# ma-compbio/MATCHA

Measured on AMD Instinct MI355X. Metric: training hyperedges/sec at k∈{2..5}, embed_dim=64; 1/2/4/8 MI355X, higher is better.
Workload: dtype f32; 1 GPU; hg38_1mb bins (N=3067), k in {2,3,4,5} mixed-k zero-padded to L=5, embed_dim=64, front end=table, neg_num=3, dropout on, AdamW lr=1e-3, 400000 known hyperedges; parallelism=dp1, hipgraph=False, table_gradient_exchange=none, embedding_backward=float atomics, exchange_overlapped=False

## Files before the change

matcha_amd/csrc/fused_bwd.hip:

```cpp
#include <stdlib.h>
#include <string.h>

#include "bf16x3.hpp"
#include "kernels.hpp"
#include "tail_reduce.hpp"

namespace matcha {

typedef float f32x16 __attribute__((ext_vector_type(16)));

namespace {

constexpr int kLd = 68;
constexpr float kEpsLn = 1e-5f;
constexpr int kWgSlab = 4 * 4096 + 6 * 64;
constexpr int kVecOff = 4 * 4096;
constexpr int kMaxChunks = 64;

#define ZR8(p)                                                                                           \
  do {                                                                                                   \
    *reinterpret_cast<float4*>(p) = make_float4(0.f, 0.f, 0.f, 0.f);                                     \
    *reinterpret_cast<float4*>((p) + 4) = make_float4(0.f, 0.f, 0.f, 0.f);                               \
  } while (0)

__device__ __forceinline__ void ln_row16(const float4& v, float& mean, float& rstd) {
  const float s = group_sum<16>((v.x + v.y) + (v.z + v.w));
  mean = s * (1.f / 64.f);
  const float a = v.x - mean, b = v.y - mean, c = v.z - mean, e = v.w - mean;
  const float q = group_sum<16>((a * a + b * b) + (c * c + e * e));
  rstd = __builtin_amdgcn_rsqf(q * (1.f / 64.f) + kEpsLn);
}


#define FB_PIN(addr, x) asm volatile("" : "+v"(addr), "+v"((x).a), "+v"((x).b), "+v"((x).c), "+v"((x).d))
template <int ML>
__device__ __forceinline__ void attn_row8_kv(const float* __restrict__ Qs, const float* __restrict__ Xs, const float* __restrict__ Fs,
                                             const float* __restrict__ xpad, const float* __restrict__ Ps, float* __restrict__ dSs, int li, int li0,
                                             int k, int n_pad, int sub, float inv_temp, V8& o, V8& gq, V8& accK, V8& accV) {
  const float padf = (float)n_pad;
  const bool hp = n_pad > 0;
  float p[ML], ds[ML], pp;
  {
    const float4 pa = *reinterpret_cast<const float4*>(&Ps[li * 8]), pb = *reinterpret_cast<const float4*>(&Ps[li * 8 + 4]);
    const float w[8] = {pa.x, pa.y, pa.z, pa.w, pb.x, pb.y, pb.z, pb.w};
#pragma unroll
    for (int j = 0; j < ML; ++j) p[j] = (j < k) ? w[j] : 0.f;
    pp = hp ? w[7] : 0.f;
  }
  const float ppf = padf * pp;
  const int ro0 = li0 * kLd + 8 * sub;
  const V8 go = ld8(&Fs[li * kLd + 8 * sub]);
  const V8 vp = ld8(xpad + 8 * sub);
  const float dsp_raw = group_sum8_dpp(dot8(go, vp));
  float sig = ppf * dsp_raw;
  o = scale8(ppf, vp);
  V8 a = scale8(ppf * dsp_raw, vp);
  V8 vn = ld8(&Xs[ro0]), vn2 = ld8(&Xs[ro0 + (1 < k ? 1 : 0) * kLd]);
#pragma unroll
  for (int j = 0; j < ML; ++j) {
    const V8 v = vn;
    vn = vn2;
    if (j + 2 < ML) {
      int ad = ro0 + (j + 2 < k ? j + 2 : 0) * kLd;
      FB_PIN(ad, o);
      vn2 = ld8(&Xs[ad]);
    }
    axpy8(o, p[j], v);
    const float d = group_sum8_dpp(dot8(go, v));
    ds[j] = d;
    const float wd = p[j] * d;
    sig += wd;
    axpy8(a, wd, v);
  }
#pragma unroll
  for (int j = 0; j < ML; ++j) ds[j] = p[j] * (ds[j] - sig) * inv_temp;
  const float dspf = padf * (pp * (dsp_raw - sig) * inv_temp);
  axpy8(accV, ppf, go);
  {
    const float ns = -sig;
    axpy8(a, ns, o);
    gq = scale8(inv_temp, a);
  }
  {
    int ad = li * kLd + 8 * sub;
    FB_PIN(ad, gq);
    const V8 q = ld8(&Qs[ad]);
    axpy8(accK, dspf, q);
  }
  if (sub == 1) {
    float* dst = dSs + li * 8;
    *reinterpret_cast<float4*>(dst) = make_float4(ds[0], ds[1 % ML], ML > 2 ? ds[2 % ML] : 0.f, ML > 3 ? ds[3 % ML] : 0.f);
    if (ML > 4) *reinterpret_cast<float4*>(dst + 4) = make_float4(ds[4 % ML], ML > 5 ? ds[5 % ML] : 0.f, ML > 6 ? ds[6 % ML] : 0.f, ML > 7 ? ds[7 % ML] : 0.f);
  }
}

template <int ML>
__device__ __forceinline__ void attn_col8(const float* __restrict__ Qs, const float* __restrict__ Fs, const float* __restrict__ Ps,
                                          const float* __restrict__ dSs, int li, int li0, int k, int sub, V8& gk, V8& gv) {
  const int jj = li - li0;
  gk = zero8();
  gv = zero8();
  const int ro0 = li0 * kLd + 8 * sub;
  V8 qn = ld8(&Qs[ro0]), gn = ld8(&Fs[ro0]);
#pragma unroll
  for (int i = 0; i < ML; ++i) {
    const V8 q = qn, go = gn;
    const int ri = li0 + (i < k ? i : 0);
    const float pl = Ps[ri * 8 + jj], dl = dSs[ri * 8 + jj];
    const float pij = (i < k) ? pl : 0.f, dsij = (i < k) ? dl : 0.f;
    if (i + 1 < ML) {
      int a = ro0 + (i + 1 < k ? i + 1 : 0) * kLd;
      FB_PIN(a, gk);
      qn = ld8(&Qs[a]); gn = ld8(&Fs[a]);
    }
    axpy8(gv, pij, go);
    axpy8(gk, dsij, q);
  }
}

#ifdef FB_TIMING
#define FB_T(i) do { const long long now__ = wall_clock64(); tph[i] += now__ - tlast; tlast = now__; } while (0)
#else
#define FB_T(i) do { } while (0)
#endif

#define MFMA16(A, B, C) __builtin_amdgcn_mfma_f32_16x16x4f32((A), (B), (C), 0, 0, 0)

constexpr int kWgSlabM = 2 * 4096 + 4 * 64;
constexpr int kVecOffM = 2 * 4096;
constexpr int kTileH = 32 * kLd;
constexpr int kPS = 80;
constexpr int kPlane = 32 * kPS;
constexpr int kPT = 3 * kPlane;
typedef Planes<kPS, 16> PL;
__device__ __forceinline__ Frag3 frag_row(const short* __restrict__ p) { return PL::row(p); }
__device__ __forceinline__ void frag_store(short* __restrict__ p, const Frag3& f) { PL::store(p, f); }
__device__ __forceinline__ Frag3 frag_col(const short* __restrict__ p) { return PL::col(p); }

struct FusedBwdHArgs {
  const float* X; const float* dDyn; const int32_t* count; const int32_t* half_meta; const int32_t* tok_pos;
  int L; int nhalves; int nchunks;
  const float* mB; const float* mM;
  float* dxh; int64_t tcap;
  int dx_atomic;
  float* wslab;
  const float* rimg;
  const int32_t* xrow;
  const float* rn; int64_t rn_head;
};
constexpr size_t kBwdLdsBytes = (size_t)2 * kTileH * 4 + (size_t)4 * kPT * 2 + (64 + 256 + 256 + 32) * 4;

template <int ML, bool NODE>
__global__ __launch_bounds__(256) __attribute__((amdgpu_waves_per_eu(2, 2))) void fused_bwdh_kernel(FusedBwdHArgs g) {
  extern __shared__ __attribute__((aligned(16))) float lds[];
  float* Xs = lds;
  float* Gs = lds + kTileH;
  short* Xp = reinterpret_cast<short*>(lds + 2 * kTileH);
  short* Dp = Xp + kPT;
  short* RBp = Dp + kPT;
  short* FBp = RBp + kPT;
  float* Rs = reinterpret_cast<float*>(RBp);
  float* Fs = reinterpret_cast<float*>(FBp);
  float* sm = reinterpret_cast<float*>(FBp + kPT);
  float* xpad = sm;
  float* dSs = xpad + 64;
  float* Ps = dSs + 256;
  int* tinfo = reinterpret_cast<int*>(Ps + 256);

  const int tid = threadIdx.x, lane = tid & 63, wave = tid >> 6;
  const int c16 = lane & 15, kq = lane >> 4;
  const int fb = 16 * wave;
  const int srow = tid >> 4, sc4 = (tid & 15) * 4;

  int head, chunk;
  if ((g.nchunks & 7) == 0) {
    const int xcd = blockIdx.x & 7, j = blockIdx.x >> 3;
    head = j & 7;
    chunk = (j >> 3) * 8 + xcd;
  } else {
    head = blockIdx.x & 7;
    chunk = blockIdx.x >> 3;
  }
  const int tr = g.count[1];
  int nh = g.count[3];
  if (nh > g.nhalves) nh = g.nhalves;
  const int per = (nh + g.nchunks - 1) / g.nchunks;
  const int tile_lo = chunk * per;
  const int tile_hi = (tile_lo + per < nh) ? tile_lo + per : nh;
  const float inv_temp = 0.125f;
#ifdef FB_TIMING
  long long tph[8] = {0, 0, 0, 0, 0, 0, 0, 0};
  long long tlast = wall_clock64();
#endif

  if (tid < 16) {
    const float4 xv = *reinterpret_cast<const float4*>(g.X + (NODE ? (int64_t)0 : (int64_t)tr * 64) + sc4);
    if constexpr (NODE) {
      *reinterpret_cast<float4*>(&xpad[sc4]) = xv;
    } else {
      float m, rs;
      ln_row16(xv, m, rs);
      *reinterpret_cast<float4*>(&xpad[sc4]) = make_float4((xv.x - m) * rs, (xv.y - m) * rs, (xv.z - m) * rs, (xv.w - m) * rs);
    }
  }

  f32x4 ab0 = {0.f, 0.f, 0.f, 0.f}, ab1 = ab0, ab2 = ab0, ab3 = ab0, am0 = ab0, am1 = ab0, am2 = ab0, am3 = ab0;
  V8 accK = zero8(), accV = zero8();
  f2 cd0 = {0.f, 0.f}, cd1 = cd0;
  V8 accR = zero8();

  const int4* meta = reinterpret_cast<const int4*>(g.half_meta);
  const int4 mzero = make_int4(0, 0, 0, 0);
  int4 mc = tile_lo < tile_hi ? meta[tile_lo] : mzero;
  int4 mn = tile_lo + 1 < tile_hi ? meta[tile_lo + 1] : mzero;
  float4 xn0, xn1, dn0, dn1;
  int tpn = 0;
  int kx0 = 0, kx1 = 0;
#define FBH_KEY_GLOAD(I, M)                                                                              \
  do {                                                                                                   \
    const int row__ = srow + 16 * (I);                                                                   \
    kx##I = g.xrow[(M).x + (row__ < (M).y ? row__ : ((M).y > 0 ? (M).y - 1 : 0))];                       \
  } while (0)
  f32x4 ri0, ri1, pn = {0.f, 0.f, 0.f, 0.f};
#define FBH_ROW_GLOAD(I, M)                                                                              \
  do {                                                                                                   \
    const int row__ = srow + 16 * (I);                                                                   \
    const int64_t tok__ = (M).x + (row__ < (M).y ? row__ : ((M).y > 0 ? (M).y - 1 : 0));                 \
    xn##I = *reinterpret_cast<const float4*>(g.X + (NODE ? (int64_t)kx##I : tok__) * 64 + sc4);           \
    dn##I = *reinterpret_cast<const float4*>(g.dDyn + tok__ * 64 + sc4);                                 \
  } while (0)
#define FBH_ROWS_GLOAD(M)                                                                                \
  do {                                                                                                   \
    FBH_ROW_GLOAD(0, M); FBH_ROW_GLOAD(1, M);                                                            \
    if (tid < 32) tpn = g.tok_pos[(M).x + (tid < (M).y ? tid : ((M).y > 0 ? (M).y - 1 : 0))];           \
  } while (0)
  const bool r_tab = NODE && g.rn != nullptr;
#define FBH_R_GLOAD()                                                                                    \
  do {                                                                                                   \
    const float* rh__ = g.rn + (int64_t)head * g.rn_head + sc4;                                          \
    ri0 = *reinterpret_cast<const f32x4*>(rh__ + (int64_t)kx0 * 64); ri1 = *reinterpret_cast<const f32x4*>(rh__ + (int64_t)kx1 * 64); \
  } while (0)
#define FBH_ROW_STAGE(I)                                                                                 \
  do {                                                                                                   \
    const int row__ = srow + 16 * (I);                                                                   \
    const float msk__ = row__ < n_real ? 1.f : 0.f;                                                      \
    const float4 xv__ = xn##I, dv__ = dn##I;                                                             \
    float4 xh__;                                                                                         \
    if constexpr (NODE) {                                                                                \
      xh__ = make_float4(xv__.x * msk__, xv__.y * msk__, xv__.z * msk__, xv__.w * msk__);                \
    } else {                                                                                             \
      const float mean__ = group_sum16_dpp((xv__.x + xv__.y) + (xv__.z + xv__.w)) * (1.f / 64.f);        \
      const float a__ = xv__.x - mean__, b__ = xv__.y - mean__, c__ = xv__.z - mean__, e__ = xv__.w - mean__; \
      const float q__ = group_sum16_dpp((a__ * a__ + b__ * b__) + (c__ * c__ + e__ * e__));              \
      const float rs__ = msk__ * __builtin_amdgcn_rsqf(q__ * (1.f / 64.f) + kEpsLn);                     \
      xh__ = make_float4(a__ * rs__, b__ * rs__, c__ * rs__, e__ * rs__);                                \
    }                                                                                                    \
    *reinterpret_cast<float4*>(&Xs[row__ * kLd + sc4]) = xh__;                                           \
    {                                                                                                    \
      const P3 p0__ = split2(xh__.x, xh__.y), p1__ = split2(xh__.z, xh__.w);                             \
      short* d__ = Xp + row__ * kPS + sc4;                                                               \
      *reinterpret_cast<u32x2*>(d__) = (u32x2){p0__.h, p1__.h}; *reinterpret_cast<u32x2*>(d__ + kPlane) = (u32x2){p0__.m, p1__.m}; \
      *reinterpret_cast<u32x2*>(d__ + 2 * kPlane) = (u32x2){p0__.l, p1__.l};                             \
    }                                                                                                    \
    const float4 dm__ = make_float4(dv__.x * msk__, dv__.y * msk__, dv__.z * msk__, dv__.w * msk__);     \
    {                                                                                                    \
      const P3 p0__ = split2(dm__.x, dm__.y), p1__ = split2(dm__.z, dm__.w);                             \
      short* d__ = Dp + row__ * kPS + sc4;                                                               \
      *reinterpret_cast<u32x2*>(d__) = (u32x2){p0__.h, p1__.h}; *reinterpret_cast<u32x2*>(d__ + kPlane) = (u32x2){p0__.m, p1__.m}; \
      *reinterpret_cast<u32x2*>(d__ + 2 * kPlane) = (u32x2){p0__.l, p1__.l};                             \
    }                                                                                                    \
    cd0 += (f2){dm__.x, dm__.y}; cd1 += (f2){dm__.z, dm__.w};                                            \
  } while (0)
#define FBH_RIMG_GLOAD(HALF)                                                                             \
  do {                                                                                                   \
    const f32x4* r__ = reinterpret_cast<const f32x4*>(g.rimg + ((int64_t)(HALF) * MATCHA_N_HEAD + head) * kImgRecH);  \
    if (tid < 64) pn = __builtin_nontemporal_load(r__ + 512 + tid);                                      \
    if (!r_tab) { ri0 = __builtin_nontemporal_load(r__ + tid); ri1 = __builtin_nontemporal_load(r__ + 256 + tid); } \
  } while (0)
  Frag3 Mf[2], Bf[2];
  {
    if constexpr (NODE) { FBH_KEY_GLOAD(0, mc); FBH_KEY_GLOAD(1, mc); }
    FBH_ROWS_GLOAD(mc);
    if constexpr (NODE) { if (r_tab) FBH_R_GLOAD(); FBH_KEY_GLOAD(0, mn); FBH_KEY_GLOAD(1, mn); }
    if (tile_lo < tile_hi) FBH_RIMG_GLOAD(tile_lo);
    const float* mp = g.mM + (int64_t)head * 4096 + (8 * kq) * 64 + fb + c16;
    const float* bp = g.mB + (int64_t)head * 4096 + (8 * kq) * 64 + fb + c16;
#pragma unroll
    for (int s = 0; s < 2; ++s) {
      float vm[8], vb[8];
#pragma unroll
      for (int j = 0; j < 8; ++j) { vm[j] = mp[(32 * s + j) * 64]; vb[j] = bp[(32 * s + j) * 64]; }
      Mf[s] = split8(vm); Bf[s] = split8(vb);
    }
  }

  for (int tile = tile_lo; tile < tile_hi; ++tile) {
    const int4 mnn = tile + 2 < tile_hi ? meta[tile + 2] : mzero;
    const int t0 = mc.x, n_real = mc.y;
    FB_T(0);
    __syncthreads();
    FB_T(7);
    {
      FBH_ROW_STAGE(0); FBH_ROW_STAGE(1);
      if (tid < 32) tinfo[tid] = tid < n_real ? ((tid - (tpn & 255)) | (tpn & ~255)) : 0;
      if (r_tab) {
        *reinterpret_cast<f32x4*>(&Rs[srow * kLd + sc4]) = ri0; *reinterpret_cast<f32x4*>(&Rs[(srow + 16) * kLd + sc4]) = ri1;
      } else {
        f32x4* d__ = reinterpret_cast<f32x4*>(&Rs[(lane & 31) * kLd + 8 * wave + 4 * (lane >> 5)]);
        d__[0] = ri0; d__[8] = ri1;
      }
      if (tid < 64) reinterpret_cast<f32x4*>(Ps)[tid] = pn;
    }
    __syncthreads();
    int tid_ = tid;
    asm volatile("" : "+v"(tid_));
    const int lane = tid_ & 63, wave = tid_ >> 6;
    const int c16 = lane & 15, kq = lane >> 4;
    const int fb = 16 * wave;
    const int srow = tid_ >> 4, sc4 = (tid_ & 15) * 4;
    const int sub = lane & 7;
    (void)srow; (void)sc4;
    {
      f32x4 acc0 = {0.f, 0.f, 0.f, 0.f}, acc1 = acc0;
      const short* dp = Dp + c16 * kPS + 8 * kq;
#pragma unroll
      for (int s = 0; s < 2; ++s) {
        const Frag3 b0 = frag_row(dp + 32 * s), b1 = frag_row(dp + 16 * kPS + 32 * s);
        acc0 = mma6(acc0, Mf[s], b0); acc1 = mma6(acc1, Mf[s], b1);
      }
      *reinterpret_cast<f32x4*>(&Fs[c16 * kLd + fb + 4 * kq]) = acc0;
      *reinterpret_cast<f32x4*>(&Fs[(16 + c16) * kLd + fb + 4 * kq]) = acc1;
    }
    FB_T(1);
    __syncthreads();
    FB_T(7);
    {
      V8 o0, q0, k0, v0;
      const int la = wave * 8 + (lane >> 3);
      const bool acta = la < n_real;
      int ia = 0;
      if (acta) { ia = tinfo[la]; attn_row8_kv<ML>(Rs, Xs, Fs, xpad, Ps, dSs, la, ia & 255, ia >> 8, g.L - (ia >> 8), sub, inv_temp, o0, q0, accK, accV); }
      __builtin_amdgcn_sched_barrier(0);
      FB_T(2);
      __syncthreads();
      FB_T(7);
      if (acta) {
        attn_col8<ML>(Rs, Fs, Ps, dSs, la, ia & 255, ia >> 8, sub, k0, v0);
        k0.a += v0.a; k0.b += v0.b; k0.c += v0.c; k0.d += v0.d;
        st8(&Gs[la * kLd + 8 * sub], k0);
      } else {
        ZR8(&Gs[la * kLd + 8 * sub]);
      }
      FB_T(3);
      __syncthreads();
      FB_T(7);
      if (!acta) { o0 = zero8(); q0 = zero8(); }
      frag_store(FBp + la * kPS + 8 * sub, split8(o0));
      frag_store(RBp + la * kPS + 8 * sub, split8(q0));
      accR.a += q0.a; accR.b += q0.b; accR.c += q0.c; accR.d += q0.d;
    }
    FB_T(4);
    __syncthreads();
    FB_T(7);
    FBH_ROWS_GLOAD(mn);
    if constexpr (NODE) { if (r_tab) FBH_R_GLOAD(); FBH_KEY_GLOAD(0, mnn); FBH_KEY_GLOAD(1, mnn); }
    if (g.dx_atomic) {
      const float* gp = Gs + (4 * kq) * kLd + fb + c16;
      f32x4 dx0 = {gp[0], gp[kLd], gp[2 * kLd], gp[3 * kLd]};
      f32x4 dx1 = {gp[16 * kLd], gp[17 * kLd], gp[18 * kLd], gp[19 * kLd]};
      const short* arow = RBp + c16 * kPS + 8 * kq;
#pragma unroll
      for (int s = 0; s < 2; ++s) {
        const Frag3 a0 = frag_row(arow + 32 * s), a1 = frag_row(arow + 16 * kPS + 32 * s);
        dx0 = mma6(dx0, a0, Bf[s]); dx1 = mma6(dx1, a1, Bf[s]);
      }
      float* out = g.dxh + ((int64_t)t0 + 4 * kq) * 64 + fb + c16;
#pragma unroll
      for (int reg = 0; reg < 4; ++reg) {
        if (4 * kq + reg < n_real) unsafeAtomicAdd(out + reg * 64, dx0[reg]);
        if (16 + 4 * kq + reg < n_real) unsafeAtomicAdd(out + (16 + reg) * 64, dx1[reg]);
      }
    } else {
      f32x4 dx0 = *reinterpret_cast<const f32x4*>(&Gs[c16 * kLd + fb + 4 * kq]);
      f32x4 dx1 = *reinterpret_cast<const f32x4*>(&Gs[(16 + c16) * kLd + fb + 4 * kq]);
      const short* arow = RBp + c16 * kPS + 8 * kq;
#pragma unroll
      for (int s = 0; s < 2; ++s) {
        const Frag3 a0 = frag_row(arow + 32 * s), a1 = frag_row(arow + 16 * kPS + 32 * s);
        dx0 = mma6(dx0, Bf[s], a0); dx1 = mma6(dx1, Bf[s], a1);
      }
      float* out = g.dxh + ((int64_t)head * g.tcap + t0 + c16) * 64 + fb + 4 * kq;
      if (c16 < n_real) *reinterpret_cast<f32x4*>(out) = dx0;
      if (16 + c16 < n_real) *reinterpret_cast<f32x4*>(out + 16 * 64) = dx1;
    }
    FB_T(5);
    if (tile + 1 < tile_hi) FBH_RIMG_GLOAD(tile + 1);
    {
      const int blk = ((4 * kq + ((lane & 15) >> 2)) * kPS) + 4 * (lane & 3);
      const Frag3 xb = frag_col(Xp + blk + fb), zb = frag_col(FBp + blk + fb);
      {
        const Frag3 r0 = frag_col(RBp + blk), r1 = frag_col(RBp + blk + 16);
        ab0 = mma6(ab0, r0, xb); ab1 = mma6(ab1, r1, xb);
        const Frag3 r2 = frag_col(RBp + blk + 32), r3 = frag_col(RBp + blk + 48);
        ab2 = mma6(ab2, r2, xb); ab3 = mma6(ab3, r3, xb);
      }
      {
        const Frag3 d0 = frag_col(Dp + blk), d1 = frag_col(Dp + blk + 16);
        am0 = mma6(am0, d0, zb); am1 = mma6(am1, d1, zb);
        const Frag3 d2 = frag_col(Dp + blk + 32), d3 = frag_col(Dp + blk + 48);
        am2 = mma6(am2, d2, zb); am3 = mma6(am3, d3, zb);
      }
    }
    FB_T(6);
    mc = mn; mn = mnn;
  }

  __syncthreads();
#ifdef FB_TIMING
  if (blockIdx.x == 0 && (tid == 0 || tid == 192))
    printf("fused_bwdh wg0 wave %d us: stage %.1f dZ %.1f attn-row %.1f attn-col %.1f attn-write %.1f dx %.1f tn %.1f barrier-wait %.1f (halves %d)\n", tid >> 6,
           tph[0] * 0.01, tph[1] * 0.01, tph[2] * 0.01, tph[3] * 0.01, tph[4] * 0.01, tph[5] * 0.01, tph[6] * 0.01, tph[7] * 0.01, tile_hi - tile_lo);
#endif
  float* slab = g.wslab + ((int64_t)head * g.nchunks + chunk) * kWgSlabM;
  {
    const int col = fb + c16;
#pragma unroll
    for (int reg = 0; reg < 4; ++reg) {
      const int row = 4 * kq + reg;
      slab[0 * 4096 + row * 64 + col] = ab0[reg]; slab[0 * 4096 + (row + 16) * 64 + col] = ab1[reg];
      slab[0 * 4096 + (row + 32) * 64 + col] = ab2[reg]; slab[0 * 4096 + (row + 48) * 64 + col] = ab3[reg];
      slab[1 * 4096 + row * 64 + col] = am0[reg]; slab[1 * 4096 + (row + 16) * 64 + col] = am1[reg];
      slab[1 * 4096 + (row + 32) * 64 + col] = am2[reg]; slab[1 * 4096 + (row + 48) * 64 + col] = am3[reg];
    }
  }
  float* redd = lds;
  {
    const float cdv[4] = {cd0.x, cd0.y, cd1.x, cd1.y};
#pragma unroll
    for (int i = 0; i < 4; ++i) {
      float v = cdv[i];
      v += __shfl_xor(v, 16, 64);
      v += __shfl_xor(v, 32, 64);
      if (lane < 16) redd[wave * 64 + 4 * lane + i] = v;
    }
  }
  float* redr = lds + 4 * 64;
  float* redp = lds + 8 * 64;
  const float accp[16] = {accK.a.x + accV.a.x, accK.a.y + accV.a.y, accK.b.x + accV.b.x, accK.b.y + accV.b.y,
                          accK.c.x + accV.c.x, accK.c.y + accV.c.y, accK.d.x + accV.d.x, accK.d.y + accV.d.y,
                          accR.a.x, accR.a.y, accR.b.x, accR.b.y, accR.c.x, accR.c.y, accR.d.x, accR.d.y};
#pragma unroll
  for (int i = 0; i < 16; ++i) {
    float v = accp[i];
    v += __shfl_xor(v, 8, 64);
    v += __shfl_xor(v, 16, 64);
    v += __shfl_xor(v, 32, 64);
    if (lane < 8) (i < 8 ? redp : redr)[wave * 64 + 8 * lane + (i & 7)] = v;
  }
  __syncthreads();
  if (tid < 64) {
    slab[kVecOffM + 64 + tid] = (redd[tid] + redd[64 + tid]) + (redd[128 + tid] + redd[192 + tid]);
    slab[kVecOffM + tid] = (redr[tid] + redr[64 + tid]) + (redr[128 + tid] + redr[192 + tid]);
    slab[kVecOffM + 128 + tid] = (redp[tid] + redp[64 + tid]) + (redp[128 + tid] + redp[192 + tid]);
  }
}

struct ChainArgs {
  const float* wslab; int nchunks;
  float* red;
  const float* wq; const float* wk; const float* wv; const float* cq; const float* cv;
  const float* fc1_w;
  float* out;
  float* dxpad;
};
constexpr int kFbmReduceX = (kWgSlabM + 255) / 256;
constexpr int kFbmReduceBlocks = kFbmReduceX * MATCHA_N_HEAD;
__global__ __launch_bounds__(256) void fbm_reduce_kernel(ChainArgs a, TailReduceArgs tl, int tail_blocks) {
  __shared__ float4 part[8 * 32];
  if ((int)blockIdx.x >= kFbmReduceBlocks) {
    tail_reduce_role(tl, (int)blockIdx.x - kFbmReduceBlocks, part);
    return;
  }
  const int head = blockIdx.x / kFbmReduceX, i = (blockIdx.x % kFbmReduceX) * 256 + threadIdx.x;
  if (i >= kWgSlabM) return;
  const float* base = a.wslab + (int64_t)head * a.nchunks * kWgSlabM + i;
  float s0 = 0.f, s1 = 0.f, s2 = 0.f, s3 = 0.f, s4 = 0.f, s5 = 0.f, s6 = 0.f, s7 = 0.f;
  int c = 0;
  for (; c + 7 < a.nchunks; c += 8) {
    s0 += base[(int64_t)c * kWgSlabM]; s1 += base[(int64_t)(c + 1) * kWgSlabM]; s2 += base[(int64_t)(c + 2) * kWgSlabM]; s3 += base[(int64_t)(c + 3) * kWgSlabM];
    s4 += base[(int64_t)(c + 4) * kWgSlabM]; s5 += base[(int64_t)(c + 5) * kWgSlabM]; s6 += base[(int64_t)(c + 6) * kWgSlabM]; s7 += base[(int64_t)(c + 7) * kWgSlabM];
  }
  for (; c < a.nchunks; ++c) s0 += base[(int64_t)c * kWgSlabM];
  a.red[(int64_t)head * kWgSlabM + i] = ((s0 + s1) + (s2 + s3)) + ((s4 + s5) + (s6 + s7));
}
__device__ __forceinline__ void mm64_slice(const float* __restrict__ A, int a_rs, int a_cs, const float* __restrict__ B, int b_rs, int b_cs,
                                           const float* __restrict__ u, const float* __restrict__ v, float* __restrict__ out, int slice,
                                           float* __restrict__ As, float* __restrict__ Bs) {
  const int tid = threadIdx.x;
  {
    float av[4], bv[16];
#pragma unroll
    for (int t = 0; t < 4; ++t) { const int i = tid + 256 * t; av[t] = A[(int64_t)(16 * slice + (i >> 6)) * a_rs + (int64_t)(i & 63) * a_cs]; }
#pragma unroll
    for (int t = 0; t < 16; ++t) { const int i = tid + 256 * t; bv[t] = B[(int64_t)(i >> 6) * b_rs + (int64_t)(i & 63) * b_cs]; }
#pragma unroll
    for (int t = 0; t < 4; ++t) { const int i = tid + 256 * t; As[(i >> 6) * 65 + (i & 63)] = av[t]; }
#pragma unroll
    for (int t = 0; t < 16; ++t) { const int i = tid + 256 * t; Bs[(i >> 6) * 65 + (i & 63)] = bv[t]; }
  }
  __syncthreads();
  const int lane = tid & 63, wave = tid >> 6, c16 = lane & 15, kq = lane >> 4;
  f32x4 acc = {0.f, 0.f, 0.f, 0.f};
#pragma unroll
  for (int kk = 0; kk < 16; ++kk) acc = MFMA16(As[c16 * 65 + 4 * kk + kq], Bs[(4 * kk + kq) * 65 + 16 * wave + c16], acc);
  const int j = 16 * wave + c16;
  const float vj = u ? v[j] : 0.f;
#pragma unroll
  for (int reg = 0; reg < 4; ++reg) {
    const int i = 4 * kq + reg;
    out[(16 * slice + i) * 64 + j] = acc[reg] + (u ? u[16 * slice + i] * vj : 0.f);
  }
}
__global__ __launch_bounds__(256) void fbm_chain_kernel(ChainArgs a) {
  __shared__ float As[16 * 65];
  __shared__ float Bs[64 * 65];
  const int slice = blockIdx.x, job = blockIdx.y, head = blockIdx.z, tid = threadIdx.x;
  const float* red = a.red + (int64_t)head * kWgSlabM;
  const float* dB = red; const float* dM = red + 4096; const float* db = red + kVecOffM;
  const float* dbdyn = a.red + kVecOffM + 64;
  const float* Wq = a.wq + (int64_t)head * 4096; const float* Wk = a.wk + (int64_t)head * 4096; const float* Wv = a.wv + (int64_t)head * 4096;
  const float* Wf = a.fc1_w + head * 64;
  float* out = a.out + (int64_t)head * kWgSlab;
  if (job == 0) {
    mm64_slice(Wk, 64, 1, dB, 64, 1, nullptr, nullptr, out + 0 * 4096, slice, As, Bs);
  } else if (job == 1) {
    mm64_slice(Wq, 64, 1, dB, 1, 64, a.cq + head * 64, db, out + 1 * 4096, slice, As, Bs);
  } else if (job == 2) {
    mm64_slice(Wf, 1, 512, dM, 64, 1, nullptr, nullptr, out + 2 * 4096, slice, As, Bs);
  } else {
    mm64_slice(dM, 64, 1, Wv, 1, 64, dbdyn, a.cv + head * 64, out + 3 * 4096, slice, As, Bs);
  }
  if (slice == 0 && job == 0 && tid < 64) {
    float s0 = 0.f, s1 = 0.f, t0 = 0.f, t1 = 0.f;
#pragma unroll 8
    for (int x = 0; x < 64; x += 2) {
      s0 += Wk[tid * 64 + x] * db[x]; s1 += Wk[tid * 64 + x + 1] * db[x + 1];
      t0 += Wf[x * 512 + tid] * dbdyn[x]; t1 += Wf[(x + 1) * 512 + tid] * dbdyn[x + 1];
    }
    const float s = s0 + s1, t = t0 + t1;
    out[kVecOff + tid] = s;
    out[kVecOff + 64 + tid] = 0.f;
    out[kVecOff + 128 + tid] = t;
    out[kVecOff + 192 + tid] = 0.f; out[kVecOff + 256 + tid] = 0.f;
    out[kVecOff + 320 + tid] = head == 0 ? dbdyn[tid] : 0.f;
    if (head == 0) {
      float p = 0.f;
      for (int hh = 0; hh < MATCHA_N_HEAD; ++hh) p += a.red[(int64_t)hh * kWgSlabM + kVecOffM + 128 + tid];
      a.dxpad[tid] = p;
    }
  }
}

struct UnfoldArgs {
  const float* wslab; int nchunks;
  const float* X; const int32_t* count; int x_pad_row0;
  const float* W[3]; const float* g[3]; const float* b[3];
  float* gW[3]; float* gfc1;
  float* part;
};
__global__ __launch_bounds__(256) void fb_unfold_kernel(UnfoldArgs a) {
  __shared__ float red[16][3][64];
  const int slice = blockIdx.x, mat = blockIdx.y, head = blockIdx.z;
  const int tid = threadIdx.x, rl = tid >> 4, c4 = (tid & 15) * 4;
  const int row = slice * 16 + rl;
  const float* base = a.wslab + (int64_t)head * a.nchunks * kWgSlab;
  float4 s = make_float4(0.f, 0.f, 0.f, 0.f);
  {
    float4 t0 = s, t1 = s, t2 = s, t3 = s;
    const float* pb = base + mat * 4096 + row * 64 + c4;
    int c = 0;
    for (; c + 3 < a.nchunks; c += 4) {
      const float4 v0 = *reinterpret_cast<const float4*>(pb + (int64_t)c * kWgSlab), v1 = *reinterpret_cast<const float4*>(pb + (int64_t)(c + 1) * kWgSlab);
      const float4 v2 = *reinterpret_cast<const float4*>(pb + (int64_t)(c + 2) * kWgSlab), v3 = *reinterpret_cast<const float4*>(pb + (int64_t)(c + 3) * kWgSlab);
      t0.x += v0.x; t0.y += v0.y; t0.z += v0.z; t0.w += v0.w;
      t1.x += v1.x; t1.y += v1.y; t1.z += v1.z; t1.w += v1.w;
      t2.x += v2.x; t2.y += v2.y; t2.z += v2.z; t2.w += v2.w;
      t3.x += v3.x; t3.y += v3.y; t3.z += v3.z; t3.w += v3.w;
    }
    for (; c < a.nchunks; ++c) {
      const float4 v = *reinterpret_cast<const float4*>(pb + (int64_t)c * kWgSlab);
      t0.x += v.x; t0.y += v.y; t0.z += v.z; t0.w += v.w;
    }
    s.x = (t0.x + t1.x) + (t2.x + t3.x); s.y = (t0.y + t1.y) + (t2.y + t3.y);
    s.z = (t0.z + t1.z) + (t2.z + t3.z); s.w = (t0.w + t1.w) + (t2.w + t3.w);
  }
  if (mat == 3) {
    float4* o = reinterpret_cast<float4*>(a.gfc1 + (int64_t)row * 512 + head * 64 + c4);
    float4 v = *o;
    v.x += s.x; v.y += s.y; v.z += s.z; v.w += s.w;
    *o = v;
    return;
  }
  float dc = 0.f, dpad = 0.f;
  for (int c = 0; c < a.nchunks; ++c) {
    const float* vb = base + (int64_t)c * kWgSlab + kVecOff;
    dc += vb[mat * 64 + row];
    if (mat > 0) dpad += vb[192 + (mat - 1) * 64 + row];
  }
  const float4 xv = *reinterpret_cast<const float4*>(a.X + (a.x_pad_row0 ? (int64_t)0 : (int64_t)a.count[1] * 64) + c4);
  float m, rs;
  ln_row16(xv, m, rs);
  s.x += dpad * (xv.x - m) * rs; s.y += dpad * (xv.y - m) * rs; s.z += dpad * (xv.z - m) * rs; s.w += dpad * (xv.w - m) * rs;
  dc += dpad;
  const int64_t wi = ((int64_t)head * 64 + row) * 64 + c4;
  const float4 W = *reinterpret_cast<const float4*>(a.W[mat] + wi);
  const float4 G = *reinterpret_cast<const float4*>(a.g[mat] + c4), Bv = *reinterpret_cast<const float4*>(a.b[mat] + c4);
  {
    float4* o = reinterpret_cast<float4*>(a.gW[mat] + wi);
    float4 v = *o;
    v.x += s.x * G.x + dc * Bv.x; v.y += s.y * G.y + dc * Bv.y; v.z += s.z * G.z + dc * Bv.z; v.w += s.w * G.w + dc * Bv.w;
    *o = v;
  }
  *reinterpret_cast<float4*>(&red[rl][0][c4]) = make_float4(s.x * W.x, s.y * W.y, s.z * W.z, s.w * W.w);
  *reinterpret_cast<float4*>(&red[rl][1][c4]) = make_float4(dc * W.x, dc * W.y, dc * W.z, dc * W.w);
  *reinterpret_cast<float4*>(&red[rl][2][c4]) = make_float4(dpad * W.x * G.x, dpad * W.y * G.y, dpad * W.z * G.z, dpad * W.w * G.w);
  __syncthreads();
  if (tid < 192) {
    const int which = tid >> 6, k = tid & 63;
    float t = 0.f;
#pragma unroll
    for (int q = 0; q < 16; ++q) t += red[q][which][k];
    a.part[(((int64_t)(head * 4 + slice) * 3 + mat) * 3 + which) * 64 + k] = t;
  }
}

struct Unfold2Args {
  const float* part; const float* wslab; int nchunks;
  float* dg[3]; float* db[3]; float* dfc1_b; float* dxpad;
  int dxpad_add;
};
__global__ __launch_bounds__(512) void fb_unfold2_kernel(Unfold2Args a) {
  const int vec = threadIdx.x >> 6, k = threadIdx.x & 63;
  float s = 0.f;
  if (vec < 6) {
    const int mat = vec >> 1, which = vec & 1;
    for (int p = 0; p < 32; ++p) s += a.part[(((int64_t)p * 3 + mat) * 3 + which) * 64 + k];
    float* o = (which == 0 ? a.dg[mat] : a.db[mat]) + k;
    *o += s;
  } else if (vec == 6) {
    for (int p = 0; p < 32; ++p) s += a.part[(((int64_t)p * 3 + 1) * 3 + 2) * 64 + k] + a.part[(((int64_t)p * 3 + 2) * 3 + 2) * 64 + k];
    a.dxpad[k] = a.dxpad_add ? a.dxpad[k] + s : s;
  } else {
    for (int c = 0; c < a.nchunks; ++c) s += a.wslab[(int64_t)c * kWgSlab + kVecOff + 320 + k];
    a.dfc1_b[k] += s;
  }
}

__global__ __launch_bounds__(256) void lnhat_bwd_kernel(const float* __restrict__ X, const float* __restrict__ dxh, int64_t tcap,
                                                        const float* __restrict__ dxpad, const float* __restrict__ dXs,
                                                        float* __restrict__ dZ0, const int32_t* __restrict__ count, int nslab) {
  const int T = count[0];
  const int64_t t = (int64_t)blockIdx.x * 16 + (threadIdx.x >> 4);
  const int c4 = (threadIdx.x & 15) * 4;
  if (t >= T) return;
  const float4 xv = *reinterpret_cast<const float4*>(X + t * 64 + c4);
  float m, rs;
  ln_row16(xv, m, rs);
  const float4 xh = make_float4((xv.x - m) * rs, (xv.y - m) * rs, (xv.z - m) * rs, (xv.w - m) * rs);
  float4 d;
  if (t < T - 1) {
    d = *reinterpret_cast<const float4*>(dxh + t * 64 + c4);
    for (int hd = 1; hd < nslab; ++hd) {
      const float4 v = *reinterpret_cast<const float4*>(dxh + ((int64_t)hd * tcap + t) * 64 + c4);
      d.x += v.x; d.y += v.y; d.z += v.z; d.w += v.w;
    }
  } else {
    d = *reinterpret_cast<const float4*>(dxpad + c4);
  }
  const float a = group_sum<16>((d.x + d.y) + (d.z + d.w)) * (1.f / 64.f);
  const float b = group_sum<16>((d.x * xh.x + d.y * xh.y) + (d.z * xh.z + d.w * xh.w)) * (1.f / 64.f);
  const float4 s = *reinterpret_cast<const float4*>(dXs + t * 64 + c4);
  float4 o;
  o.x = (rs * (d.x - a - xh.x * b) + s.x) * (1.f - xv.x * xv.x);
  o.y = (rs * (d.y - a - xh.y * b) + s.y) * (1.f - xv.y * xv.y);
  o.z = (rs * (d.z - a - xh.z * b) + s.z) * (1.f - xv.z * xv.z);
  o.w = (rs * (d.w - a - xh.w * b) + s.w) * (1.f - xv.w * xv.w);
  *reinterpret_cast<float4*>(dZ0 + t * 64 + c4) = o;
}

int chunks_for(int ntiles) {
  const int cus = device_cu_count();
  int c = cus / MATCHA_N_HEAD;
  if (c > kMaxChunks) c = kMaxChunks;
  if (c > ntiles) c = ntiles;
  return c < 1 ? 1 : c;
}

}

const float* fused_bwd_dxpad(const float* ws) { return ws + (size_t)MATCHA_N_HEAD * kMaxChunks * kWgSlab + 32 * 3 * 3 * 64; }

size_t fused_bwd_ws_floats(int64_t B, int L) {
  (void)B; (void)L;
  return (size_t)MATCHA_N_HEAD * kMaxChunks * kWgSlab + (size_t)32 * 3 * 3 * 64 + 64;
}

int launch_fused_bwd_merged(const matcha_tensors& p, const float* folded, const float* merged, const float* X, const float* dDyn, const float* dXs,
                            const Ragged& rg, int64_t B, int L, float* dxh, float* ws, matcha_tensors& grads, float* dZ0, hipStream_t st, const float* rimg,
                            bool dx_atomic, bool dx_zeroed, const TailReduceArgs* tail, const int32_t* xrow, const float* xhatN, const float* rn, int64_t rn_rows) {
  const int64_t tcap = B * L + 1;
  MATCHA_CHECK_ARG(!xrow || xhatN, "fused backward: the node route needs the table of normalised rows");
  MATCHA_CHECK_ARG(!rn || xrow, "fused backward: the r table belongs to the node route");
  if (dx_atomic && !dx_zeroed) MATCHA_TRY(zero_async(dxh, (size_t)tcap * 64 * sizeof(float), st));
  int nchunks = 2 * chunks_for(rg.nhalves);
  if (nchunks > kMaxChunks) nchunks = kMaxChunks;
  if (nchunks > rg.nhalves) nchunks = rg.nhalves > 0 ? rg.nhalves : 1;
  float* wslab = ws;
  float* chain = ws + (size_t)MATCHA_N_HEAD * kMaxChunks * kWgSlabM;
  float* part = ws + (size_t)MATCHA_N_HEAD * kMaxChunks * kWgSlab;
  float* dxpad = part + 32 * 3 * 3 * 64;
  const size_t wsz = (size_t)MATCHA_N_HEAD * 64 * 64, csz = (size_t)MATCHA_N_HEAD * 64;
  const MergedView mv = merged_view(merged);
  {
    FusedBwdHArgs g;
    g.X = xrow ? xhatN : X; g.dDyn = dDyn; g.count = rg.count; g.half_meta = rg.half_meta; g.tok_pos = rg.tok_pos; g.L = L; g.nhalves = rg.nhalves; g.nchunks = nchunks;
    g.mB = mv.B; g.mM = mv.M; g.dxh = dxh; g.tcap = tcap; g.dx_atomic = dx_atomic ? 1 : 0; g.wslab = wslab; g.rimg = rimg; g.xrow = xrow;
    g.rn = rn; g.rn_head = rn_rows * 64;
    const size_t lds = kBwdLdsBytes;
    auto launch = [&](auto kfn) {
      (void)hipFuncSetAttribute(reinterpret_cast<const void*>(kfn), hipFuncAttributeMaxDynamicSharedMemorySize, 160 * 1024);
      hipLaunchKernelGGL(kfn, dim3(MATCHA_N_HEAD * nchunks), dim3(256), lds, st, g);
    };
    ProfScope ps(MATCHA_PROF_FUSED_BWD, (double)tcap * MATCHA_N_HEAD * 8.0 * 2.0 * 64.0 * 64.0, st);
    switch (L <= 2 ? 2 : (L <= 6 ? L : 8)) {
      case 2: if (xrow) launch(fused_bwdh_kernel<2, true>); else launch(fused_bwdh_kernel<2, false>); break;
      case 3: if (xrow) launch(fused_bwdh_kernel<3, true>); else launch(fused_bwdh_kernel<3, false>); break;
      case 4: if (xrow) launch(fused_bwdh_kernel<4, true>); else launch(fused_bwdh_kernel<4, false>); break;
      case 5: if (xrow) launch(fused_bwdh_kernel<5, true>); else launch(fused_bwdh_kernel<5, false>); break;
      case 6: if (xrow) launch(fused_bwdh_kernel<6, true>); else launch(fused_bwdh_kernel<6, false>); break;
      default: if (xrow) launch(fused_bwdh_kernel<8, true>); else launch(fused_bwdh_kernel<8, false>); break;
    }
    MATCHA_CHECK_LAUNCH("fused_bwdh_kernel");
  }
  {
    ChainArgs c;
    c.wslab = wslab; c.nchunks = nchunks; c.red = chain + (size_t)MATCHA_N_HEAD * kWgSlab;
    c.wq = folded; c.wk = folded + wsz; c.wv = folded + 2 * wsz; c.cq = folded + 3 * wsz; c.cv = c.cq + 2 * csz;
    c.fc1_w = p.fc1_w; c.out = chain; c.dxpad = dxpad;
    TailReduceArgs tl;
    if (tail) tl = *tail; else memset(&tl, 0, sizeof(tl));
    const int tail_blocks = tail ? kTailRoleBlocks : 0;
    hipLaunchKernelGGL(fbm_reduce_kernel, dim3((unsigned)(kFbmReduceBlocks + tail_blocks)), dim3(256), 0, st, c, tl, tail_blocks);
    MATCHA_CHECK_LAUNCH("fbm_reduce_kernel");
    hipLaunchKernelGGL(fbm_chain_kernel, dim3(4, 4, MATCHA_N_HEAD), dim3(256), 0, st, c);
    MATCHA_CHECK_LAUNCH("fbm_chain_kernel");
  }
  {
    UnfoldArgs a;
    a.wslab = chain; a.nchunks = 1; a.X = X; a.count = rg.count; a.x_pad_row0 = xrow ? 1 : 0;
    a.W[0] = p.w_q; a.W[1] = p.w_k; a.W[2] = p.w_v;
    a.g[0] = p.ln_q_g; a.g[1] = p.ln_k_g; a.g[2] = p.ln_v_g;
    a.b[0] = p.ln_q_b; a.b[1] = p.ln_k_b; a.b[2] = p.ln_v_b;
    a.gW[0] = grads.w_q; a.gW[1] = grads.w_k; a.gW[2] = grads.w_v; a.gfc1 = grads.fc1_w;
    a.part = part;
    hipLaunchKernelGGL(fb_unfold_kernel, dim3(4, 4, MATCHA_N_HEAD), dim3(256), 0, st, a);
    MATCHA_CHECK_LAUNCH("fb_unfold_kernel");
    Unfold2Args b;
    b.part = part; b.wslab = chain; b.nchunks = 1;
    b.dg[0] = grads.ln_q_g; b.dg[1] = grads.ln_k_g; b.dg[2] = grads.ln_v_g;
    b.db[0] = grads.ln_q_b; b.db[1] = grads.ln_k_b; b.db[2] = grads.ln_v_b;
    b.dfc1_b = grads.fc1_b; b.dxpad = dxpad; b.dxpad_add = 1;
    hipLaunchKernelGGL(fb_unfold2_kernel, dim3(1), dim3(512), 0, st, b);
    MATCHA_CHECK_LAUNCH("fb_unfold2_kernel");
  }
  if (dZ0) {
    MATCHA_CHECK_ARG(!xrow, "fused backward: the node route has no dZ0 output");
    hipLaunchKernelGGL(lnhat_bwd_kernel, dim3((unsigned)cdiv(tcap, 16)), dim3(256), 0, st, X, dxh, tcap, dxpad, dXs, dZ0, rg.count, dx_atomic ? 1 : MATCHA_N_HEAD);
    MATCHA_CHECK_LAUNCH("lnhat_bwd_kernel");
  }
  return MATCHA_OK;
}

}
```

matcha_amd/csrc/fused_fwd32.hip:

```cpp
#include "kernels.hpp"
#include "prep_heads.hpp"

#ifndef F32_ABL
#define F32_ABL 0
#endif

namespace matcha {

typedef float f32x16 __attribute__((ext_vector_type(16)));

namespace {

constexpr int kLdH = 68;
constexpr int kHT = 32 * kLdH;
constexpr float kEps32 = 1e-5f;
constexpr int kTailVec32 = 2 * 4096;
constexpr int kTailSlab32 = 2 * 4096 + 10 * 64;

struct FL { f32x16 lo, hi; };

__device__ __forceinline__ float xhalf_sum(float v) {
  float a = v, b = v;
  asm volatile("s_nop 1\n\tv_permlane32_swap_b32 %0, %1" : "+v"(a), "+v"(b));
  return a + b;
}
__device__ __forceinline__ float fl_sum(const FL& a) {
  float s0 = 0.f, s1 = 0.f;
#pragma unroll
  for (int e = 0; e < 16; ++e) { s0 += a.lo[e]; s1 += a.hi[e]; }
  return s0 + s1;
}
__device__ __forceinline__ float fl_dot(const FL& a, const FL& b) {
  float s0 = 0.f, s1 = 0.f;
#pragma unroll
  for (int e = 0; e < 16; ++e) { s0 += a.lo[e] * b.lo[e]; s1 += a.hi[e] * b.hi[e]; }
  return s0 + s1;
}
__device__ __forceinline__ void fl_stats(const FL& v, float& mean, float& rstd) {
  mean = xhalf_sum(fl_sum(v)) * (1.f / 64.f);
  float q0 = 0.f, q1 = 0.f;
#pragma unroll
  for (int e = 0; e < 16; ++e) { const float a = v.lo[e] - mean, b = v.hi[e] - mean; q0 += a * a; q1 += b * b; }
  rstd = __builtin_amdgcn_rsqf(xhalf_sum(q0 + q1) * (1.f / 64.f) + kEps32);
}
__device__ __forceinline__ void fl_store(float* __restrict__ rowp, const FL& v) {
#pragma unroll
  for (int g = 0; g < 4; ++g) {
    *reinterpret_cast<f32x4*>(rowp + 8 * g) = (f32x4){v.lo[4 * g], v.lo[4 * g + 1], v.lo[4 * g + 2], v.lo[4 * g + 3]};
    *reinterpret_cast<f32x4*>(rowp + 32 + 8 * g) = (f32x4){v.hi[4 * g], v.hi[4 * g + 1], v.hi[4 * g + 2], v.hi[4 * g + 3]};
  }
}
__device__ __forceinline__ FL fl_load(const float* __restrict__ rowp) {
  FL v;
#pragma unroll
  for (int g = 0; g < 4; ++g) {
    const f32x4 a = *reinterpret_cast<const f32x4*>(rowp + 8 * g), b = *reinterpret_cast<const f32x4*>(rowp + 32 + 8 * g);
    v.lo[4 * g] = a.x; v.lo[4 * g + 1] = a.y; v.lo[4 * g + 2] = a.z; v.lo[4 * g + 3] = a.w;
    v.hi[4 * g] = b.x; v.hi[4 * g + 1] = b.y; v.hi[4 * g + 2] = b.z; v.hi[4 * g + 3] = b.w;
  }
  return v;
}
__device__ __forceinline__ float fl_dot_lds(const FL& q, const float* __restrict__ rowp) {
  f2 s = {0.f, 0.f}, t = {0.f, 0.f};
#pragma unroll
  for (int g = 0; g < 4; ++g) {
    const f32x4 a = *reinterpret_cast<const f32x4*>(rowp + 8 * g), b = *reinterpret_cast<const f32x4*>(rowp + 32 + 8 * g);
    s = __builtin_elementwise_fma((f2){q.lo[4 * g], q.lo[4 * g + 1]}, (f2){a.x, a.y}, s);
    t = __builtin_elementwise_fma((f2){q.lo[4 * g + 2], q.lo[4 * g + 3]}, (f2){a.z, a.w}, t);
    s = __builtin_elementwise_fma((f2){q.hi[4 * g], q.hi[4 * g + 1]}, (f2){b.x, b.y}, s);
    t = __builtin_elementwise_fma((f2){q.hi[4 * g + 2], q.hi[4 * g + 3]}, (f2){b.z, b.w}, t);
  }
  s += t;
  return s.x + s.y;
}
__device__ __forceinline__ void fl_axpy_lds(FL& o, float w, const float* __restrict__ rowp) {
#pragma unroll
  for (int g = 0; g < 4; ++g) {
    const f32x4 a = *reinterpret_cast<const f32x4*>(rowp + 8 * g), b = *reinterpret_cast<const f32x4*>(rowp + 32 + 8 * g);
    o.lo[4 * g] += w * a.x; o.lo[4 * g + 1] += w * a.y; o.lo[4 * g + 2] += w * a.z; o.lo[4 * g + 3] += w * a.w;
    o.hi[4 * g] += w * b.x; o.hi[4 * g + 1] += w * b.y; o.hi[4 * g + 2] += w * b.z; o.hi[4 * g + 3] += w * b.w;
  }
}
__device__ __forceinline__ void fl_add_vec(FL& v, const float* __restrict__ vec_h) {
#pragma unroll
  for (int g = 0; g < 4; ++g) {
    const f32x4 a = *reinterpret_cast<const f32x4*>(vec_h + 8 * g), b = *reinterpret_cast<const f32x4*>(vec_h + 32 + 8 * g);
    v.lo[4 * g] += a.x; v.lo[4 * g + 1] += a.y; v.lo[4 * g + 2] += a.z; v.lo[4 * g + 3] += a.w;
    v.hi[4 * g] += b.x; v.hi[4 * g + 1] += b.y; v.hi[4 * g + 2] += b.z; v.hi[4 * g + 3] += b.w;
  }
}
__device__ __forceinline__ FL fl_vec(const float* __restrict__ vec_h) {
  FL v;
#pragma unroll
  for (int e = 0; e < 16; ++e) { v.lo[e] = 0.f; v.hi[e] = 0.f; }
  fl_add_vec(v, vec_h);
  return v;
}
__device__ __forceinline__ void fl_store_global(float* __restrict__ rowp_h, const FL& v) {
#pragma unroll
  for (int g = 0; g < 4; ++g) {
    *reinterpret_cast<f32x4*>(rowp_h + 8 * g) = (f32x4){v.lo[4 * g], v.lo[4 * g + 1], v.lo[4 * g + 2], v.lo[4 * g + 3]};
    *reinterpret_cast<f32x4*>(rowp_h + 32 + 8 * g) = (f32x4){v.hi[4 * g], v.hi[4 * g + 1], v.hi[4 * g + 2], v.hi[4 * g + 3]};
  }
}

__device__ __forceinline__ int f32_tok(int lane, int t0, int n, int tok_pad) {
  asm volatile("" : "+v"(lane));
  const int rr = lane & 31;
  return rr < n ? t0 + rr : tok_pad;
}
__device__ __forceinline__ int64_t f32_row(int lane, int t0, int n, int tok_pad) {
  asm volatile("" : "+v"(lane));
  const int rr = lane & 31;
  return (int64_t)(rr < n ? t0 + rr : tok_pad) * 64 + 4 * (lane >> 5);
}
#define F32_TOK() f32_tok(lane, t0, n, tok_pad)
#define F32_ROW() f32_row(lane, t0, n, tok_pad)
__device__ __forceinline__ FL fl_unpark(const float* __restrict__ base, int64_t off) { return fl_load(base + off); }
__device__ __forceinline__ FL fl_unpark_lds(const float* __restrict__ base, int off) {
  asm volatile("" : "+v"(off));
  return fl_load(base + off);
}
#define F32_WAVE_SYNC() asm volatile("s_waitcnt lgkmcnt(0)" ::: "memory")

#define MFMA32(A, B, C) __builtin_amdgcn_mfma_f32_32x32x2f32((A), (B), (C), 0, 0, 0)

#define MFMA_BF(A, B, C) __builtin_amdgcn_mfma_f32_32x32x16_bf16(__builtin_bit_cast(bf16x8, (A)), __builtin_bit_cast(bf16x8, (B)), (C), 0, 0, 0)
#ifndef F32_WIN
#define F32_WIN 6
#endif

struct B3 { u32x4 h, m, l; };
#define FL_CHUNK(V, C, J) ((C) < 2 ? (V).lo[8 * ((C) & 1) + (J)] : (V).hi[8 * ((C) & 1) + (J)])
#define FL_SPLIT(OUT, V, C)                                                                              \
  do {                                                                                                   \
    _Pragma("unroll") for (int q__ = 0; q__ < 4; ++q__) {                                                \
      if (F32_ABL & 128) { (OUT).h[q__] = __builtin_bit_cast(uint32_t, FL_CHUNK(V, C, 2 * q__)); (OUT).m[q__] = (OUT).h[q__]; (OUT).l[q__] = (OUT).h[q__]; continue; } \
      const P3 p__ = split2(FL_CHUNK(V, C, 2 * q__), FL_CHUNK(V, C, 2 * q__ + 1));                       \
      (OUT).h[q__] = p__.h; (OUT).m[q__] = p__.m; (OUT).l[q__] = p__.l;                                  \
    }                                                                                                    \
  } while (0)
#define WB_MMA(ACC, XB, S)                                                                               \
  do {                                                                                                   \
    const u32x4 ah__ = W_[(3 * (S)) % F32_WIN], am__ = W_[(3 * (S) + 1) % F32_WIN], al__ = W_[(3 * (S) + 2) % F32_WIN]; \
    if constexpr (((S) & 1) == 0) {                                                                      \
      ACC.lo = MFMA_BF(al__, (XB).h, ACC.lo); ACC.lo = MFMA_BF(ah__, (XB).l, ACC.lo); ACC.lo = MFMA_BF(am__, (XB).m, ACC.lo); \
      ACC.lo = MFMA_BF(am__, (XB).h, ACC.lo); ACC.lo = MFMA_BF(ah__, (XB).m, ACC.lo); ACC.lo = MFMA_BF(ah__, (XB).h, ACC.lo); \
    } else {                                                                                             \
      ACC.hi = MFMA_BF(al__, (XB).h, ACC.hi); ACC.hi = MFMA_BF(ah__, (XB).l, ACC.hi); ACC.hi = MFMA_BF(am__, (XB).m, ACC.hi); \
      ACC.hi = MFMA_BF(am__, (XB).h, ACC.hi); ACC.hi = MFMA_BF(ah__, (XB).m, ACC.hi); ACC.hi = MFMA_BF(ah__, (XB).h, ACC.hi); \
    }                                                                                                    \
  } while (0)
#define WB_REFILL(S, PF)                                                                                 \
  do {                                                                                                   \
    if ((PF) && !(F32_ABL & 32)) {                                                                       \
      W_[(3 * (S)) % F32_WIN] = wp[lane]; W_[(3 * (S) + 1) % F32_WIN] = (wp + 64)[lane]; W_[(3 * (S) + 2) % F32_WIN] = (wp + 128)[lane]; \
    }                                                                                                    \
    wp += 192;                                                                                           \
    asm volatile("" ::: "memory");          \
    __builtin_amdgcn_sched_barrier(0);                                                                   \
  } while (0)
#define WB_CHUNK(ACC, B, C, PF)                                                                          \
  do {                                                                                                   \
    B3 xb__;                                                                                             \
    FL_SPLIT(xb__, B, C);                                                                                \
    WB_MMA(ACC, xb__, 2 * (C)); WB_REFILL(2 * (C), PF); WB_MMA(ACC, xb__, 2 * (C) + 1); WB_REFILL(2 * (C) + 1, PF); \
  } while (0)
#define W32_CHAIN(ACC, B, PF_LAST)                                                                       \
  do { WB_CHUNK(ACC, B, 0, true); WB_CHUNK(ACC, B, 1, true); WB_CHUNK(ACC, B, 2, true); WB_CHUNK(ACC, B, 3, PF_LAST); } while (0)
#define W32_CHAIN_XS(ACC, XS, PF_LAST)                                                                   \
  do {                                                                                                   \
    WB_MMA(ACC, XS[0], 0); WB_REFILL(0, true); WB_MMA(ACC, XS[0], 1); WB_REFILL(1, true);                \
    WB_MMA(ACC, XS[1], 2); WB_REFILL(2, true); WB_MMA(ACC, XS[1], 3); WB_REFILL(3, true);                \
    WB_MMA(ACC, XS[2], 4); WB_REFILL(4, true); WB_MMA(ACC, XS[2], 5); WB_REFILL(5, true);                \
    WB_MMA(ACC, XS[3], 6); WB_REFILL(6, PF_LAST); WB_MMA(ACC, XS[3], 7); WB_REFILL(7, PF_LAST);          \
  } while (0)
#define W32_PRIME_AT(MAT)                                                                                \
  do {                                                                                                   \
    wp = g.wfrag + (MAT) * kFragU4;                                                                      \
    _Pragma("unroll") for (int i__ = 0; i__ < F32_WIN; ++i__) W_[i__] = (wp + i__ * 64)[lane];           \
    wp += F32_WIN * 64;                                                                                  \
  } while (0)

__device__ __forceinline__ FL fl_zero() {
  FL v;
#pragma unroll
  for (int e = 0; e < 16; ++e) { v.lo[e] = 0.f; v.hi[e] = 0.f; }
  return v;
}

}

__global__ __launch_bounds__(256) void prep_heads_kernel(PrepArgs a) {
  __shared__ __attribute__((aligned(16))) float sm[kPrepLdsFloats];
  prep_heads_role(a, blockIdx.x, blockIdx.y, blockIdx.z, sm);
}

struct Fwd32Args {
  const float* X;
  const int32_t* xrow;
  const int32_t* row_off; const int32_t* tok_slot; const int32_t* count; const int32_t* half_meta; const int32_t* tok_pos;
  int L;
  const u32x4* wfrag;
  HeadParams hp;
  const float* y; const float* w;
  float* Y; float* H1; float* H2;
  float* logits; float* row_loss;
  const uint64_t* seed;
  float p_fc1, p_pff;
  float* ddyn0; float* dXs; float* tslab; float alpha_over_B;
  int objective;
  float* qkv;
  float* tail_dh2;
  const float* rn;
  int rn_rows;
};

template <int ML>
__global__ __launch_bounds__(64) __attribute__((amdgpu_waves_per_eu(2, 2))) void fused_fwd32_kernel(Fwd32Args g) {
  extern __shared__ __attribute__((aligned(16))) float lds[];
#ifdef FF_TIMING
  long long tph[16] = {0};
  long long tlast = wall_clock64();
#define FF_T(i) do { const long long now__ = wall_clock64(); tph[i] += now__ - tlast; tlast = now__; } while (0)
#else
#define FF_T(i) do { } while (0)
#endif
  float* TK = lds;
  float* TV = lds + kHT;
  float* outs = lds + 2 * kHT;
  float* douts = outs + 32;
  const int lane = threadIdx.x, r = lane & 31, h = lane >> 5;

  const int4 meta = reinterpret_cast<const int4*>(g.half_meta)[blockIdx.x];
  const int t0 = meta.x, n = meta.y, b0 = meta.z, n_h = meta.w;
  if (n_h <= 0) return;
  const int tok_pad = g.count[1];
  const float inv_temp = 0.125f;
  const bool real = r < n;

  const u32x4* wp;
  u32x4 W_[F32_WIN];
  W32_PRIME_AT(g.rn ? 2 : 0);
  {
    const f32x4* bsrc = reinterpret_cast<const f32x4*>(g.wfrag + (kNMat + 1) * kFragU4);
    for (int i4 = lane; i4 < kNBias * 16; i4 += 64) reinterpret_cast<f32x4*>(TV)[i4] = bsrc[i4];
  }
#define F32_BIAS(ROW) fl_vec(TV + (ROW) * 64 + 4 * h)

  int64_t xoff = F32_ROW();
  if (g.xrow) xoff = (int64_t)g.xrow[F32_TOK()] * 64 + 4 * h;
  FL xh = fl_load(g.X + xoff);
  int pos = 0, k = 0;
  if (real) {
    const int tp = g.tok_pos[F32_TOK()];
    pos = tp & 255; k = tp >> 8;
  }
  const int li0 = r - pos;
  float rx;
  {
    float mean;
    fl_stats(xh, mean, rx);
#pragma unroll
    for (int e = 0; e < 16; ++e) { xh.lo[e] = (xh.lo[e] - mean) * rx; xh.hi[e] = (xh.hi[e] - mean) * rx; }
  }
  constexpr int kRec = kImgRecH;
  float* const img_base = g.qkv ? g.qkv + (int64_t)blockIdx.x * MATCHA_N_HEAD * kImgRecH : nullptr;
  const bool img_on = g.qkv != nullptr && real;
#define F32_IMG_STORE(ACC, HD, M)                                                                        \
  do {                                                                                                   \
    if (img_on && !(F32_ABL & 2)) {                                                                      \
      int l__ = lane;                                                                                    \
      asm volatile("" : "+v"(l__));                                                                      \
      f32x4* d__ = reinterpret_cast<f32x4*>(img_base + (HD) * kRec + (M) * 4096 + l__ * 4);             \
      _Pragma("unroll") for (int g__ = 0; g__ < 4; ++g__) {                                              \
        if (F32_ABL & 16) {                                                                              \
          d__[g__ * 64] = (f32x4){ACC.lo[4 * g__], ACC.lo[4 * g__ + 1], ACC.lo[4 * g__ + 2], ACC.lo[4 * g__ + 3]};   \
          d__[(4 + g__) * 64] = (f32x4){ACC.hi[4 * g__], ACC.hi[4 * g__ + 1], ACC.hi[4 * g__ + 2], ACC.hi[4 * g__ + 3]}; \
        } else {                                                                                         \
        __builtin_nontemporal_store((f32x4){ACC.lo[4 * g__], ACC.lo[4 * g__ + 1], ACC.lo[4 * g__ + 2], ACC.lo[4 * g__ + 3]}, d__ + g__ * 64); \
        __builtin_nontemporal_store((f32x4){ACC.hi[4 * g__], ACC.hi[4 * g__ + 1], ACC.hi[4 * g__ + 2], ACC.hi[4 * g__ + 3]}, d__ + (4 + g__) * 64); \
        }                                                                                                \
      }                                                                                                  \
    }                                                                                                    \
  } while (0)

  const int n_pad = g.L - k;
  const float padf = (float)n_pad;
  const bool hpad = n_pad > 0;
  int ro[ML + 1];
#pragma unroll
  for (int j = 0; j < ML; ++j) ro[j] = (li0 + (j < k ? j : 0)) * kLdH + 4 * h;
  ro[ML] = n * kLdH + 4 * h;
  float* krow = TK + r * kLdH + 4 * h;
  float* vrow = TV + r * kLdH + 4 * h;

#define F32_PIN1(V) asm volatile("" : "+v"(V))
  float p[ML + 1];
  float sc_part = 0.f;
#define F32_SC_PIECE(S)                                                                                  \
  do {                                                                                                   \
    constexpr int j__ = (S) >> 1, hf__ = (S) & 1;                                                        \
    if constexpr (j__ <= ML) {                                                                           \
      const float* rp__ = TK + ro[j__] + 32 * hf__;                                                      \
      f2 s__ = {0.f, 0.f}, t__ = {0.f, 0.f};                                                             \
      _Pragma("unroll") for (int g__ = 0; g__ < 4; ++g__) {                                              \
        const f32x4 a__ = *reinterpret_cast<const f32x4*>(rp__ + 8 * g__);                               \
        const f32x16& qq__ = hf__ ? q.hi : q.lo;                                                         \
        s__ = __builtin_elementwise_fma((f2){qq__[4 * g__], qq__[4 * g__ + 1]}, (f2){a__.x, a__.y}, s__); \
        t__ = __builtin_elementwise_fma((f2){qq__[4 * g__ + 2], qq__[4 * g__ + 3]}, (f2){a__.z, a__.w}, t__); \
      }                                                                                                  \
      s__ += t__;                                                                                        \
      if constexpr (hf__ == 0) { sc_part = s__.x + s__.y; F32_PIN1(sc_part); }                            \
      else {                                                                                             \
        float a__ = xhalf_sum(sc_part + (s__.x + s__.y)) * inv_temp;                                     \
        if constexpr (j__ < ML) a__ = (j__ == pos) ? -1e32f : a__;      \
        p[j__] = a__;                                                                                    \
        F32_PIN1(p[j__]);                                                                                \
      }                                                                                                  \
    }                                                                                                    \
    if constexpr ((S) == 2 * (ML + 1)) {                                                                 \
      float mx__ = -3.4e38f;                                                                             \
      _Pragma("unroll") for (int i__ = 0; i__ < ML; ++i__) mx__ = (i__ < k) ? fmaxf(mx__, p[i__]) : mx__; \
      mx__ = hpad ? fmaxf(mx__, p[ML]) : mx__;                                                           \
      float den__ = 0.f;                                                                                 \
      _Pragma("unroll") for (int i__ = 0; i__ < ML; ++i__) { p[i__] = (i__ < k) ? __expf(p[i__] - mx__) : 0.f; den__ += p[i__]; } \
      p[ML] = hpad ? __expf(p[ML] - mx__) : 0.f;                                                         \
      den__ += padf * p[ML];                                                                             \
      const float inv__ = __builtin_amdgcn_rcpf(den__);                                                  \
      _Pragma("unroll") for (int i__ = 0; i__ <= ML; ++i__) { p[i__] *= inv__; F32_PIN1(p[i__]); }       \
    }                                                                                                    \
    if constexpr ((S) == 2 * (ML + 1) + 1) {                                                             \
       \
      if (img_on && h == 0) {                                                                            \
        float wv__[8];                                                                                   \
        _Pragma("unroll") for (int i__ = 0; i__ < 8; ++i__) wv__[i__] = i__ < ML ? p[i__ < ML ? i__ : 0] : 0.f; \
        if (hpad) wv__[7] = p[ML];                                                                       \
        int l__ = lane;                                                                                  \
        asm volatile("" : "+v"(l__));                                                                    \
        f32x4* dst__ = reinterpret_cast<f32x4*>(img_base + hd * kRec + 2048 + (l__ & 31) * 8);          \
        __builtin_nontemporal_store((f32x4){wv__[0], wv__[1], wv__[2], wv__[3]}, dst__);                 \
        __builtin_nontemporal_store((f32x4){wv__[4], wv__[5], wv__[6], wv__[7]}, dst__ + 1);             \
      }                                                                                                  \
    }                                                                                                    \
  } while (0)
#define F32_STAGE8(MAC) do { MAC(0); MAC(1); MAC(2); MAC(3); MAC(4); MAC(5); MAC(6); MAC(7); } while (0)

  FF_T(0);
  fl_store(krow, xh);
  FL dyn;
  if (!g.rn) {
  B3 xs[4];
  FL_SPLIT(xs[0], xh, 0); FL_SPLIT(xs[1], xh, 1); FL_SPLIT(xs[2], xh, 2); FL_SPLIT(xs[3], xh, 3);
  F32_WAVE_SYNC();
  dyn = F32_BIAS(kBiasDyn);
  {
    FL q = F32_BIAS(kBiasR), o;
    W32_CHAIN_XS(q, xs, true);
    F32_IMG_STORE(q, 0, 0);
    FF_T(1);
#define F32_Z_PIECE(S)                                                                                   \
  do {                                                                                                   \
    constexpr int j__ = (S) >> 1, hf__ = (S) & 1;                                                        \
    if constexpr (j__ <= ML) {                                                                           \
      const float* rp__ = TK + ro[j__] + 32 * hf__;                                                      \
      const float w__ = j__ < ML ? p[j__] : padf * p[ML];                                                \
      const f2 w2__ = {w__, w__};                                                                        \
      f32x16& oo__ = hf__ ? o.hi : o.lo;                                                                 \
      _Pragma("unroll") for (int g__ = 0; g__ < 4; ++g__) {                                              \
        const f32x4 a__ = *reinterpret_cast<const f32x4*>(rp__ + 8 * g__);                               \
        const f2 u0__ = __builtin_elementwise_fma(w2__, (f2){a__.x, a__.y}, (f2){oo__[4 * g__], oo__[4 * g__ + 1]});     \
        const f2 u1__ = __builtin_elementwise_fma(w2__, (f2){a__.z, a__.w}, (f2){oo__[4 * g__ + 2], oo__[4 * g__ + 3]}); \
        oo__[4 * g__] = u0__.x; oo__[4 * g__ + 1] = u0__.y; oo__[4 * g__ + 2] = u1__.x; oo__[4 * g__ + 3] = u1__.y;      \
      }                                                                                                  \
      asm volatile("" : "+v"(oo__));                                                                     \
    }                                                                                                    \
  } while (0)
#define F32_MG_PIECE(Q)                                                                                  \
  do {                                                                                                   \
    if constexpr ((F32_ABL & 1) != 0) { } else                                                           \
    if constexpr ((Q) < 2 * (ML + 1) + 2) F32_SC_PIECE(Q); else F32_Z_PIECE((Q) - (2 * (ML + 1) + 2));   \
  } while (0)
#define F32_MG_ONLY(S) do { F32_MG_PIECE(5 * (S)); F32_MG_PIECE(5 * (S) + 1); F32_MG_PIECE(5 * (S) + 2); F32_MG_PIECE(5 * (S) + 3); F32_MG_PIECE(5 * (S) + 4); } while (0)
#define F32_MG_STEP(S) do { WB_MMA(acc, xs[(S) >> 1], S); F32_MG_ONLY(S); WB_REFILL(S, true); } while (0)
    int hd = 0;
    for (; hd + 1 < MATCHA_N_HEAD; ++hd) {
      o = fl_zero();
      {
        FL acc = F32_BIAS(kBiasR + hd + 1);
        F32_STAGE8(F32_MG_STEP);
        q = acc;
        F32_IMG_STORE(q, hd + 1, 0);
      }
      FF_T(2);
      W32_CHAIN(dyn, o, true);
      FF_T(5);
    }
    o = fl_zero();
    F32_STAGE8(F32_MG_ONLY);
    FF_T(2);
    W32_CHAIN(dyn, o, true);
    FF_T(5);
  }
  } else {
    F32_WAVE_SYNC();
    dyn = F32_BIAS(kBiasDyn);
    int roff = g.xrow[F32_TOK()] * 64 + 4 * h;
    const float* rnh = g.rn;
    FL q = fl_load(rnh + roff), o;
    FF_T(1);
    int hd = 0;
    for (; hd + 1 < MATCHA_N_HEAD; ++hd) {
      o = fl_zero();
      rnh += (int64_t)g.rn_rows * 64;
      const FL acc = fl_load(rnh + roff);
      F32_STAGE8(F32_MG_ONLY);
      FF_T(2);
      W32_CHAIN(dyn, o, false);
      W32_PRIME_AT(hd + 1 < MATCHA_N_HEAD - 1 ? 2 * hd + 4 : 15);
      q = acc;
      FF_T(5);
    }
    o = fl_zero();
    F32_STAGE8(F32_MG_ONLY);
    FF_T(2);
    W32_CHAIN(dyn, o, true);
    FF_T(5);
  }
  if (F32_ABL & 8) { if (dyn.lo[0] == 12345.f) g.logits[0] = dyn.hi[3]; return; }
#define F32_XH_RELOAD() do { xh = fl_load(krow); } while (0)
#define F32_TAIL_SYNC() F32_WAVE_SYNC()
#define F32_PARK_Y(V) do { if (g.Y) fl_store_global(g.Y + F32_ROW(), V); } while (0)
#define F32_PARK_H1(V) do { if (g.H1) fl_store_global(g.H1 + F32_ROW(), V); } while (0)
#define F32_UNPARK_Y() fl_unpark(g.Y, F32_ROW())
#define F32_UNPARK_H1() fl_unpark(g.H1, F32_ROW())
#define F32_PARK_HH(V) do { if (g.H2) fl_store_global(g.H2 + F32_ROW(), V); } while (0)
#define F32_UNPARK_HH() fl_unpark(g.H2, F32_ROW())
#include "fused_fwd32_tail.hpp"
#undef F32_TAIL_SYNC
#undef F32_PARK_Y
#undef F32_PARK_H1
#undef F32_UNPARK_Y
#undef F32_UNPARK_H1
#undef F32_PARK_HH
#undef F32_UNPARK_HH
#ifdef FF_TIMING
  if (blockIdx.x == 2000 && lane == 0)
    printf("fused_fwd32 wave 2000 us: setup %.1f prologue K0 Q0 %.1f | 8 heads: V+scores %.1f K'+PV %.1f Q' %.1f fc1 %.1f | pff fwd %.1f ln+logit %.1f | ln-bwd+colsums %.1f dW1 %.1f dZ1 %.1f dW0 %.1f ddyn %.1f\n",
           tph[0] * 0.01, tph[1] * 0.01, tph[2] * 0.01, tph[3] * 0.01, tph[4] * 0.01, tph[5] * 0.01, tph[7] * 0.01, tph[8] * 0.01, tph[9] * 0.01,
           tph[10] * 0.01, tph[11] * 0.01, tph[12] * 0.01, tph[13] * 0.01);
#endif
}

template <int ML>
__global__ __launch_bounds__(512) void fused_fwd32h_kernel(Fwd32Args g) {
  extern __shared__ __attribute__((aligned(16))) float lds[];
#undef FF_T
#define FF_T(i) do { } while (0)
  float* TK = lds;
  float* TV = lds + kHT;
  float* outs = lds + 2 * kHT;
  float* douts = outs + 32;
  float* Pd = lds + 2 * kHT + 64;
  const int lane = threadIdx.x & 63, r = lane & 31, h = lane >> 5;
  const int hd = __builtin_amdgcn_readfirstlane(threadIdx.x >> 6);

  const int4 meta = reinterpret_cast<const int4*>(g.half_meta)[blockIdx.x];
  const int t0 = meta.x, n = meta.y, b0 = meta.z, n_h = meta.w;
  if (n_h <= 0) return;
  const int tok_pad = g.count[1];
  const float inv_temp = 0.125f;
  const bool real = r < n;

  const u32x4* wp;
  u32x4 W_[F32_WIN];
  W32_PRIME_AT(hd == 0 ? 0 : 2 * hd - 1);
#undef F32_BIAS
#define F32_BIAS(ROW) fl_vec(reinterpret_cast<const float*>(g.wfrag + (kNMat + 1) * kFragU4) + (ROW) * 64 + 4 * h)

  FL xh = fl_load(g.X + F32_ROW());
  int pos = 0, k = 0;
  if (real) {
    const int tp = g.tok_pos[F32_TOK()];
    pos = tp & 255; k = tp >> 8;
  }
  const int li0 = r - pos;
  float rx;
  {
    float mean;
    fl_stats(xh, mean, rx);
#pragma unroll
    for (int e = 0; e < 16; ++e) { xh.lo[e] = (xh.lo[e] - mean) * rx; xh.hi[e] = (xh.hi[e] - mean) * rx; }
  }
  const int kRec = kImgRecH;
  float* const img_base = g.qkv ? g.qkv + (int64_t)blockIdx.x * MATCHA_N_HEAD * kImgRecH : nullptr;
  const bool img_on = g.qkv != nullptr && real;
  const int n_pad = g.L - k;
  const float padf = (float)n_pad;
  const bool hpad = n_pad > 0;
  int ro[ML + 1];
#pragma unroll
  for (int j = 0; j < ML; ++j) ro[j] = (li0 + (j < k ? j : 0)) * kLdH + 4 * h;
  ro[ML] = n * kLdH + 4 * h;
  float* krow = TK + r * kLdH + 4 * h;
  float p[ML + 1];
  float sc_part = 0.f;

  if (hd == 0) fl_store(krow, xh);
  FL q = F32_BIAS(kBiasR + hd), o = fl_zero();
  W32_CHAIN(q, xh, false);
  F32_IMG_STORE(q, hd, 0);
  W32_PRIME_AT(hd < 7 ? 2 * hd + 2 : 15);
  __syncthreads();
  F32_STAGE8(F32_MG_ONLY);
  {
    FL dynp = fl_zero();
    if (hd == 0) dynp = F32_BIAS(kBiasDyn);
    W32_CHAIN(dynp, o, false);
    fl_store(Pd + hd * kHT + r * kLdH + 4 * h, dynp);
  }
  __syncthreads();
  if (hd != 0) return;
  FL dyn = fl_load(Pd + r * kLdH + 4 * h);
#pragma unroll 1
  for (int j = 1; j < MATCHA_N_HEAD; ++j) {
    const FL t = fl_load(Pd + j * kHT + r * kLdH + 4 * h);
#pragma unroll
    for (int e = 0; e < 16; ++e) { dyn.lo[e] += t.lo[e]; dyn.hi[e] += t.hi[e]; }
  }
  W32_PRIME_AT(16);
#define F32_TAIL_SYNC() F32_WAVE_SYNC()
#define F32_PARK_Y(V) do { fl_store(Pd + r * kLdH + 4 * h, V); if (g.Y && !g.ddyn0 && r <= n) fl_store_global(g.Y + F32_ROW(), V); } while (0)
#define F32_PARK_H1(V) do { fl_store(Pd + kHT + r * kLdH + 4 * h, V); if (g.H1 && !g.ddyn0 && r <= n) fl_store_global(g.H1 + F32_ROW(), V); } while (0)
#define F32_UNPARK_Y() fl_unpark_lds(Pd, r * kLdH + 4 * h)
#define F32_UNPARK_H1() fl_unpark_lds(Pd + kHT, r * kLdH + 4 * h)
#define F32_PARK_HH(V) fl_store(Pd + 2 * kHT + r * kLdH + 4 * h, V)
#define F32_UNPARK_HH() fl_unpark_lds(Pd + 2 * kHT, r * kLdH + 4 * h)
#include "fused_fwd32_tail.hpp"
#undef F32_TAIL_SYNC
#undef F32_PARK_Y
#undef F32_PARK_H1
#undef F32_UNPARK_Y
#undef F32_UNPARK_H1
#undef F32_PARK_HH
#undef F32_UNPARK_HH
#ifdef F32H_REPRO
  if (g.L == 0x40000000) {
    __threadfence();
    unsigned int* ctr = reinterpret_cast<unsigned int*>(g.tslab);
    unsigned int t = 0;
    if (lane == 0) t = atomicAdd(ctr, 1u);
    t = __shfl(t, 0, 64);
    if (t == gridDim.x - 1) {
      float s = 0.f;
      for (int i = lane; i < g.L * 977; i += 64) s += g.row_loss[i];
#pragma unroll
      for (int o = 32; o > 0; o >>= 1) s += __shfl_xor(s, o, 64);
      if (lane == 0) g.logits[0] = s;
    }
  }
#endif
}

struct NodeRArgs { const float* X; const u32x4* wfrag; float* rn; int rows; };
__global__ __launch_bounds__(64) void node_r_kernel(NodeRArgs g) {
  const int lane = threadIdx.x, r = lane & 31, h = lane >> 5;
  const int hd = blockIdx.y;
  const int row = (int)blockIdx.x * 32 + r;
  const bool live = row < g.rows;
  const u32x4* wp;
  u32x4 W_[F32_WIN];
  W32_PRIME_AT(hd == 0 ? 0 : 2 * hd - 1);
  FL xh = fl_load(g.X + (int64_t)(live ? row : g.rows - 1) * 64 + 4 * h);
  {
    float mean, rx;
    fl_stats(xh, mean, rx);
#pragma unroll
    for (int e = 0; e < 16; ++e) { xh.lo[e] = (xh.lo[e] - mean) * rx; xh.hi[e] = (xh.hi[e] - mean) * rx; }
  }
  B3 xs[4];
  FL_SPLIT(xs[0], xh, 0); FL_SPLIT(xs[1], xh, 1); FL_SPLIT(xs[2], xh, 2); FL_SPLIT(xs[3], xh, 3);
  FL q = F32_BIAS(kBiasR + hd);
  W32_CHAIN_XS(q, xs, false);
  if (live) fl_store_global(g.rn + ((int64_t)hd * g.rows + row) * 64 + 4 * h, q);
}

size_t node_r_floats(int64_t rows) { return (size_t)MATCHA_N_HEAD * rows * 64; }
int launch_node_r(const float* XN, const float* frag, int64_t rows, float* rn, hipStream_t st) {
  NodeRArgs g;
  g.X = XN; g.wfrag = reinterpret_cast<const u32x4*>(frag); g.rn = rn; g.rows = (int)rows;
  ProfScope ps(MATCHA_PROF_FUSED_FWD, 0.0, st);
  hipLaunchKernelGGL(node_r_kernel, dim3((unsigned)cdiv(rows, 32), MATCHA_N_HEAD), dim3(64), 0, st, g);
  MATCHA_CHECK_LAUNCH("node_r_kernel");
  return MATCHA_OK;
}

static int fwd32h_max_halves() { return 2 * device_cu_count(); }

bool fused_small_batch(const Ragged& rg) { return rg.nhalves <= fwd32h_max_halves() && !options().disable_small_batch; }

size_t fused_frag_floats() { return (size_t)(kNMat + 1) * kFragU4 * 4 + (size_t)kNBias * 64; }
size_t fused_tail_slab32_floats(int64_t B, int L) { return (size_t)(ragged_halves_cap(B, L) + 2) * kTailSlab32; }

size_t fused_merged_floats() { return (size_t)2 * MATCHA_N_HEAD * 4096 + MATCHA_N_HEAD * 64 + 64; }
MergedView merged_view(const float* m) {
  return MergedView{m, m + (size_t)MATCHA_N_HEAD * 4096, m + (size_t)2 * MATCHA_N_HEAD * 4096, m + (size_t)2 * MATCHA_N_HEAD * 4096 + MATCHA_N_HEAD * 64};
}
void prep_heads_args(const matcha_tensors& p, float* folded, float* merged, float* frag, PrepArgs& a) {
  const size_t wsz = (size_t)MATCHA_N_HEAD * 64 * 64, csz = (size_t)MATCHA_N_HEAD * 64;
  a.Wq = p.w_q; a.Wk = p.w_k; a.Wv = p.w_v;
  a.gq = p.ln_q_g; a.gk = p.ln_k_g; a.gv = p.ln_v_g; a.bq = p.ln_q_b; a.bv = p.ln_v_b;
  a.fc1_w = p.fc1_w; a.fc1_b = p.fc1_b; a.p0w = p.pff0_w; a.p0b = p.pff0_b; a.p1w = p.pff1_w; a.p1b = p.pff1_b;
  a.fwq = folded; a.fwk = folded + wsz; a.fwv = folded + 2 * wsz; a.fcq = folded + 3 * wsz; a.fcv = a.fcq + 2 * csz;
  const MergedView v = merged_view(merged);
  a.B = const_cast<float*>(v.B); a.M = const_cast<float*>(v.M); a.bvec = const_cast<float*>(v.bvec); a.bdyn = const_cast<float*>(v.bdyn);
  a.frag = reinterpret_cast<u32x4*>(frag);
}
int launch_prep_heads(const matcha_tensors& p, float* folded, float* merged, float* frag, hipStream_t st) {
  PrepArgs a;
  prep_heads_args(p, folded, merged, frag, a);
  hipLaunchKernelGGL(prep_heads_kernel, dim3(kPrepGridX, kPrepGridY, kPrepGridZ), dim3(256), 0, st, a);
  MATCHA_CHECK_LAUNCH("prep_heads_kernel");
  return MATCHA_OK;
}

int launch_fused_fwd32(const matcha_tensors& p, const float* folded, const float* frag, const float* X, const Ragged& rg, int64_t B, int L, const float* y,
                       const float* w, float* Y, float* H1, float* H2, float* logits, float* row_loss, const uint64_t* seed, float p_fc1, float p_pff,
                       hipStream_t st, float* ddyn0, float* dXs, float* tslab, float alpha, float* rimg, float* tail_dh2, int objective, const int32_t* xrow,
                       const float* rn, int64_t rn_rows) {
  Fwd32Args g;
  g.xrow = xrow;
  MATCHA_CHECK_ARG(!rn || xrow, "fused forward: the r table belongs to the node route");
  g.rn = rn; g.rn_rows = (int)rn_rows;
  g.tail_dh2 = nullptr;
  g.X = X; g.row_off = rg.row_off; g.tok_slot = rg.tok_slot; g.count = rg.count; g.half_meta = rg.half_meta; g.tok_pos = rg.tok_pos;
  g.L = L;
  g.wfrag = reinterpret_cast<const u32x4*>(frag);
  (void)folded;
  g.hp = HeadParams{p.pff_ln_g, p.pff_ln_b, p.ln1_g, p.ln1_b, p.ln2_g, p.ln2_b, p.cls_w, p.cls_b};
  const bool target = objective == MATCHA_OBJECTIVE_SOFTPLUS_MSE ? y != nullptr : (y && w);
  g.objective = objective;
  g.y = y; g.w = w; g.Y = Y; g.H1 = H1; g.H2 = H2; g.logits = logits; g.row_loss = target ? row_loss : nullptr;
  g.seed = seed; g.p_fc1 = p_fc1; g.p_pff = p_pff;
  g.ddyn0 = target ? ddyn0 : nullptr; g.dXs = dXs; g.tslab = tslab; g.alpha_over_B = alpha / (float)B; g.qkv = rimg;
  size_t lds = ((size_t)2 * kHT + 64) * sizeof(float);
  auto launch = [&](auto kfn) { hipLaunchKernelGGL(kfn, dim3(rg.nhalves), dim3(64), lds, st, g); };
  ProfScope ps(MATCHA_PROF_FUSED_FWD, (double)(B * L + 1) * (MATCHA_N_HEAD * 4.0 + 2.0) * 2.0 * 64.0 * 64.0, st);
  const int ml = L <= 2 ? 2 : (L <= 6 ? L : 8);
  if (fused_small_batch(rg)) {
    MATCHA_CHECK_ARG(!xrow, "fused forward: the node route runs the large-batch kernel only");
    const size_t ldsh = ((size_t)10 * kHT + 64) * sizeof(float);
    auto launchh = [&](auto kfn) {
      (void)hipFuncSetAttribute(reinterpret_cast<const void*>(kfn), hipFuncAttributeMaxDynamicSharedMemorySize, (int)ldsh);
      hipLaunchKernelGGL(kfn, dim3(rg.nhalves), dim3(512), ldsh, st, g);
    };
    switch (ml) {
      case 2: launchh(fused_fwd32h_kernel<2>); break;
      case 3: launchh(fused_fwd32h_kernel<3>); break;
      case 4: launchh(fused_fwd32h_kernel<4>); break;
      case 5: launchh(fused_fwd32h_kernel<5>); break;
      case 6: launchh(fused_fwd32h_kernel<6>); break;
      default: launchh(fused_fwd32h_kernel<8>); break;
    }
    MATCHA_CHECK_LAUNCH("fused_fwd32h_kernel");
    return MATCHA_OK;
  }
  g.tail_dh2 = g.ddyn0 ? tail_dh2 : nullptr;
  switch (ml) {
    case 2: launch(fused_fwd32_kernel<2>); break;
    case 3: launch(fused_fwd32_kernel<3>); break;
    case 4: launch(fused_fwd32_kernel<4>); break;
    case 5: launch(fused_fwd32_kernel<5>); break;
    case 6: launch(fused_fwd32_kernel<6>); break;
    default: launch(fused_fwd32_kernel<8>); break;
  }
  MATCHA_CHECK_LAUNCH("fused_fwd32_kernel");
  return MATCHA_OK;
}

}
```

matcha_amd/csrc/kernels.hpp:

```cpp
#pragma once
#include "common.hpp"

namespace matcha {

struct GemmArgs {
  const float* A[3];
  const float* B[3];
  float* C[3];
  int64_t M, N, K;
  int64_t lda, ldb, ldc;
  int batch;
  int flags;
  const float* bias[3];
  const float* residual;
  const float* aux;
  const int64_t* row_ids;
  const uint64_t* seed;
  uint32_t stream_id;
  float p_drop;
  float aux_scale;
  const int32_t* m_dev;
  const int32_t* a_row_map;
  const int32_t* c_row_map;
  const int32_t* seg;
  int n_groups;
  int64_t b_group_stride;
  const int32_t* rng_row_map;
};

struct Ragged {
  int32_t* row_off;
  int32_t* tok_slot;
  int64_t* tok_id;
  int32_t* count;
  int32_t* blk_sum;
  int nblk;
  int ntiles;
  int32_t* tok_pos;
  int32_t* tok_key;
  int32_t* tile_meta;
  int32_t* sb_tiles;
  int32_t* sb_cnt;
  int32_t* sb_first;
  int nsb, sb_cap;
  int32_t* half_meta;
  int32_t* tok_tile;
  int32_t* sb_htiles;
  int32_t* sb_hcnt;
  int nhalves, sb_hcap;
};
size_t ragged_bytes(int64_t B, int L);
int ragged_tiles_cap(int64_t B, int L);
int ragged_halves_cap(int64_t B, int L);
void ragged_carve(int64_t B, int L, char* base, Ragged& r);
int launch_ragged_plan(const int64_t* x, int64_t B, int L, int64_t n_nodes, int32_t* status, const Ragged& r, hipStream_t st, int level = 2,
                       int64_t* node_ids = nullptr, int32_t* node_cnt = nullptr, float* node_zero = nullptr);

struct HeadParams {
  const float *gp, *bp, *g1, *b1, *g2, *b2, *wc, *bc;
};

int launch_gemm_rm(bool b_kn, const GemmArgs& g, hipStream_t st);
size_t gemm_tn_ws_bytes(int64_t M, int64_t N, int64_t R);
int launch_gemm_tn(const float* A, const float* B, float* C, float* colsum, int64_t M, int64_t N, int64_t R, int64_t lda,
                   int64_t ldb, const int64_t* b_gather, bool accumulate, void* ws, size_t ws_bytes, hipStream_t st,
                   const int32_t* r_dev = nullptr, const float* out_scale_dev = nullptr, float out_scale = 1.f);
int launch_slab_reduce(const float* slab, float* out1, int64_t n1, float* out2, int64_t stride, int P, bool accumulate, hipStream_t st,
                       const float* scale_dev = nullptr, float scale = 1.f);

struct BmmProduct {
  const float* A; int64_t a_rs, a_cs, a_hs;
  const float* B; int64_t b_rs, b_cs, b_hs;
  float* C; int64_t c_rs, c_hs;
  int accumulate;
};
bool bmm_heads_supported(int d);
int launch_bmm_heads(const BmmProduct* prods, int n, int d, hipStream_t st);

bool gemm_wide_eligible(bool b_kn, const GemmArgs& g);
int launch_gemm_wide(bool b_kn, const GemmArgs& g, hipStream_t st);
bool gemm_tn_wide_eligible(int64_t M, int64_t N, int64_t R, int64_t lda, int64_t ldb, const float* A, const float* B, const int64_t* b_gather);
size_t gemm_tn_wide_ws_bytes(int64_t M, int64_t N, int64_t R);
int launch_gemm_tn_wide(const float* A, const float* B, int64_t M, int64_t N, int64_t R, int64_t lda, int64_t ldb, bool colsum, void* ws,
                        size_t ws_bytes, const int32_t* r_dev, int* P_out, int64_t* slab_stride_out, hipStream_t st);

int launch_embed_fwd(const int64_t* x, int64_t T, int d, const float* table, const float* dense, const matcha_frozen& f,
                     int n_attr, const float* Wa, const float* ba, float* x0, hipStream_t st, const int32_t* t_dev = nullptr);
int launch_embed_scatter(const int64_t* x, int64_t T, int d, const float* dx0, float* dtable, hipStream_t st, const int32_t* t_dev = nullptr);
int launch_gather_rows(const int64_t* ids, int64_t T, int d, const float* table, int64_t n_nodes, float* rows, int32_t* status, hipStream_t st);
int launch_check_ids(const int64_t* ids, int64_t T, int64_t n_nodes, int32_t* status, hipStream_t st);
int launch_expand_embedding(const int64_t* x, int64_t B, int L, int d, const int32_t* row_off, const float* H2, const float* X, const float* gp,
                            const float* bp, float* dynamic, float* static_, hipStream_t st);

size_t table_grad_ws_bytes(int64_t n, int n_nodes);
int launch_table_grad(const int32_t* ids, const float* rows, int64_t n, int d, int n_nodes, float* dtable, void* ws, size_t ws_bytes, hipStream_t st);

struct Options {
  int disable_fused;
  int disable_merged;
  int disable_small_batch;
  int disable_wide_gemm;
  int disable_node_front;
  int disable_node_r;
  int debug_nan, fused_dbg;
};
Options& options();
int launch_fill_i32(int32_t* p, int n, int32_t v, hipStream_t st);
int zero_async(void* p, size_t bytes, hipStream_t st);
int launch_ln3_fwd(const float* X, int64_t T, int d, const float* gq, const float* bq, const float* gk, const float* bk,
                   const float* gv, const float* bv, float* qin, float* kin, float* vin, float* stats, hipStream_t st,
                   const int32_t* t_dev = nullptr);
int launch_ln3_bwd(const float* X, const float* dqin, const float* dkin, const float* dvin, const float* dXs, int64_t T, int d,
                   const float* gq, const float* gk, const float* gv, float* dZ0, float* slab, float* dgq, float* dbq,
                   float* dgk, float* dbk, float* dgv, float* dbv, hipStream_t st, const int32_t* t_dev = nullptr);
int launch_head_fwd(const int32_t* row_off, const float* H2, const float* X, int64_t B, int L, int d, const HeadParams& hp,
                    const float* y, const float* w, float* logits, float* row_loss, float* bce_out, hipStream_t st,
                    int objective = MATCHA_OBJECTIVE_BCE);
int launch_head_bwd(const int32_t* row_off, const float* H2, const float* X, int64_t B, int L, int d, const HeadParams& hp,
                    const float* y, const float* w, const float* logits, const float* dlogits, float alpha, float* dH2,
                    float* dXs, float* slab, const HeadParams& ghp, hipStream_t st, int objective = MATCHA_OBJECTIVE_BCE,
                    const int32_t* xrow = nullptr);
size_t colsum_slab_bytes(int64_t n, int nv, int d);
int launch_loss_reduce(const float* row_loss, int64_t B, float* bce_out, hipStream_t st, bool zero_recon = false,
                       float* zero_buf = nullptr, size_t zero_bytes = 0);

size_t fused_fold_floats();
size_t fused_tail_slab_floats(int64_t B, int L);
size_t fused_tail_partial_floats();
int launch_tail_reduce(const float* tslab, const Ragged& rg, int L, matcha_tensors& grads, hipStream_t st, bool halves, float* partial);
bool fused_small_batch(const Ragged& rg);

size_t fused_frag_floats();
size_t fused_tail_slab32_floats(int64_t B, int L);
size_t fused_merged_floats();
struct MergedView { const float* B; const float* M; const float* bvec; const float* bdyn; };
MergedView merged_view(const float* merged);
int launch_prep_heads(const matcha_tensors& p, float* folded, float* merged, float* frag, hipStream_t st);
int launch_fused_fwd32(const matcha_tensors& p, const float* folded, const float* frag, const float* X, const Ragged& rg, int64_t B, int L, const float* y,
                       const float* w, float* Y, float* H1, float* H2, float* logits, float* row_loss, const uint64_t* seed, float p_fc1, float p_pff,
                       hipStream_t st, float* ddyn0 = nullptr, float* dXs = nullptr, float* tslab = nullptr, float alpha = 0.f, float* rimg = nullptr,
                       float* tail_dh2 = nullptr, int objective = MATCHA_OBJECTIVE_BCE,
                       const int32_t* xrow = nullptr,
                       const float* rn = nullptr, int64_t rn_rows = 0);
size_t node_r_floats(int64_t rows);
int launch_node_r(const float* XN, const float* frag, int64_t rows, float* rn, hipStream_t st);
int tail_bwd_grid();
size_t tail_bwd_slab_floats();
int launch_tail_bwd64(const matcha_tensors& p, const float* dH2, const float* Y, const float* H1, const Ragged& rg, const uint64_t* seed, float p_fc1,
                      float p_pff, float* ddyn0, float* slab, const float* vslab, float* zero_rows, hipStream_t st,
                      const float* row_loss = nullptr, int64_t B = 0, float* losses = nullptr, bool zero_recon = false);

size_t fused_bwd_ws_floats(int64_t B, int L);
struct TailReduceArgs;
int launch_fused_bwd_merged(const matcha_tensors& p, const float* folded, const float* merged, const float* X, const float* dDyn, const float* dXs,
                            const Ragged& rg, int64_t B, int L, float* dxh, float* ws, matcha_tensors& grads, float* dZ0, hipStream_t st, const float* rimg,
                            bool dx_atomic, bool dx_zeroed = false,
                            const struct TailReduceArgs* tail = nullptr, const int32_t* xrow = nullptr, const float* xhatN = nullptr,
                            const float* rn = nullptr, int64_t rn_rows = 0);
size_t fused_qkv_floats(int64_t B, int L);
constexpr int kImgRecH = 2048 + 256;

const float* fused_bwd_dxpad(const float* ws);

bool enc128_shape(int d);
size_t enc128_ws_floats();
size_t enc128_rec_floats(const Ragged& rg);
int launch_enc128_fwd(const matcha_tensors& p, const float* lwB, const float* lwM, const float* X, const Ragged& rg, int64_t B, int L, float* Y, float* rec,
                      float* ws, const int32_t* tok_slot, const uint64_t* seed, float p_drop, hipStream_t st);
int launch_enc128_bwd(const matcha_tensors& p, const float* lwB, const float* lwM, const float* X, const float* dDyn, const float* dXs, const Ragged& rg,
                      int64_t B, int L, float* dxh, const float* rec, float* ws, float* lwdB, float* lwdM, matcha_tensors& grads, float* dZ0,
                      hipStream_t st);

bool front_bwd_supported(int d, int n_attr);
struct PrepSpec { const matcha_tensors* p; float* folded; float* merged; float* frag; };
int launch_front_fwd(const matcha_tensors& p, const int64_t* ids, const float* table, const float* dense, const matcha_frozen& f, int n_attr,
                     const Ragged& rg, int64_t tcap, float* x0, float* X, hipStream_t st, const PrepSpec* prep = nullptr,
                     const int32_t* count = nullptr);
size_t front_bwd_ws_floats();
int launch_front_bwd(const matcha_tensors& p, const float* X, const float* dxh, int nslab, int64_t tcap, const float* dxpad, const float* dXs, const float* x0,
                     const int64_t* ids, const matcha_frozen& f, int n_attr, const Ragged& rg, float* dX0, float* dtable, float* ws,
                     matcha_tensors& grads, hipStream_t st, int32_t* touched = nullptr,
                     const int32_t* node_count = nullptr);
int launch_node_xhat(const float* XN, const int32_t* node_count, int64_t rows_cap, float* xhatN, hipStream_t st);
int launch_node_scatter(const float* XN, const float* dxh, const float* dxpad, const float* dXs, const Ragged& rg, int64_t tcap, float* G, hipStream_t st);

int launch_attn_fwd(const float* Q, const float* K, const float* V, const int32_t* row_off, int64_t B, int L, int d, float* O, float* P,
                    hipStream_t st, bool shared_kv = false);
int launch_attn_bwd(const float* Q, const float* K, const float* V, const float* P, const float* dO, const int32_t* row_off, int64_t B, int L,
                    int d, float* dQ, float* dK, float* dV, float* slab, hipStream_t st, bool shared_kv = false, float* dKsum = nullptr,
                    float* dVsum = nullptr);
size_t attn_bwd_slab_bytes(int64_t B, int d);
bool attn_wide_eligible(int d);
int launch_attn_fwd_wide(const float* Q, const float* K, const float* V, const int32_t* row_off, int64_t B, int L, int d, float inv_temp, float* O,
                         float* P, int nblk, hipStream_t st, bool shared_kv = false);
int launch_attn_bwd_wide(const float* Q, const float* K, const float* V, const float* P, const float* dO, const int32_t* row_off, int64_t B, int L,
                         int d, float inv_temp, float* dQ, float* dK, float* dV, float* slab, int nblk, hipStream_t st, bool shared_kv = false,
                         float* dKs = nullptr, float* dVs = nullptr);

}
```

matcha_amd/csrc/model.hip:

```cpp
#include <stdlib.h>
#include <string.h>

#include <mutex>
#include <unordered_map>

#include "kernels.hpp"
#include "tail_reduce.hpp"

namespace matcha {

thread_local char g_err[512] = "";
void set_error(const char* fmt, ...) {
  va_list ap;
  va_start(ap, fmt);
  vsnprintf(g_err, sizeof(g_err), fmt, ap);
  va_end(ap);
}

int device_cu_count() {
  static int cache[64] = {};
  int dev = 0;
  if (hipGetDevice(&dev) != hipSuccess) { (void)hipGetLastError(); return 256; }
  if (dev >= 0 && dev < 64 && cache[dev] > 0) return cache[dev];
  int n = 0;
  if (hipDeviceGetAttribute(&n, hipDeviceAttributeMultiprocessorCount, dev) != hipSuccess || n <= 0) { (void)hipGetLastError(); return 256; }
  if (dev >= 0 && dev < 64) cache[dev] = n;
  return n;
}

int g_prof_class = 0;
static hipEvent_t* g_prof_ev = nullptr;
static int g_prof_cap = 0, g_prof_used = 0;
static double g_prof_work = 0.0;
void prof_record(bool start, double work, hipStream_t st) {
  if (start) {
    if (g_prof_used + 2 > g_prof_cap) {
      const int ncap = g_prof_cap ? 2 * g_prof_cap : 1024;
      hipEvent_t* ne = (hipEvent_t*)realloc(g_prof_ev, sizeof(hipEvent_t) * ncap);
      if (!ne) return;
      g_prof_ev = ne;
      for (int i = g_prof_cap; i < ncap; ++i)
        if (hipEventCreate(&g_prof_ev[i]) != hipSuccess) { g_prof_cap = i & ~1; return; }
      g_prof_cap = ncap;
    }
    g_prof_work += work;
    (void)hipEventRecord(g_prof_ev[g_prof_used], st);
  } else if (g_prof_used + 1 < g_prof_cap) {
    (void)hipEventRecord(g_prof_ev[g_prof_used + 1], st);
    g_prof_used += 2;
  }
}

int g_launch_log = 0;
namespace {
struct LaunchCount { const char* name; int64_t n; };
constexpr int kLaunchNames = 128;
LaunchCount g_launches[kLaunchNames];
int g_launch_names = 0;
}
void note_launch(const char* name) {
  for (int i = 0; i < g_launch_names; ++i)
    if (g_launches[i].name == name || strcmp(g_launches[i].name, name) == 0) { ++g_launches[i].n; return; }
  if (g_launch_names < kLaunchNames) g_launches[g_launch_names++] = LaunchCount{name, 1};
}

int adj_forward(const matcha_shape& s, const matcha_tensors& p, const matcha_frozen& f, const matcha_step_opts& o,
                const int64_t* x, int64_t T, float* node_out, float* recon_out, void* ws, size_t ws_bytes, hipStream_t st,
                const int32_t* t_dev, const int32_t* slot_map, float* fused_x0 = nullptr, float* fused_X = nullptr, bool save = false,
                bool fused_node = false);
int adj_backward(const matcha_shape& s, const matcha_tensors& p, const matcha_frozen& f, const matcha_step_opts& o,
                 const int64_t* x, int64_t T, float* dnode, const float* drecon, matcha_tensors& g, int32_t* touched,
                 void* ws, size_t ws_bytes, void* gemm_ws, size_t gemm_ws_bytes, hipStream_t st, const int32_t* slot_map, bool fused = false);
size_t adj_workspace_bytes(const matcha_shape& s, int64_t T);
bool adj_fused_eligible(const matcha_shape& s, const matcha_frozen& f);

struct Workspace {
  Ragged rg;
  float *x0, *X, *qin, *kin, *vin, *stats, *Q, *K, *V, *P, *O, *Y, *H1, *H2, *row_loss, *logits, *node;
  float *dH2, *dXs, *dZ1, *ddyn0, *dO, *dQ, *dK, *dV, *dqin, *dkin, *dvin, *dZ0, *dX0;
  float* slab;      size_t slab_bytes;
  float* gemm_ws;   size_t gemm_ws_bytes;
  void* adj_ws;     size_t adj_ws_bytes;
  float* folded;
  float* lwB; float* lwM; float* lwdB; float* lwdM;
  float* enc;
  float* enc_rec; size_t enc_rec_floats;
  float* merged;
  float* frag;
  float* fb_ws;
  float* tslab;
  float* tpart;
  float* tslab2;
  float* qkv;
  float* front_ws;
  void* tg_ws;      size_t tg_ws_bytes;
  float *XN, *x0N, *xhN, *GN; int64_t* node_ids; int32_t* node_cnt;
  float* RN;
  size_t total;
};

struct OptionName { const char* name; int Options::*field; };
static const OptionName kOptionNames[] = {
    {"disable_fused", &Options::disable_fused}, {"disable_merged", &Options::disable_merged}, {"disable_small_batch", &Options::disable_small_batch},
    {"disable_wide_gemm", &Options::disable_wide_gemm}, {"disable_node_front", &Options::disable_node_front}, {"disable_node_r", &Options::disable_node_r}, {"debug_nan", &Options::debug_nan}, {"fused_dbg", &Options::fused_dbg}};
Options& options() {
  static Options o = [] {
    Options v;
    memset(&v, 0, sizeof(v));
    for (const OptionName& n : kOptionNames) {
      char env[64] = "MATCHA_";
      size_t k = strlen(env);
      for (const char* c = n.name; *c && k + 1 < sizeof(env); ++c) env[k++] = (char)((*c >= 'a' && *c <= 'z') ? *c - 32 : *c);
      env[k] = 0;
      const char* e = getenv(env);
      if (e) v.*(n.field) = (*e == 0) ? 1 : atoi(e);
      if (e && v.*(n.field) == 0 && strcmp(e, "0") != 0) v.*(n.field) = 1;
    }
    return v;
  }();
  return o;
}
static bool merged_layerwise_shape(const matcha_shape& s) { return s.d >= 128 && s.d % 64 == 0; }
static bool merged_layerwise(const matcha_shape& s) { return merged_layerwise_shape(s) && attn_wide_eligible(s.d) && !options().disable_merged; }
static bool enc128_enabled(const matcha_shape& s, const matcha_step_opts& o) {
  return enc128_shape(s.d) && merged_layerwise(s) && options().disable_fused != 1 && !o.deterministic && !o.sparse_table_grad;
}
static bool fused_enabled(const matcha_shape& s) { return s.d == 64 && options().disable_fused != 1 && !options().disable_merged; }
static bool fused_front_enabled() { return (options().disable_fused & 2) == 0; }
static bool node_front_shape(const matcha_shape& s, int64_t B, int L) {
  return s.mode == 0 && s.d == 64 && front_bwd_supported(s.d, s.n_attr) && B * L + 1 >= 4 * ((int64_t)s.n_nodes + 1);
}
static bool has_target(int objective, const float* y, const float* w) { return objective == MATCHA_OBJECTIVE_SOFTPLUS_MSE ? y != nullptr : (y && w); }
static bool loss_in_forward(const matcha_shape& s, const matcha_step_opts& o, const float* y, const float* w, int objective) {
  return o.loss_in_forward && !o.forward_only && has_target(objective, y, w) && fused_enabled(s);
}
static int check_objective(int32_t objective, const char* fn) {
  if (objective == MATCHA_OBJECTIVE_BCE || objective == MATCHA_OBJECTIVE_SOFTPLUS_MSE) return MATCHA_OK;
  set_error("%s: unknown objective %d (MATCHA_OBJECTIVE_BCE or MATCHA_OBJECTIVE_SOFTPLUS_MSE)", fn, (int)objective);
  return MATCHA_EINVAL;
}
static std::mutex g_fwd_mu;
static std::unordered_map<const void*, std::pair<int, uint64_t>> g_fwd_state;
static uint64_t g_fwd_clock = 0;
static void note_forward(const void* ws, bool merged, bool fused, bool enc = false, bool split_tail = false, bool dx_zeroed = false, bool node = false, bool node_r = false) {
  std::lock_guard<std::mutex> lk(g_fwd_mu);
  if (g_fwd_state.size() >= 4096 && g_fwd_state.find(ws) == g_fwd_state.end()) {
    auto old = g_fwd_state.begin();
    for (auto it = g_fwd_state.begin(); it != g_fwd_state.end(); ++it)
      if (it->second.second < old->second.second) old = it;
    g_fwd_state.erase(old);
  }
  g_fwd_state[ws] = std::make_pair((merged ? 1 : 0) | (fused ? 2 : 0) | (enc ? 4 : 0) | (split_tail ? 8 : 0) | (dx_zeroed ? 16 : 0) | (node ? 32 : 0) | (node_r ? 64 : 0), ++g_fwd_clock);
}
static int ws_state(const void* ws) {
  std::lock_guard<std::mutex> lk(g_fwd_mu);
  auto it = g_fwd_state.find(ws);
  return it != g_fwd_state.end() ? it->second.first : -1;
}
static void forget_forward(const void* ws) {
  std::lock_guard<std::mutex> lk(g_fwd_mu);
  g_fwd_state.erase(ws);
}

static int merged_weights(const matcha_shape& s, const matcha_tensors& p, Workspace& w, hipStream_t st) {
  const int64_t d = s.d, hd = (int64_t)MATCHA_N_HEAD * d;
  const BmmProduct pr[2] = {
      {p.w_k, 1, d, d * d, p.w_q, d, 1, d * d, w.lwB, d, d * d, 0},
      {p.fc1_w, hd, 1, d, p.w_v, d, 1, d * d, w.lwM, hd, d, 0}};
  return launch_bmm_heads(pr, 2, s.d, st);
}
static int merged_chain(const matcha_shape& s, const matcha_tensors& p, matcha_tensors& g_, Workspace& w, hipStream_t st) {
  const int64_t d = s.d, hd = (int64_t)MATCHA_N_HEAD * d;
  const BmmProduct pr[4] = {
      {p.w_k, d, 1, d * d, w.lwdB, d, 1, d * d, g_.w_q, d, d * d, 1},
      {p.w_q, d, 1, d * d, w.lwdB, 1, d, d * d, g_.w_k, d, d * d, 1},
      {w.lwdM, hd, 1, d, p.w_v, 1, d, d * d, g_.fc1_w, hd, d, 1},
      {p.fc1_w, 1, hd, d, w.lwdM, hd, 1, d, g_.w_v, d, d * d, 1}};
  return launch_bmm_heads(pr, 4, s.d, st);
}

static size_t carve(const matcha_shape& s, int64_t B, int L, char* base, Workspace& w, bool compact = false) {
  const int64_t Tn = B * L + 1, d = s.d, hd = (int64_t)MATCHA_N_HEAD * d;
  size_t off = 0;
  auto take_always = [&](size_t n_floats) {
    float* p = base ? (float*)(base + off) : nullptr;
    off += align_up(n_floats * sizeof(float), 256);
    return p;
  };
  auto take = [&](size_t n_floats) { return compact ? (float*)nullptr : take_always(n_floats); };
  {
    const size_t rb = ragged_bytes(B, L);
    if (base) ragged_carve(B, L, base + off, w.rg);
    off += align_up(rb, 256);
  }
  w.x0 = take_always(Tn * d); w.X = take_always(Tn * d);
  w.qin = take(Tn * d); w.kin = take(Tn * d); w.vin = take(Tn * d);
  w.stats = take(Tn * 2);
  w.Q = take(Tn * hd); w.K = take(Tn * hd); w.V = take(Tn * hd);
  w.P = take(B * MATCHA_N_HEAD * L * L);
  w.O = take(Tn * hd);
  w.Y = take(Tn * d); w.H1 = take(Tn * d); w.H2 = take(Tn * d);
  w.row_loss = take_always(B); w.logits = take_always(B);
  w.node = take_always(s.mode == 1 ? Tn * d : 0);
  w.dH2 = take(Tn * d); w.dXs = take(Tn * d); w.dZ1 = take(Tn * d); w.ddyn0 = take(Tn * d);
  w.dO = w.O; w.dQ = w.K; w.dK = w.Q; w.dV = w.V;
  w.dqin = w.qin; w.dkin = w.kin; w.dvin = w.vin;
  w.dZ0 = take(Tn * d); w.dX0 = take(Tn * d);
  size_t sb = colsum_slab_bytes(Tn, 6, (int)d);
  size_t sb2 = colsum_slab_bytes(B, 7, (int)d);
  if (sb2 > sb) sb = sb2;
  sb2 = attn_bwd_slab_bytes(B, (int)d);
  if (sb2 > sb) sb = sb2;
  w.slab_bytes = sb; w.slab = take(sb / sizeof(float));
  size_t gb = gemm_tn_ws_bytes(hd, d, Tn);
  size_t g2 = gemm_tn_ws_bytes(d, hd, Tn); if (g2 > gb) gb = g2;
  g2 = gemm_tn_ws_bytes(d, d, Tn); if (g2 > gb) gb = g2;
  g2 = gemm_tn_ws_bytes(d, s.n_attr, Tn); if (g2 > gb) gb = g2;
  if (s.mode == 1) {
    for (int64_t m = 64;; m += 64) {
      const int64_t mm = m < s.max_bins ? m : s.max_bins;
      g2 = gemm_tn_ws_bytes(mm, d, Tn); if (g2 > gb) gb = g2;
      if (mm >= s.max_bins) break;
    }
  }
  w.gemm_ws_bytes = gb; w.gemm_ws = take(gb / sizeof(float));
  w.adj_ws_bytes = (s.mode == 1) ? adj_workspace_bytes(s, Tn) : 0;
  w.adj_ws = take_always(w.adj_ws_bytes / sizeof(float));
  w.folded = take_always(s.d == 64 ? fused_fold_floats() : 0);
  w.frag = take_always(s.d == 64 ? fused_frag_floats() : 0);
  w.merged = take_always(s.d == 64 ? fused_merged_floats() : 0);
  {
    const size_t nm = merged_layerwise_shape(s) ? (size_t)hd * d : 0;
    w.lwB = take_always(nm); w.lwM = take_always(nm);
    w.lwdB = take(nm); w.lwdM = take(nm);
  }
  w.enc = take_always(enc128_shape((int)d) ? enc128_ws_floats() : 0);
  w.enc_rec = w.Q;
  w.enc_rec_floats = (w.Q && w.O) ? (size_t)((w.O + Tn * hd) - w.Q) : 0;
  w.fb_ws = take(s.d == 64 ? fused_bwd_ws_floats(B, L) : 0);
  w.tpart = take(s.d == 64 ? fused_tail_partial_floats() : 0);
  w.tslab = take(s.d == 64 ? fused_tail_slab32_floats(B, L) : 0);
  w.tslab2 = take(s.d == 64 ? tail_bwd_slab_floats() : 0);
  w.qkv = take(s.d == 64 ? fused_qkv_floats(B, L) : 0);
  w.front_ws = take(front_bwd_supported(s.d, s.n_attr) ? front_bwd_ws_floats() : 0);
  w.tg_ws_bytes = (s.mode == 0 && !compact) ? table_grad_ws_bytes(Tn, s.n_nodes) : 0;
  w.tg_ws = take(w.tg_ws_bytes / sizeof(float));
  {
    const size_t nn = node_front_shape(s, B, L) ? (size_t)(s.n_nodes + 1) : 0;
    w.XN = take_always(nn * 64); w.x0N = take(nn * 64); w.xhN = take(nn * 64); w.GN = take(nn * 64);
    w.node_ids = reinterpret_cast<int64_t*>(take_always(nn * 2));
    w.node_cnt = reinterpret_cast<int32_t*>(take_always(nn ? 64 : 0));
    w.RN = nn ? (compact ? take_always(node_r_floats((int64_t)nn)) : w.Q) : nullptr;
  }
  w.total = off;
  return off;
}

static int table_gradient(const matcha_shape& s, const matcha_step_opts& o, const Workspace& w, int64_t Tn, matcha_tensors& g, hipStream_t st) {
  if (o.sparse_table_grad) return MATCHA_OK;
  if (!o.deterministic) return MATCHA_OK;
  return launch_table_grad(w.rg.tok_key, w.dX0, Tn, s.d, s.n_nodes, g.table, w.tg_ws, w.tg_ws_bytes, st);
}

static int encoder_done(const matcha_step_opts& o, hipStream_t st) {
  if (o.encoder_done_event && hipEventRecord((hipEvent_t)o.encoder_done_event, st) != hipSuccess) {
    set_error("matcha_backward: recording encoder_done_event failed"); return MATCHA_EHIP;
  }
  return MATCHA_OK;
}

static int check_shape(const matcha_shape* s, int64_t B, int32_t L) {
  MATCHA_CHECK_ARG(s, "null shape");
  MATCHA_CHECK_ARG(s->d >= 8 && s->d <= 256 && s->d % 8 == 0 && (s->d <= 64 || s->d % 64 == 0),
                   "embed_dim d=%d unsupported (multiples of 8 up to 64, then 128, 192, 256)", s->d);
  MATCHA_CHECK_ARG(s->d % 4 == 0, "d must be a multiple of 4");
  MATCHA_CHECK_ARG(L >= 1 && L <= MATCHA_MAX_L, "L=%d outside 1..%d", L, MATCHA_MAX_L);
  MATCHA_CHECK_ARG(B >= 1 && B * (int64_t)L < (1ll << 31) - 2, "B=%lld must be >= 1 and B*L < 2^31", (long long)B);
  MATCHA_CHECK_ARG(s->d == 64 || B * (int64_t)L + 1 <= 65535ll * 128, "B*L=%lld exceeds the %lld token rows the layer-by-layer kernels (embed_dim != 64) launch",
                   (long long)(B * (int64_t)L), 65535ll * 128);
  MATCHA_CHECK_ARG(s->n_nodes >= 1, "n_nodes=%d must be >= 1", s->n_nodes);
  MATCHA_CHECK_ARG(s->mode == 0 || s->mode == 1, "mode=%d must be 0 (table) or 1 (adj)", s->mode);
  MATCHA_CHECK_ARG(s->n_attr >= 1 && (size_t)s->n_attr * s->d * 4 <= 160 * 1024, "n_attr=%d does not fit the LDS staging", s->n_attr);
  return MATCHA_OK;
}

static GemmArgs gemm1(const Workspace& w, const float* A, const float* B, float* C, int64_t M, int64_t N, int64_t K, bool b_kn) {
  GemmArgs g;
  memset(&g, 0, sizeof(g));
  g.A[0] = A; g.B[0] = B; g.C[0] = C; g.batch = 1;
  g.M = M; g.N = N; g.K = K; g.lda = K; g.ldb = b_kn ? N : K; g.ldc = N;
  g.aux_scale = 1.f;
  g.m_dev = w.rg.count;
  g.rng_row_map = w.rg.tok_slot;
  return g;
}

__global__ void nan_count_kernel(const float* __restrict__ p, const int32_t* __restrict__ rows_dev, int64_t rows, int64_t width, int* __restrict__ out) {
  if (rows_dev) rows = *rows_dev;
  int bad = 0;
  for (int64_t i = (int64_t)blockIdx.x * blockDim.x + threadIdx.x; i < rows * width; i += (int64_t)gridDim.x * blockDim.x)
    bad += isfinite(p[i]) ? 0 : 1;
  if (bad) atomicAdd(out, bad);
}
static void nan_check(const char* name, const float* p, const int32_t* rows_dev, int64_t rows, int64_t width, hipStream_t st) {
  if (!options().debug_nan || !p) return;
  int* d = nullptr;
  int h = 0;
  if (hipMalloc(&d, sizeof(int)) != hipSuccess) return;
  (void)hipMemsetAsync(d, 0, sizeof(int), st);
  hipLaunchKernelGGL(nan_count_kernel, dim3(256), dim3(256), 0, st, p, rows_dev, rows, width, d);
  (void)hipMemcpyAsync(&h, d, sizeof(int), hipMemcpyDeviceToHost, st);
  (void)hipStreamSynchronize(st);
  (void)hipFree(d);
  fprintf(stderr, "[matcha nan-check] %-10s %d non-finite values in the valid rows\n", name, h);
}

}

using namespace matcha;

extern "C" int matcha_abi_version(void) { return MATCHA_ABI_VERSION; }
extern "C" const char* matcha_last_error(void) { return g_err; }
extern "C" int matcha_device_count(void) {
  int n = 0;
  if (hipGetDeviceCount(&n) != hipSuccess) { (void)hipGetLastError(); return 0; }
  return n;
}

extern "C" int matcha_profile_select(int32_t kernel_class) {
  g_prof_class = kernel_class;
  g_prof_used = 0;
  g_prof_work = 0.0;
  return MATCHA_OK;
}

extern "C" int matcha_launch_log(int32_t on) {
  if (on) g_launch_names = 0;
  g_launch_log = on ? 1 : 0;
  return MATCHA_OK;
}

extern "C" int matcha_launch_log_read(char* out, size_t cap) {
  MATCHA_CHECK_ARG(out && cap > 0, "matcha_launch_log_read: null buffer");
  size_t n = 0;
  out[0] = 0;
  for (int i = 0; i < g_launch_names; ++i) {
    const int k = snprintf(out + n, cap - n, "%s %lld\n", g_launches[i].name, (long long)g_launches[i].n);
    if (k < 0 || (size_t)k >= cap - n) { set_error("matcha_launch_log_read: buffer too small"); return MATCHA_ENOMEM; }
    n += (size_t)k;
  }
  return MATCHA_OK;
}

extern "C" int matcha_profile_read(double* total_ms, int64_t* launches, double* work) {
  double ms = 0.0;
  for (int i = 0; i + 1 < g_prof_used; i += 2) {
    if (hipEventSynchronize(g_prof_ev[i + 1]) != hipSuccess) { set_error("matcha_profile_read: event sync failed"); return MATCHA_EHIP; }
    float t = 0.f;
    if (hipEventElapsedTime(&t, g_prof_ev[i], g_prof_ev[i + 1]) != hipSuccess) { set_error("matcha_profile_read: elapsed failed"); return MATCHA_EHIP; }
    ms += t;
  }
  if (total_ms) *total_ms = ms;
  if (launches) *launches = g_prof_used / 2;
  if (work) *work = g_prof_work;
  g_prof_used = 0;
  g_prof_work = 0.0;
  return MATCHA_OK;
}

extern "C" size_t matcha_workspace_bytes(const matcha_shape* shp, int64_t B, int32_t L) {
  if (check_shape(shp, B, L) != MATCHA_OK) return 0;
  Workspace w;
  return carve(*shp, B, L, nullptr, w);
}

static bool compact_forward(const matcha_shape& s, const matcha_step_opts& o) { return o.forward_only && fused_enabled(s); }
extern "C" size_t matcha_workspace_bytes_forward(const matcha_shape* shp, int64_t B, int32_t L) {
  if (check_shape(shp, B, L) != MATCHA_OK) return 0;
  Workspace w;
  return carve(*shp, B, L, nullptr, w, fused_enabled(*shp));
}

static int forward_impl(const matcha_shape* shp, const matcha_tensors* params, const matcha_frozen* frozen,
                        const matcha_step_opts* opts, const int64_t* x, int64_t B, int32_t L, const float* y,
                        const float* w_bce, float* logits, float* losses, void* ws, size_t ws_bytes,
                        matcha_stream_t stream, bool force_layerwise, bool stop_before_head, int objective) {
  MATCHA_TRY(check_shape(shp, B, L));
  MATCHA_CHECK_ARG(params && frozen && opts && x && ws, "matcha_forward: null pointer");
  MATCHA_CHECK_ARG(((uintptr_t)ws) % 256 == 0, "matcha_forward: workspace must be 256-byte aligned");
  const matcha_shape& s = *shp;
  const matcha_tensors& p = *params;
  hipStream_t st = (hipStream_t)stream;
  Workspace w;
  const size_t need = carve(s, B, L, (char*)ws, w, !force_layerwise && compact_forward(s, *opts));
  if (ws_bytes < need) { set_error("matcha_forward: workspace %zu < %zu bytes", ws_bytes, need); return MATCHA_ENOMEM; }
  const int64_t Tn = B * L + 1;
  const int d = s.d;
  const int64_t hd = (int64_t)MATCHA_N_HEAD * d;
  const bool train = opts->training != 0;
  MATCHA_CHECK_ARG(!train || opts->seed || (opts->p_drop_adj <= 0 && opts->p_drop_fc1 <= 0 && opts->p_drop_pff <= 0),
                   "matcha_forward: training with dropout needs opts->seed");
  MATCHA_CHECK_ARG((frozen->attr_table || frozen->attr_mode == 1) && p.attr_w && p.attr_b && p.next_w && p.next_b && p.w_q && p.w_k && p.w_v && p.fc1_w &&
                       p.fc1_b && p.pff0_w && p.pff0_b && p.pff1_w && p.pff1_b && p.pff_ln_g && p.pff_ln_b && p.ln1_g && p.ln1_b &&
                       p.ln2_g && p.ln2_b && p.cls_w && p.cls_b && p.ln_q_g && p.ln_q_b && p.ln_k_g && p.ln_k_b && p.ln_v_g && p.ln_v_b,
                   "matcha_forward: a parameter pointer is null");
  const int32_t* cnt = w.rg.count;
  const int64_t* ids = w.rg.tok_id;

  const bool fused_path = !force_layerwise && fused_enabled(s);
  const bool tgt = has_target(objective, y, w_bce);
  const bool lif = fused_path && loss_in_forward(s, *opts, y, w_bce, objective);
  const bool keep_rimg = !opts->forward_only;
  const bool enc = !force_layerwise && enc128_enabled(s, *opts) && (opts->forward_only || enc128_rec_floats(w.rg) <= w.enc_rec_floats);
  const int plan_level = (fused_enabled(s) || enc) ? 1 : 0;
  const bool front = !force_layerwise && fused_enabled(s) && front_bwd_supported(s.d, s.n_attr) && fused_front_enabled();
  const bool node = front && fused_path && node_front_shape(s, B, L) && !fused_small_batch(w.rg) && !opts->deterministic && !opts->sparse_table_grad &&
                    !options().disable_node_front;
  const bool node_r = node && !options().disable_node_r;
  MATCHA_TRY(launch_ragged_plan(x, B, L, s.n_nodes, opts->status, w.rg, st, plan_level, node ? w.node_ids : nullptr, node ? w.node_cnt : nullptr,
                                (node && !opts->forward_only) ? w.GN : nullptr));
  float* recon_out = losses ? losses + 1 : nullptr;
  const bool recon_zero_in_loss = s.mode == 0 && recon_out && fused_path && tgt && losses;
  const bool adj_fused = front && fused_path && s.mode == 1 && adj_fused_eligible(s, *frozen);
  if (s.mode == 0) {
    MATCHA_CHECK_ARG(p.table, "matcha_forward: table mode without table");
    if (recon_out && !recon_zero_in_loss) MATCHA_TRY(zero_async(recon_out, 2 * sizeof(float), st));
  } else if (adj_fused) {
    MATCHA_TRY(adj_forward(s, p, *frozen, *opts, ids, Tn, nullptr, recon_out, w.adj_ws, w.adj_ws_bytes, st, cnt, w.rg.tok_slot,
                           opts->forward_only ? nullptr : w.x0, w.X, !opts->forward_only));
  } else {
    MATCHA_TRY(adj_forward(s, p, *frozen, *opts, ids, Tn, w.node, recon_out, w.adj_ws, w.adj_ws_bytes, st, cnt, w.rg.tok_slot));
  }
  bool prep_in_front = false;
  if (adj_fused) {
  } else if (front) {
    const PrepSpec prep = {&p, w.folded, w.merged, w.frag};
    prep_in_front = fused_path;
    if (node) {
      MATCHA_TRY(launch_front_fwd(p, w.node_ids, p.table, nullptr, *frozen, s.n_attr, w.rg, (int64_t)s.n_nodes + 1, opts->forward_only ? nullptr : w.x0N, w.XN, st,
                                  prep_in_front ? &prep : nullptr, w.node_cnt));
      if (!opts->forward_only) MATCHA_TRY(launch_node_xhat(w.XN, w.node_cnt, (int64_t)s.n_nodes + 1, w.xhN, st));
      if (node_r) MATCHA_TRY(launch_node_r(w.XN, w.frag, (int64_t)s.n_nodes + 1, w.RN, st));
    } else
    MATCHA_TRY(launch_front_fwd(p, ids, s.mode == 0 ? p.table : nullptr, s.mode == 0 ? nullptr : w.node, *frozen, s.n_attr, w.rg, Tn,
                                opts->forward_only ? nullptr : w.x0, w.X, st, prep_in_front ? &prep : nullptr));
  } else {
    MATCHA_TRY(launch_embed_fwd(ids, Tn, d, s.mode == 0 ? p.table : nullptr, s.mode == 0 ? nullptr : w.node, *frozen, s.n_attr, p.attr_w,
                                p.attr_b, w.x0, st, cnt));
    GemmArgs g = gemm1(w, w.x0, p.next_w, w.X, Tn, d, d, false);
    g.flags = MATCHA_EPI_BIAS | MATCHA_EPI_TANH; g.bias[0] = p.next_b;
    MATCHA_TRY(launch_gemm_rm(false, g, st));
  }
  if (fused_path) {
    const bool save = !opts->forward_only && !lif;
    if (!prep_in_front) MATCHA_TRY(launch_prep_heads(p, w.folded, w.merged, w.frag, st));
    float* lg_out = (logits && !save) ? logits : w.logits;
    const bool split_tail = lif && !fused_small_batch(w.rg) && (options().fused_dbg & 1) == 0;
    const bool zero_dx = lif && !opts->deterministic && !opts->sparse_table_grad && (split_tail || fused_small_batch(w.rg)) && tgt && losses;
    if (opts->forward_only) forget_forward(ws); else note_forward(ws, true, true, false, split_tail, zero_dx, node, node_r);
    MATCHA_TRY(launch_fused_fwd32(p, w.folded, w.frag, node ? w.XN : w.X, w.rg, B, L, y, w_bce, (save || lif) ? w.Y : nullptr, (save || lif) ? w.H1 : nullptr, (save || lif) ? w.H2 : nullptr,
                                  lg_out, w.row_loss, opts->seed, train ? opts->p_drop_fc1 : 0.f, train ? opts->p_drop_pff : 0.f, st,
                                  lif ? w.ddyn0 : nullptr, w.dXs, w.tslab, opts->alpha, keep_rimg ? w.qkv : nullptr, split_tail ? w.dH2 : nullptr, objective,
                                  node ? w.rg.tok_key : nullptr, node_r ? w.RN : nullptr, (int64_t)s.n_nodes + 1));
    if (split_tail)
      MATCHA_TRY(launch_tail_bwd64(p, w.dH2, w.Y, w.H1, w.rg, opts->seed, train ? opts->p_drop_fc1 : 0.f, train ? opts->p_drop_pff : 0.f, w.ddyn0, w.tslab2, w.tslab,
                                   zero_dx ? w.dO : nullptr, st, w.row_loss, B, tgt ? losses : nullptr, recon_zero_in_loss));
    const bool zero_in_loss = zero_dx && !split_tail;
    if (tgt && losses && !split_tail)
      MATCHA_TRY(launch_loss_reduce(w.row_loss, B, losses, st, recon_zero_in_loss, zero_in_loss ? w.dO : nullptr, zero_in_loss ? (size_t)Tn * 64 * sizeof(float) : 0));
    if (logits && lg_out != logits && hipMemcpyAsync(logits, w.logits, B * sizeof(float), hipMemcpyDeviceToDevice, st) != hipSuccess) {
      set_error("logits copy failed"); return MATCHA_EHIP;
    }
    return MATCHA_OK;
  }
  nan_check("x0", w.x0, cnt, 0, d, st);
  nan_check("X", w.X, cnt, 0, d, st);
  const bool mlw = merged_layerwise(s);
  if (opts->forward_only) forget_forward(ws); else note_forward(ws, mlw, false, enc);
  if (enc) {
    MATCHA_TRY(merged_weights(s, p, w, st));
    const bool keep = !opts->forward_only;
    if (keep && enc128_rec_floats(w.rg) > w.enc_rec_floats) { set_error("matcha_forward: the fused d = 128 records do not fit the workspace"); return MATCHA_ENOMEM; }
    MATCHA_TRY(launch_enc128_fwd(p, w.lwB, w.lwM, w.X, w.rg, B, L, w.Y, keep ? w.enc_rec : nullptr, w.enc, w.rg.tok_slot, opts->seed,
                                 (train && opts->p_drop_fc1 > 0.f) ? opts->p_drop_fc1 : 0.f, st));
  } else {
  MATCHA_TRY(launch_ln3_fwd(w.X, Tn, d, p.ln_q_g, p.ln_q_b, p.ln_k_g, p.ln_k_b, p.ln_v_g, p.ln_v_b, w.qin, w.kin, w.vin, w.stats, st, cnt));
  if (mlw) {
    MATCHA_TRY(merged_weights(s, p, w, st));
    GemmArgs g = gemm1(w, w.qin, w.lwB, w.Q, Tn, hd, d, false);
    MATCHA_TRY(launch_gemm_rm(false, g, st));
  } else {
    GemmArgs g = gemm1(w, w.qin, p.w_q, w.Q, Tn, hd, d, false);
    g.A[1] = w.kin; g.B[1] = p.w_k; g.C[1] = w.K;
    g.A[2] = w.vin; g.B[2] = p.w_v; g.C[2] = w.V;
    g.batch = 3;
    MATCHA_TRY(launch_gemm_rm(false, g, st));
  }
  nan_check("qin", w.qin, cnt, 0, d, st);
  nan_check("Q", w.Q, cnt, 0, hd, st);
  nan_check("K", w.K, cnt, 0, hd, st);
  nan_check("V", w.V, cnt, 0, hd, st);
  if (mlw) MATCHA_TRY(launch_attn_fwd(w.Q, w.kin, w.vin, w.rg.row_off, B, L, d, w.O, w.P, st, true));
  else MATCHA_TRY(launch_attn_fwd(w.Q, w.K, w.V, w.rg.row_off, B, L, d, w.O, w.P, st));
  nan_check("O", w.O, cnt + 1, 0, hd, st);
  {
    GemmArgs g = gemm1(w, w.O, mlw ? w.lwM : p.fc1_w, w.Y, Tn, d, hd, false);
    g.flags = MATCHA_EPI_BIAS | MATCHA_EPI_ROWMASK; g.bias[0] = p.fc1_b; g.row_ids = ids;
    if (train && opts->p_drop_fc1 > 0.f) { g.flags |= MATCHA_EPI_DROPOUT; g.seed = opts->seed; g.stream_id = kStreamDropFc1; g.p_drop = opts->p_drop_fc1; }
    MATCHA_TRY(launch_gemm_rm(false, g, st));
  }
  }
  {
    GemmArgs g = gemm1(w, w.Y, p.pff0_w, w.H1, Tn, d, d, false);
    g.flags = MATCHA_EPI_BIAS | MATCHA_EPI_TANH; g.bias[0] = p.pff0_b;
    if (train && opts->p_drop_pff > 0.f) { g.flags |= MATCHA_EPI_DROPOUT; g.seed = opts->seed; g.stream_id = kStreamDropPff; g.p_drop = opts->p_drop_pff; }
    MATCHA_TRY(launch_gemm_rm(false, g, st));
  }
  {
    GemmArgs g = gemm1(w, w.H1, p.pff1_w, w.H2, Tn, d, d, false);
    g.flags = MATCHA_EPI_BIAS | MATCHA_EPI_RESIDUAL; g.bias[0] = p.pff1_b; g.residual = w.Y;
    MATCHA_TRY(launch_gemm_rm(false, g, st));
  }
  nan_check("Y", w.Y, cnt, 0, d, st);
  nan_check("H1", w.H1, cnt, 0, d, st);
  nan_check("H2", w.H2, cnt, 0, d, st);
  if (stop_before_head) return MATCHA_OK;
  HeadParams hp = {p.pff_ln_g, p.pff_ln_b, p.ln1_g, p.ln1_b, p.ln2_g, p.ln2_b, p.cls_w, p.cls_b};
  MATCHA_TRY(launch_head_fwd(w.rg.row_off, w.H2, w.X, B, L, d, hp, y, w_bce, w.logits, w.row_loss, losses, st, objective));
  if (logits && hipMemcpyAsync(logits, w.logits, B * sizeof(float), hipMemcpyDeviceToDevice, st) != hipSuccess) {
    set_error("logits copy failed"); return MATCHA_EHIP;
  }
  return MATCHA_OK;
}

extern "C" int matcha_forward(const matcha_shape* shp, const matcha_tensors* params, const matcha_frozen* frozen,
                              const matcha_step_opts* opts, const int64_t* x, int64_t B, int32_t L, const float* y,
                              const float* w_bce, float* logits, float* losses, void* ws, size_t ws_bytes,
                              matcha_stream_t stream) {
  return forward_impl(shp, params, frozen, opts, x, B, L, y, w_bce, logits, losses, ws, ws_bytes, stream, false, false, MATCHA_OBJECTIVE_BCE);
}

extern "C" int matcha_forward_objective(int32_t objective, const matcha_shape* shp, const matcha_tensors* params, const matcha_frozen* frozen,
                                        const matcha_step_opts* opts, const int64_t* x, int64_t B, int32_t L, const float* y,
                                        const float* w, float* logits, float* losses, void* ws, size_t ws_bytes, matcha_stream_t stream) {
  MATCHA_TRY(check_objective(objective, "matcha_forward_objective"));
  return forward_impl(shp, params, frozen, opts, x, B, L, y, w, logits, losses, ws, ws_bytes, stream, false, false, objective);
}

extern "C" int matcha_get_embedding(const matcha_shape* shp, const matcha_tensors* params, const matcha_frozen* frozen,
                                    const matcha_step_opts* opts, const int64_t* x, int64_t B, int32_t L, float* dynamic,
                                    float* static_, float* attn, float* losses, void* ws, size_t ws_bytes, matcha_stream_t stream) {
  MATCHA_CHECK_ARG(dynamic && static_ && opts, "matcha_get_embedding: null pointer");
  matcha_step_opts o = *opts;
  o.forward_only = 0;
  o.loss_in_forward = 0;
  MATCHA_TRY(forward_impl(shp, params, frozen, &o, x, B, L, nullptr, nullptr, nullptr, losses, ws, ws_bytes, stream, true, true, MATCHA_OBJECTIVE_BCE));
  Workspace w;
  carve(*shp, B, L, (char*)ws, w);
  if (attn && hipMemcpyAsync(attn, w.P, (size_t)B * MATCHA_N_HEAD * L * L * sizeof(float), hipMemcpyDeviceToDevice, (hipStream_t)stream) != hipSuccess) {
    set_error("matcha_get_embedding: attention copy failed"); return MATCHA_EHIP;
  }
  return launch_expand_embedding(x, B, L, shp->d, w.rg.row_off, w.H2, w.X, params->pff_ln_g, params->pff_ln_b, dynamic, static_, (hipStream_t)stream);
}

extern "C" int matcha_debug_layout(const matcha_shape* shp, int64_t B, int32_t L, char* out, size_t cap) {
  MATCHA_TRY(check_shape(shp, B, L));
  MATCHA_CHECK_ARG(out && cap > 0, "matcha_debug_layout: null buffer");
  Workspace w;
  char* const base = reinterpret_cast<char*>((uintptr_t)1 << 20);
  const size_t total = carve(*shp, B, L, base, w);
  struct { const char* name; const void* p; } f[] = {
      {"plan", w.rg.row_off}, {"x0", w.x0}, {"X", w.X}, {"qin", w.qin}, {"kin", w.kin}, {"vin", w.vin}, {"stats", w.stats}, {"Q", w.Q}, {"K", w.K}, {"V", w.V},
      {"P", w.P}, {"O_dxh", w.O}, {"Y", w.Y}, {"H1", w.H1}, {"H2", w.H2}, {"row_loss", w.row_loss}, {"logits", w.logits}, {"node", w.node}, {"dH2", w.dH2},
      {"dXs", w.dXs}, {"dZ1", w.dZ1}, {"ddyn0", w.ddyn0}, {"dZ0", w.dZ0}, {"dX0", w.dX0}, {"slab", w.slab}, {"gemm_ws", w.gemm_ws}, {"adj_ws", w.adj_ws},
      {"folded", w.folded}, {"frag", w.frag}, {"merged", w.merged}, {"lwB", w.lwB}, {"lwM", w.lwM}, {"lwdB", w.lwdB}, {"lwdM", w.lwdM}, {"enc", w.enc}, {"fb_ws", w.fb_ws},
      {"tpart", w.tpart}, {"tslab", w.tslab}, {"tslab2", w.tslab2}, {"qkv_records", w.qkv}, {"front_ws", w.front_ws}, {"tg_ws", w.tg_ws}, {"XN", w.XN}, {"x0N", w.x0N}, {"xhN", w.xhN}, {"GN", w.GN},
      {"node_ids", w.node_ids}, {"node_cnt", w.node_cnt}, {"RN", w.RN}};
  size_t n = 0;
  for (const auto& e : f) {
    if (!e.p) continue;
    const int k = snprintf(out + n, cap - n, "%s %zu\n", e.name, (size_t)((const char*)e.p - base));
    if (k < 0 || (size_t)k >= cap - n) { set_error("matcha_debug_layout: buffer too small"); return MATCHA_ENOMEM; }
    n += (size_t)k;
  }
  const int k = snprintf(out + n, cap - n, "end %zu\n", total);
  if (k < 0 || (size_t)k >= cap - n) { set_error("matcha_debug_layout: buffer too small"); return MATCHA_ENOMEM; }
  return MATCHA_OK;
}

extern "C" int matcha_random_chrom_dev_supported(const matcha_shape* shp, const matcha_frozen* frozen) {
  if (!shp || !frozen) return 0;
  if (shp->mode == 0) return 1;
  return adj_fused_eligible(*shp, *frozen) && fused_enabled(*shp) && front_bwd_supported(shp->d, shp->n_attr) ? 1 : 0;
}

extern "C" int matcha_set_option(const char* name, int32_t value) {
  MATCHA_CHECK_ARG(name, "matcha_set_option: null name");
  for (const OptionName& n : kOptionNames)
    if (strcmp(n.name, name) == 0) { options().*(n.field) = value; return MATCHA_OK; }
  set_error("matcha_set_option: unknown option '%s'", name);
  return MATCHA_EINVAL;
}

extern "C" int32_t matcha_get_option(const char* name) {
  if (!name) return -1;
  for (const OptionName& n : kOptionNames)
    if (strcmp(n.name, name) == 0) return options().*(n.field);
  return -1;
}

extern "C" int matcha_table_grad_rows(const matcha_shape* shp, int64_t B, int32_t L, void* ws, size_t ws_bytes,
                                      const int32_t** ids, const float** rows, const int32_t** n_tokens, int64_t* cap) {
  MATCHA_TRY(check_shape(shp, B, L));
  MATCHA_CHECK_ARG(ws && ids && rows && cap, "matcha_table_grad_rows: null pointer");
  MATCHA_CHECK_ARG(shp->mode == 0, "matcha_table_grad_rows: table mode only");
  Workspace w;
  const size_t need = carve(*shp, B, L, (char*)ws, w);
  if (ws_bytes < need) { set_error("matcha_table_grad_rows: workspace %zu < %zu bytes", ws_bytes, need); return MATCHA_ENOMEM; }
  *ids = w.rg.tok_key;
  *rows = w.dX0;
  if (n_tokens) *n_tokens = w.rg.count + 1;
  *cap = B * (int64_t)L + 1;
  return MATCHA_OK;
}

static int backward_impl(const matcha_shape* shp, const matcha_tensors* params, const matcha_frozen* frozen,
                         const matcha_step_opts* opts, const int64_t* x, int64_t B, int32_t L, const float* y,
                         const float* w_bce, const float* dlogits, const float* drecon, matcha_tensors* grads,
                         int32_t* touched, void* ws, size_t ws_bytes, matcha_stream_t stream, int objective) {
  MATCHA_TRY(check_shape(shp, B, L));
  MATCHA_CHECK_ARG(params && frozen && opts && x && ws && grads, "matcha_backward: null pointer");
  MATCHA_CHECK_ARG(dlogits || has_target(objective, y, w_bce),
                   objective == MATCHA_OBJECTIVE_BCE ? "matcha_backward: need dlogits or (y, w)" : "matcha_backward: need dlogits or y");
  const matcha_shape& s = *shp;
  const matcha_tensors& p = *params;
  matcha_tensors& g_ = *grads;
  hipStream_t st = (hipStream_t)stream;
  Workspace w;
  const size_t need = carve(s, B, L, (char*)ws, w);
  if (ws_bytes < need) { set_error("matcha_backward: workspace %zu < %zu bytes", ws_bytes, need); return MATCHA_ENOMEM; }
  const int64_t Tn = B * L + 1;
  const int d = s.d;
  const int64_t hd = (int64_t)MATCHA_N_HEAD * d;
  const bool train = opts->training != 0;
  const bool drop_fc1 = train && opts->p_drop_fc1 > 0.f, drop_pff = train && opts->p_drop_pff > 0.f;
  const int32_t* cnt = w.rg.count;
  const int64_t* ids = w.rg.tok_id;

  const int fwd_state = ws_state(ws);
  MATCHA_CHECK_ARG(fwd_state >= 0, "matcha_backward: no matcha_forward on record for this workspace (one backward per forward, same ws pointer)");
  const bool fused_fwd = (fwd_state & 2) != 0;
  const bool lif = fused_fwd && loss_in_forward(s, *opts, y, w_bce, objective);
  MATCHA_CHECK_ARG(!(lif && dlogits), "matcha_backward: opts->loss_in_forward excludes an explicit dlogits");
  forget_forward(ws);
  bool dx_zeroed = false, tail_in_bwd = false;
  TailReduceArgs tail_args;
  const bool node = fused_fwd && (fwd_state & 32) != 0;
  const bool node_r = node && (fwd_state & 64) != 0;
  if (lif) {
    const bool small = fused_small_batch(w.rg);
    dx_zeroed = (fwd_state & 16) != 0 && !opts->deterministic && !opts->sparse_table_grad;
    if ((fwd_state & 8) != 0) {
      tail_reduce_args(w.tslab2, w.rg, L, g_, true, tail_bwd_grid(), true, tail_args);
      tail_in_bwd = true;
    } else if (small) {
      tail_reduce_args(w.tslab, w.rg, L, g_, true, -1, false, tail_args);
      tail_in_bwd = true;
    } else
      MATCHA_TRY(launch_tail_reduce(w.tslab, w.rg, L, g_, st, true, w.tpart));
  } else {
  HeadParams hp = {p.pff_ln_g, p.pff_ln_b, p.ln1_g, p.ln1_b, p.ln2_g, p.ln2_b, p.cls_w, p.cls_b};
  HeadParams ghp = {g_.pff_ln_g, g_.pff_ln_b, g_.ln1_g, g_.ln1_b, g_.ln2_g, g_.ln2_b, g_.cls_w, g_.cls_b};
  MATCHA_TRY(launch_head_bwd(w.rg.row_off, w.H2, node ? w.XN : w.X, B, L, d, hp, y, w_bce, w.logits, dlogits, opts->alpha, w.dH2, w.dXs, w.slab, ghp, st, objective,
                             node ? w.rg.tok_key : nullptr));
  MATCHA_TRY(launch_gemm_tn(w.dH2, w.H1, g_.pff1_w, g_.pff1_b, d, d, Tn, d, d, nullptr, true, w.gemm_ws, w.gemm_ws_bytes, st, cnt));
  {
    GemmArgs g = gemm1(w, w.dH2, p.pff1_w, w.dZ1, Tn, d, d, true);
    g.flags = MATCHA_EPI_DTANH; g.aux = w.H1;
    if (drop_pff) { g.flags |= MATCHA_EPI_DROPOUT; g.seed = opts->seed; g.stream_id = kStreamDropPff; g.p_drop = opts->p_drop_pff; g.aux_scale = 1.f - opts->p_drop_pff; }
    MATCHA_TRY(launch_gemm_rm(true, g, st));
  }
  MATCHA_TRY(launch_gemm_tn(w.dZ1, w.Y, g_.pff0_w, g_.pff0_b, d, d, Tn, d, d, nullptr, true, w.gemm_ws, w.gemm_ws_bytes, st, cnt));
  {
    GemmArgs g = gemm1(w, w.dZ1, p.pff0_w, w.ddyn0, Tn, d, d, true);
    g.flags = MATCHA_EPI_RESIDUAL | MATCHA_EPI_ROWMASK; g.residual = w.dH2; g.row_ids = ids;
    if (drop_fc1) { g.flags |= MATCHA_EPI_DROPOUT; g.seed = opts->seed; g.stream_id = kStreamDropFc1; g.p_drop = opts->p_drop_fc1; }
    MATCHA_TRY(launch_gemm_rm(true, g, st));
  }
  }
  if (fused_fwd) {
    const bool front = node || (front_bwd_supported(s.d, s.n_attr) && fused_front_enabled());
    const bool dx_atomic = !opts->deterministic && !opts->sparse_table_grad;
    MATCHA_CHECK_ARG(!node || dx_atomic, "matcha_backward: deterministic / sparse_table_grad differ from the forward's on this workspace");
    MATCHA_TRY(launch_fused_bwd_merged(p, w.folded, w.merged, node ? w.XN : w.X, w.ddyn0, w.dXs, w.rg, B, L, w.dO, w.fb_ws, g_, front ? nullptr : w.dZ0, st, w.qkv, dx_atomic, dx_zeroed,
                                       tail_in_bwd ? &tail_args : nullptr, node ? w.rg.tok_key : nullptr, node ? w.xhN : nullptr,
                                       node_r ? w.RN : nullptr, (int64_t)s.n_nodes + 1));
    MATCHA_TRY(encoder_done(*opts, st));
    if (front) {
      if (s.mode == 0) MATCHA_CHECK_ARG(g_.table, "matcha_backward: table mode without a table gradient buffer");
      if (node) {
        MATCHA_TRY(launch_node_scatter(w.XN, w.dO, fused_bwd_dxpad(w.fb_ws), w.dXs, w.rg, Tn, w.GN, st));
        MATCHA_TRY(launch_front_bwd(p, w.XN, nullptr, 1, (int64_t)s.n_nodes + 1, fused_bwd_dxpad(w.fb_ws), w.GN, w.x0N, w.node_ids, *frozen, s.n_attr, w.rg,
                                    nullptr, g_.table, w.front_ws, g_, st, touched, w.node_cnt));
        return MATCHA_OK;
      }
      const bool rows_out = s.mode == 1 || opts->deterministic || opts->sparse_table_grad;
      MATCHA_TRY(launch_front_bwd(p, w.X, w.dO, dx_atomic ? 1 : MATCHA_N_HEAD, Tn, fused_bwd_dxpad(w.fb_ws), w.dXs, w.x0, ids, *frozen, s.n_attr, w.rg,
                                  rows_out ? w.dX0 : nullptr, rows_out ? nullptr : g_.table, w.front_ws, g_, st, s.mode == 0 ? touched : nullptr));
      if (s.mode == 0) {
        MATCHA_TRY(table_gradient(s, *opts, w, Tn, g_, st));
      } else {
        MATCHA_TRY(adj_backward(s, p, *frozen, *opts, ids, Tn, w.dX0, drecon, g_, touched, w.adj_ws, w.adj_ws_bytes, w.gemm_ws, w.gemm_ws_bytes, st,
                                w.rg.tok_slot, adj_fused_eligible(s, *frozen)));
      }
      return MATCHA_OK;
    }
  } else {
  if ((fwd_state & 4) != 0) {
    MATCHA_TRY(launch_enc128_bwd(p, w.lwB, w.lwM, w.X, w.ddyn0, w.dXs, w.rg, B, L, w.dqin, w.enc_rec, w.enc, w.lwdB, w.lwdM, g_, w.dZ0, st));
    MATCHA_TRY(merged_chain(s, p, g_, w, st));
    MATCHA_TRY(encoder_done(*opts, st));
  } else {
  if ((fwd_state & 1) != 0) {
    MATCHA_TRY(zero_async(w.lwdM, (size_t)hd * d * sizeof(float), st));
    MATCHA_TRY(zero_async(w.lwdB, (size_t)hd * d * sizeof(float), st));
    MATCHA_TRY(launch_gemm_tn(w.ddyn0, w.O, w.lwdM, g_.fc1_b, d, hd, Tn, d, hd, nullptr, true, w.gemm_ws, w.gemm_ws_bytes, st, cnt));
    {
      GemmArgs g = gemm1(w, w.ddyn0, w.lwM, w.dO, Tn, hd, d, true);
      MATCHA_TRY(launch_gemm_rm(true, g, st));
    }
    MATCHA_TRY(launch_attn_bwd(w.Q, w.kin, w.vin, w.P, w.dO, w.rg.row_off, B, L, d, w.dQ, w.dK, w.dV, w.slab, st, true, w.dkin, w.dvin));
    MATCHA_TRY(launch_gemm_tn(w.dQ, w.qin, w.lwdB, nullptr, hd, d, Tn, hd, d, nullptr, true, w.gemm_ws, w.gemm_ws_bytes, st, cnt));
    {
      GemmArgs g = gemm1(w, w.dQ, w.lwB, w.dqin, Tn, d, hd, true);
      MATCHA_TRY(launch_gemm_rm(true, g, st));
    }
    MATCHA_TRY(merged_chain(s, p, g_, w, st));
  } else {
  MATCHA_TRY(launch_gemm_tn(w.ddyn0, w.O, g_.fc1_w, g_.fc1_b, d, hd, Tn, d, hd, nullptr, true, w.gemm_ws, w.gemm_ws_bytes, st, cnt));
  {
    GemmArgs g = gemm1(w, w.ddyn0, p.fc1_w, w.dO, Tn, hd, d, true);
    MATCHA_TRY(launch_gemm_rm(true, g, st));
  }
  MATCHA_TRY(launch_attn_bwd(w.Q, w.K, w.V, w.P, w.dO, w.rg.row_off, B, L, d, w.dQ, w.dK, w.dV, w.slab, st));
  MATCHA_TRY(launch_gemm_tn(w.dQ, w.qin, g_.w_q, nullptr, hd, d, Tn, hd, d, nullptr, true, w.gemm_ws, w.gemm_ws_bytes, st, cnt));
  MATCHA_TRY(launch_gemm_tn(w.dK, w.kin, g_.w_k, nullptr, hd, d, Tn, hd, d, nullptr, true, w.gemm_ws, w.gemm_ws_bytes, st, cnt));
  MATCHA_TRY(launch_gemm_tn(w.dV, w.vin, g_.w_v, nullptr, hd, d, Tn, hd, d, nullptr, true, w.gemm_ws, w.gemm_ws_bytes, st, cnt));
  {
    GemmArgs g = gemm1(w, w.dQ, p.w_q, w.dqin, Tn, d, hd, true);
    g.A[1] = w.dK; g.B[1] = p.w_k; g.C[1] = w.dkin;
    g.A[2] = w.dV; g.B[2] = p.w_v; g.C[2] = w.dvin;
    g.batch = 3;
    MATCHA_TRY(launch_gemm_rm(true, g, st));
  }
  }
  MATCHA_TRY(launch_ln3_bwd(w.X, w.dqin, w.dkin, w.dvin, w.dXs, Tn, d, p.ln_q_g, p.ln_k_g, p.ln_v_g, w.dZ0, w.slab, g_.ln_q_g,
                            g_.ln_q_b, g_.ln_k_g, g_.ln_k_b, g_.ln_v_g, g_.ln_v_b, st, cnt));
  MATCHA_TRY(encoder_done(*opts, st));
  }
  }
  MATCHA_TRY(launch_gemm_tn(w.dZ0, w.x0, g_.next_w, g_.next_b, d, d, Tn, d, d, nullptr, true, w.gemm_ws, w.gemm_ws_bytes, st, cnt));
  {
    GemmArgs g = gemm1(w, w.dZ0, p.next_w, w.dX0, Tn, d, d, true);
    MATCHA_TRY(launch_gemm_rm(true, g, st));
  }
  MATCHA_CHECK_ARG(frozen->attr_table, "matcha_backward: the layer-by-layer attribute_nn backward gathers attr_table rows (also under attr_mode 1)");
  MATCHA_TRY(launch_gemm_tn(w.dX0, frozen->attr_table, g_.attr_w, g_.attr_b, d, s.n_attr, Tn, d, frozen->attr_ld > 0 ? frozen->attr_ld : s.n_attr, ids, true,
                            w.gemm_ws, w.gemm_ws_bytes, st, cnt));
  if (s.mode == 0) {
    MATCHA_CHECK_ARG(g_.table, "matcha_backward: table mode without a table gradient buffer");
    if (opts->deterministic || opts->sparse_table_grad) MATCHA_TRY(table_gradient(s, *opts, w, Tn, g_, st));
    else MATCHA_TRY(launch_embed_scatter(ids, Tn, d, w.dX0, g_.table, st, cnt));
    if (touched) MATCHA_TRY(launch_fill_i32(touched, 2, 1, st));
  } else {
    MATCHA_TRY(adj_backward(s, p, *frozen, *opts, ids, Tn, w.dX0, drecon, g_, touched, w.adj_ws, w.adj_ws_bytes, w.gemm_ws, w.gemm_ws_bytes, st,
                            w.rg.tok_slot));
  }
  return MATCHA_OK;
}

extern "C" int matcha_backward(const matcha_shape* shp, const matcha_tensors* params, const matcha_frozen* frozen,
                               const matcha_step_opts* opts, const int64_t* x, int64_t B, int32_t L, const float* y,
                               const float* w_bce, const float* dlogits, const float* drecon, matcha_tensors* grads,
                               int32_t* touched, void* ws, size_t ws_bytes, matcha_stream_t stream) {
  return backward_impl(shp, params, frozen, opts, x, B, L, y, w_bce, dlogits, drecon, grads, touched, ws, ws_bytes, stream, MATCHA_OBJECTIVE_BCE);
}

extern "C" int matcha_backward_objective(int32_t objective, const matcha_shape* shp, const matcha_tensors* params, const matcha_frozen* frozen,
                                         const matcha_step_opts* opts, const int64_t* x, int64_t B, int32_t L, const float* y,
                                         const float* w, const float* dlogits, const float* drecon, matcha_tensors* grads,
                                         int32_t* touched, void* ws, size_t ws_bytes, matcha_stream_t stream) {
  MATCHA_TRY(check_objective(objective, "matcha_backward_objective"));
  return backward_impl(shp, params, frozen, opts, x, B, L, y, w, dlogits, drecon, grads, touched, ws, ws_bytes, stream, objective);
}

extern "C" int matcha_node_embeddings(const matcha_shape* shp, const matcha_tensors* params, const matcha_frozen* frozen,
                                      const int64_t* ids, int64_t T, float* rows, void* ws, size_t ws_bytes,
                                      int32_t* status, matcha_stream_t stream) {
  MATCHA_CHECK_ARG(shp && params && frozen && ids && rows, "matcha_node_embeddings: null pointer");
  MATCHA_CHECK_ARG(shp->d >= 4 && shp->d <= 256 && shp->d % 4 == 0, "matcha_node_embeddings: d=%d", shp->d);
  hipStream_t st = (hipStream_t)stream;
  if (shp->mode == 0) {
    MATCHA_CHECK_ARG(params->table, "matcha_node_embeddings: null table");
    return launch_gather_rows(ids, T, shp->d, params->table, shp->n_nodes, rows, status, st);
  }
  MATCHA_TRY(launch_check_ids(ids, T, shp->n_nodes, status, st));
  matcha_step_opts o;
  memset(&o, 0, sizeof(o));
  o.random_chrom = -1;
  MATCHA_CHECK_ARG(ws && ws_bytes >= adj_workspace_bytes(*shp, T), "matcha_node_embeddings: adj mode needs a workspace of matcha_workspace_bytes()");
  return adj_forward(*shp, *params, *frozen, o, ids, T, rows, nullptr, ws, ws_bytes, st, nullptr, nullptr, nullptr, nullptr, false, true);
}
```

Measured before the change: 54.74 million hyperedges/s.

## Precompute per-node value table and use it in fused attention backward

Adds a node-route variant of the fused backward kernel (VTAB) that reads precomputed per-node, per-head value projections (VN), produced by the forward node_r launch. This replaces the per-tile dDyn-by-M fragment MMA and the padded-row value contribution with table lookups. The M-weight gradient is folded into an extra MMA over the staged value-gradient fragments plus a rank-one pad correction at the end. It trades extra forward work and memory (the VN table carved from the Q buffer) for less matrix work per tile in backward. It is gated to shapes where total tokens greatly exceed node count.

```diff
diff --git a/matcha_amd/csrc/fused_bwd.hip b/matcha_amd/csrc/fused_bwd.hip
--- a/matcha_amd/csrc/fused_bwd.hip
+++ b/matcha_amd/csrc/fused_bwd.hip
@@ -80,6 +80,76 @@
     const float ns = -sig;
     axpy8(a, ns, o);
     gq = scale8(inv_temp, a);
+  }
+  {
+    int ad = li * kLd + 8 * sub;
+    FB_PIN(ad, gq);
+    const V8 q = ld8(&Qs[ad]);
+    axpy8(accK, dspf, q);
+  }
+  if (sub == 1) {
+    float* dst = dSs + li * 8;
+    *reinterpret_cast<float4*>(dst) = make_float4(ds[0], ds[1 % ML], ML > 2 ? ds[2 % ML] : 0.f, ML > 3 ? ds[3 % ML] : 0.f);
+    if (ML > 4) *reinterpret_cast<float4*>(dst + 4) = make_float4(ds[4 % ML], ML > 5 ? ds[5 % ML] : 0.f, ML > 6 ? ds[6 % ML] : 0.f, ML > 7 ? ds[7 % ML] : 0.f);
+  }
+}
+
+#define FB_PIN1(addr, s) asm volatile("" : "+v"(addr), "+v"(s))
+template <int ML>
+__device__ __forceinline__ void attn_row8_v(const float* __restrict__ Qs, const float* __restrict__ Xs, const float* __restrict__ Ys, const float* __restrict__ Ds,
+                                            const float* __restrict__ xpad, const float* __restrict__ ypad, const float* __restrict__ Ps, float* __restrict__ dSs,
+                                            int li, int li0, int k, int n_pad, int sub, float inv_temp, V8& gq, V8& accK, V8& accU) {
+  const float padf = (float)n_pad;
+  const bool hp = n_pad > 0;
+  float p[ML], ds[ML], pp;
+  {
+    const float4 pa = *reinterpret_cast<const float4*>(&Ps[li * 8]), pb = *reinterpret_cast<const float4*>(&Ps[li * 8 + 4]);
+    const float w[8] = {pa.x, pa.y, pa.z, pa.w, pb.x, pb.y, pb.z, pb.w};
+#pragma unroll
+    for (int j = 0; j < ML; ++j) p[j] = (j < k) ? w[j] : 0.f;
+    pp = hp ? w[7] : 0.f;
+  }
+  const float ppf = padf * pp;
+  const int ro0 = li0 * kLd + 8 * sub;
+  const V8 go = ld8(&Ds[li * kLd + 8 * sub]);
+  const float dsp_raw = group_sum8_dpp(dot8(go, ld8(ypad + 8 * sub)));
+  float sig = ppf * dsp_raw;
+  {
+    V8 vn = ld8(&Ys[ro0]), vn2 = ld8(&Ys[ro0 + (1 < k ? 1 : 0) * kLd]);
+    float part = 0.f;
+#pragma unroll
+    for (int j = 0; j < ML; ++j) {
+      const V8 v = vn;
+      vn = vn2;
+      if (j + 2 < ML) {
+        int ad = ro0 + (j + 2 < k ? j + 2 : 0) * kLd;
+        FB_PIN1(ad, part);
+        vn2 = ld8(&Ys[ad]);
+      }
+      part = dot8(go, v);
+      const float d = group_sum8_dpp(part);
+      ds[j] = d;
+      sig += p[j] * d;
+    }
+  }
+#pragma unroll
+  for (int j = 0; j < ML; ++j) ds[j] = p[j] * (ds[j] - sig) * inv_temp;
+  const float dspf = padf * (pp * (dsp_raw - sig) * inv_temp);
+  axpy8(accU, ppf, go);
+  gq = scale8(dspf, ld8(xpad + 8 * sub));
+  {
+    V8 vn = ld8(&Xs[ro0]), vn2 = ld8(&Xs[ro0 + (1 < k ? 1 : 0) * kLd]);
+#pragma unroll
+    for (int j = 0; j < ML; ++j) {
+      const V8 v = vn;
+      vn = vn2;
+      if (j + 2 < ML) {
+        int ad = ro0 + (j + 2 < k ? j + 2 : 0) * kLd;
+        FB_PIN(ad, gq);
+        vn2 = ld8(&Xs[ad]);
+      }
+      axpy8(gq, ds[j], v);
+    }
   }
   {
     int ad = li * kLd + 8 * sub;
@@ -147,11 +217,13 @@
   const float* rimg;
   const int32_t* xrow;
   const float* rn; int64_t rn_head;
+  const float* vn;
 };
 constexpr size_t kBwdLdsBytes = (size_t)2 * kTileH * 4 + (size_t)4 * kPT * 2 + (64 + 256 + 256 + 32) * 4;
 
-template <int ML, bool NODE>
+template <int ML, bool NODE, bool VTAB = false>
 __global__ __launch_bounds__(256) __attribute__((amdgpu_waves_per_eu(2, 2))) void fused_bwdh_kernel(FusedBwdHArgs g) {
+  static_assert(NODE || !VTAB, "the value table belongs to the node route");
   extern __shared__ __attribute__((aligned(16))) float lds[];
   float* Xs = lds;
   float* Gs = lds + kTileH;
@@ -161,6 +233,8 @@
   short* FBp = RBp + kPT;
   float* Rs = reinterpret_cast<float*>(RBp);
   float* Fs = reinterpret_cast<float*>(FBp);
+  float* Ds = reinterpret_cast<float*>(Dp);
+  float* ypad = Ds + kTileH;
   float* sm = reinterpret_cast<float*>(FBp + kPT);
   float* xpad = sm;
   float* dSs = xpad + 64;
@@ -202,6 +276,10 @@
       ln_row16(xv, m, rs);
       *reinterpret_cast<float4*>(&xpad[sc4]) = make_float4((xv.x - m) * rs, (xv.y - m) * rs, (xv.z - m) * rs, (xv.w - m) * rs);
     }
+  }
+  if constexpr (VTAB) {
+    static_assert((size_t)(kTileH + 64) * 4 <= (size_t)kPT * 2, "dDyn rows + y_pad fit the Dp region");
+    if (tid >= 64 && tid < 80) *reinterpret_cast<float4*>(&ypad[sc4]) = *reinterpret_cast<const float4*>(g.vn + (int64_t)head * g.rn_head + sc4);
   }
 
   f32x4 ab0 = {0.f, 0.f, 0.f, 0.f}, ab1 = ab0, ab2 = ab0, ab3 = ab0, am0 = ab0, am1 = ab0, am2 = ab0, am3 = ab0;
@@ -221,7 +299,7 @@
     const int row__ = srow + 16 * (I);                                                                   \
     kx##I = g.xrow[(M).x + (row__ < (M).y ? row__ : ((M).y > 0 ? (M).y - 1 : 0))];                       \
   } while (0)
-  f32x4 ri0, ri1, pn = {0.f, 0.f, 0.f, 0.f};
+  f32x4 ri0, ri1, yi0, yi1, pn = {0.f, 0.f, 0.f, 0.f};
 #define FBH_ROW_GLOAD(I, M)                                                                              \
   do {                                                                                                   \
     const int row__ = srow + 16 * (I);                                                                   \
@@ -234,11 +312,15 @@
     FBH_ROW_GLOAD(0, M); FBH_ROW_GLOAD(1, M);                                                            \
     if (tid < 32) tpn = g.tok_pos[(M).x + (tid < (M).y ? tid : ((M).y > 0 ? (M).y - 1 : 0))];           \
   } while (0)
-  const bool r_tab = NODE && g.rn != nullptr;
+  const bool r_tab = VTAB || (NODE && g.rn != nullptr);
 #define FBH_R_GLOAD()                                                                                    \
   do {                                                                                                   \
     const float* rh__ = g.rn + (int64_t)head * g.rn_head + sc4;                                          \
     ri0 = *reinterpret_cast<const f32x4*>(rh__ + (int64_t)kx0 * 64); ri1 = *reinterpret_cast<const f32x4*>(rh__ + (int64_t)kx1 * 64); \
+    if constexpr (VTAB) {                                                                                \
+      const float* vh__ = g.vn + (int64_t)head * g.rn_head + sc4;                                        \
+      yi0 = *reinterpret_cast<const f32x4*>(vh__ + (int64_t)kx0 * 64); yi1 = *reinterpret_cast<const f32x4*>(vh__ + (int64_t)kx1 * 64); \
+    }                                                                                                    \
   } while (0)
 #define FBH_ROW_STAGE(I)                                                                                 \
   do {                                                                                                   \
@@ -263,7 +345,9 @@
       *reinterpret_cast<u32x2*>(d__ + 2 * kPlane) = (u32x2){p0__.l, p1__.l};                             \
     }                                                                                                    \
     const float4 dm__ = make_float4(dv__.x * msk__, dv__.y * msk__, dv__.z * msk__, dv__.w * msk__);     \
-    {                                                                                                    \
+    if constexpr (VTAB) {                                                                                \
+      *reinterpret_cast<float4*>(&Ds[row__ * kLd + sc4]) = dm__;                                         \
+    } else {                                                                                             \
       const P3 p0__ = split2(dm__.x, dm__.y), p1__ = split2(dm__.z, dm__.w);                             \
       short* d__ = Dp + row__ * kPS + sc4;                                                               \
       *reinterpret_cast<u32x2*>(d__) = (u32x2){p0__.h, p1__.h}; *reinterpret_cast<u32x2*>(d__ + kPlane) = (u32x2){p0__.m, p1__.m}; \
@@ -303,6 +387,9 @@
     {
       FBH_ROW_STAGE(0); FBH_ROW_STAGE(1);
       if (tid < 32) tinfo[tid] = tid < n_real ? ((tid - (tpn & 255)) | (tpn & ~255)) : 0;
+      if constexpr (VTAB) {
+        *reinterpret_cast<f32x4*>(&Fs[srow * kLd + sc4]) = yi0; *reinterpret_cast<f32x4*>(&Fs[(srow + 16) * kLd + sc4]) = yi1;
+      }
       if (r_tab) {
         *reinterpret_cast<f32x4*>(&Rs[srow * kLd + sc4]) = ri0; *reinterpret_cast<f32x4*>(&Rs[(srow + 16) * kLd + sc4]) = ri1;
       } else {
@@ -320,7 +407,7 @@
     const int srow = tid_ >> 4, sc4 = (tid_ & 15) * 4;
     const int sub = lane & 7;
     (void)srow; (void)sc4;
-    {
+    if constexpr (!VTAB) {
       f32x4 acc0 = {0.f, 0.f, 0.f, 0.f}, acc1 = acc0;
       const short* dp = Dp + c16 * kPS + 8 * kq;
 #pragma unroll
@@ -330,11 +417,35 @@
       }
       *reinterpret_cast<f32x4*>(&Fs[c16 * kLd + fb + 4 * kq]) = acc0;
       *reinterpret_cast<f32x4*>(&Fs[(16 + c16) * kLd + fb + 4 * kq]) = acc1;
-    }
-    FB_T(1);
-    __syncthreads();
-    FB_T(7);
-    {
+      FB_T(1);
+      __syncthreads();
+      FB_T(7);
+    }
+    if constexpr (VTAB) {
+      FB_T(1);
+      V8 q0, k0, v0;
+      const int la = wave * 8 + (lane >> 3);
+      const bool acta = la < n_real;
+      int ia = 0;
+      if (acta) { ia = tinfo[la]; attn_row8_v<ML>(Rs, Xs, Fs, Ds, xpad, ypad, Ps, dSs, la, ia & 255, ia >> 8, g.L - (ia >> 8), sub, inv_temp, q0, accK, accV); }
+      __builtin_amdgcn_sched_barrier(0);
+      FB_T(2);
+      __syncthreads();
+      FB_T(7);
+      if (acta) {
+        attn_col8<ML>(Rs, Ds, Ps, dSs, la, ia & 255, ia >> 8, sub, k0, v0);
+        st8(&Gs[la * kLd + 8 * sub], k0);
+      } else {
+        ZR8(&Gs[la * kLd + 8 * sub]);
+        v0 = zero8(); q0 = zero8();
+      }
+      frag_store(FBp + la * kPS + 8 * sub, split8(v0));
+      FB_T(3);
+      __syncthreads();
+      FB_T(7);
+      frag_store(RBp + la * kPS + 8 * sub, split8(q0));
+      accR.a += q0.a; accR.b += q0.b; accR.c += q0.c; accR.d += q0.d;
+    } else {
       V8 o0, q0, k0, v0;
       const int la = wave * 8 + (lane >> 3);
       const bool acta = la < n_real;
@@ -374,6 +485,14 @@
         const Frag3 a0 = frag_row(arow + 32 * s), a1 = frag_row(arow + 16 * kPS + 32 * s);
         dx0 = mma6(dx0, a0, Bf[s]); dx1 = mma6(dx1, a1, Bf[s]);
       }
+      if constexpr (VTAB) {
+        const short* urow = FBp + c16 * kPS + 8 * kq;
+#pragma unroll
+        for (int s = 0; s < 2; ++s) {
+          const Frag3 a0 = frag_row(urow + 32 * s), a1 = frag_row(urow + 16 * kPS + 32 * s);
+          dx0 = mma6(dx0, a0, Mf[s]); dx1 = mma6(dx1, a1, Mf[s]);
+        }
+      }
       float* out = g.dxh + ((int64_t)t0 + 4 * kq) * 64 + fb + c16;
 #pragma unroll
       for (int reg = 0; reg < 4; ++reg) {
@@ -389,6 +508,14 @@
         const Frag3 a0 = frag_row(arow + 32 * s), a1 = frag_row(arow + 16 * kPS + 32 * s);
         dx0 = mma6(dx0, Bf[s], a0); dx1 = mma6(dx1, Bf[s], a1);
       }
+      if constexpr (VTAB) {
+        const short* urow = FBp + c16 * kPS + 8 * kq;
+#pragma unroll
+        for (int s = 0; s < 2; ++s) {
+          const Frag3 a0 = frag_row(urow + 32 * s), a1 = frag_row(urow + 16 * kPS + 32 * s);
+          dx0 = mma6(dx0, Mf[s], a0); dx1 = mma6(dx1, Mf[s], a1);
+        }
+      }
       float* out = g.dxh + ((int64_t)head * g.tcap + t0 + c16) * 64 + fb + 4 * kq;
       if (c16 < n_real) *reinterpret_cast<f32x4*>(out) = dx0;
       if (16 + c16 < n_real) *reinterpret_cast<f32x4*>(out + 16 * 64) = dx1;
@@ -397,14 +524,21 @@
     if (tile + 1 < tile_hi) FBH_RIMG_GLOAD(tile + 1);
     {
       const int blk = ((4 * kq + ((lane & 15) >> 2)) * kPS) + 4 * (lane & 3);
-      const Frag3 xb = frag_col(Xp + blk + fb), zb = frag_col(FBp + blk + fb);
+      const Frag3 xb = frag_col(Xp + blk + fb);
+      Frag3 zb;
+      if constexpr (!VTAB) zb = frag_col(FBp + blk + fb);
       {
         const Frag3 r0 = frag_col(RBp + blk), r1 = frag_col(RBp + blk + 16);
         ab0 = mma6(ab0, r0, xb); ab1 = mma6(ab1, r1, xb);
         const Frag3 r2 = frag_col(RBp + blk + 32), r3 = frag_col(RBp + blk + 48);
         ab2 = mma6(ab2, r2, xb); ab3 = mma6(ab3, r3, xb);
       }
-      {
+      if constexpr (VTAB) {
+        const Frag3 u0 = frag_col(FBp + blk), u1 = frag_col(FBp + blk + 16);
+        am0 = mma6(am0, u0, xb); am1 = mma6(am1, u1, xb);
+        const Frag3 u2 = frag_col(FBp + blk + 32), u3 = frag_col(FBp + blk + 48);
+        am2 = mma6(am2, u2, xb); am3 = mma6(am3, u3, xb);
+      } else {
         const Frag3 d0 = frag_col(Dp + blk), d1 = frag_col(Dp + blk + 16);
         am0 = mma6(am0, d0, zb); am1 = mma6(am1, d1, zb);
         const Frag3 d2 = frag_col(Dp + blk + 32), d3 = frag_col(Dp + blk + 48);
@@ -429,8 +563,10 @@
       const int row = 4 * kq + reg;
       slab[0 * 4096 + row * 64 + col] = ab0[reg]; slab[0 * 4096 + (row + 16) * 64 + col] = ab1[reg];
       slab[0 * 4096 + (row + 32) * 64 + col] = ab2[reg]; slab[0 * 4096 + (row + 48) * 64 + col] = ab3[reg];
-      slab[1 * 4096 + row * 64 + col] = am0[reg]; slab[1 * 4096 + (row + 16) * 64 + col] = am1[reg];
-      slab[1 * 4096 + (row + 32) * 64 + col] = am2[reg]; slab[1 * 4096 + (row + 48) * 64 + col] = am3[reg];
+      if constexpr (!VTAB) {
+        slab[1 * 4096 + row * 64 + col] = am0[reg]; slab[1 * 4096 + (row + 16) * 64 + col] = am1[reg];
+        slab[1 * 4096 + (row + 32) * 64 + col] = am2[reg]; slab[1 * 4096 + (row + 48) * 64 + col] = am3[reg];
+      }
     }
   }
   float* redd = lds;
@@ -446,6 +582,20 @@
   }
   float* redr = lds + 4 * 64;
   float* redp = lds + 8 * 64;
+  float* redu = lds + 12 * 64;
+  float* upad = lds + 16 * 64;
+  if constexpr (VTAB) {
+    const float accu[8] = {accV.a.x, accV.a.y, accV.b.x, accV.b.y, accV.c.x, accV.c.y, accV.d.x, accV.d.y};
+#pragma unroll
+    for (int i = 0; i < 8; ++i) {
+      float v = accu[i];
+      v += __shfl_xor(v, 8, 64);
+      v += __shfl_xor(v, 16, 64);
+      v += __shfl_xor(v, 32, 64);
+      if (lane < 8) redu[wave * 64 + 8 * lane + i] = v;
+    }
+    accV = zero8();
+  }
   const float accp[16] = {accK.a.x + accV.a.x, accK.a.y + accV.a.y, accK.b.x + accV.b.x, accK.b.y + accV.b.y,
                           accK.c.x + accV.c.x, accK.c.y + accV.c.y, accK.d.x + accV.d.x, accK.d.y + accV.d.y,
                           accR.a.x, accR.a.y, accR.b.x, accR.b.y, accR.c.x, accR.c.y, accR.d.x, accR.d.y};
@@ -461,7 +611,29 @@
   if (tid < 64) {
     slab[kVecOffM + 64 + tid] = (redd[tid] + redd[64 + tid]) + (redd[128 + tid] + redd[192 + tid]);
     slab[kVecOffM + tid] = (redr[tid] + redr[64 + tid]) + (redr[128 + tid] + redr[192 + tid]);
-    slab[kVecOffM + 128 + tid] = (redp[tid] + redp[64 + tid]) + (redp[128 + tid] + redp[192 + tid]);
+    if constexpr (!VTAB) slab[kVecOffM + 128 + tid] = (redp[tid] + redp[64 + tid]) + (redp[128 + tid] + redp[192 + tid]);
+  }
+  if constexpr (VTAB) {
+    if (tid < 64) upad[tid] = (redu[tid] + redu[64 + tid]) + (redu[128 + tid] + redu[192 + tid]);
+    __syncthreads();
+    {
+      const float xc = xpad[fb + c16];
+#pragma unroll
+      for (int reg = 0; reg < 4; ++reg) {
+        const int row = 4 * kq + reg, col = fb + c16;
+        slab[1 * 4096 + row * 64 + col] = am0[reg] + upad[row] * xc; slab[1 * 4096 + (row + 16) * 64 + col] = am1[reg] + upad[row + 16] * xc;
+        slab[1 * 4096 + (row + 32) * 64 + col] = am2[reg] + upad[row + 32] * xc; slab[1 * 4096 + (row + 48) * 64 + col] = am3[reg] + upad[row + 48] * xc;
+      }
+    }
+    if (tid < 64) {
+      const float* mp = g.mM + (int64_t)head * 4096 + tid;
+      float s0 = 0.f, s1 = 0.f, s2 = 0.f, s3 = 0.f;
+#pragma unroll 4
+      for (int n = 0; n < 64; n += 4) {
+        s0 += upad[n] * mp[n * 64]; s1 += upad[n + 1] * mp[(n + 1) * 64]; s2 += upad[n + 2] * mp[(n + 2) * 64]; s3 += upad[n + 3] * mp[(n + 3) * 64];
+      }
+      slab[kVecOffM + 128 + tid] = ((redp[tid] + redp[64 + tid]) + (redp[128 + tid] + redp[192 + tid])) + ((s0 + s1) + (s2 + s3));
+    }
   }
 }
 
@@ -707,10 +879,11 @@
 
 int launch_fused_bwd_merged(const matcha_tensors& p, const float* folded, const float* merged, const float* X, const float* dDyn, const float* dXs,
                             const Ragged& rg, int64_t B, int L, float* dxh, float* ws, matcha_tensors& grads, float* dZ0, hipStream_t st, const float* rimg,
-                            bool dx_atomic, bool dx_zeroed, const TailReduceArgs* tail, const int32_t* xrow, const float* xhatN, const float* rn, int64_t rn_rows) {
+                            bool dx_atomic, bool dx_zeroed, const TailReduceArgs* tail, const int32_t* xrow, const float* xhatN, const float* rn, int64_t rn_rows, const float* vn) {
   const int64_t tcap = B * L + 1;
   MATCHA_CHECK_ARG(!xrow || xhatN, "fused backward: the node route needs the table of normalised rows");
   MATCHA_CHECK_ARG(!rn || xrow, "fused backward: the r table belongs to the node route");
+  MATCHA_CHECK_ARG(!vn || rn, "fused backward: the value table needs the r table");
   if (dx_atomic && !dx_zeroed) MATCHA_TRY(zero_async(dxh, (size_t)tcap * 64 * sizeof(float), st));
   int nchunks = 2 * chunks_for(rg.nhalves);
   if (nchunks > kMaxChunks) nchunks = kMaxChunks;
@@ -725,7 +898,7 @@
     FusedBwdHArgs g;
     g.X = xrow ? xhatN : X; g.dDyn = dDyn; g.count = rg.count; g.half_meta = rg.half_meta; g.tok_pos = rg.tok_pos; g.L = L; g.nhalves = rg.nhalves; g.nchunks = nchunks;
     g.mB = mv.B; g.mM = mv.M; g.dxh = dxh; g.tcap = tcap; g.dx_atomic = dx_atomic ? 1 : 0; g.wslab = wslab; g.rimg = rimg; g.xrow = xrow;
-    g.rn = rn; g.rn_head = rn_rows * 64;
+    g.rn = rn; g.rn_head = rn_rows * 64; g.vn = vn;
     const size_t lds = kBwdLdsBytes;
     auto launch = [&](auto kfn) {
       (void)hipFuncSetAttribute(reinterpret_cast<const void*>(kfn), hipFuncAttributeMaxDynamicSharedMemorySize, 160 * 1024);
@@ -733,12 +906,12 @@
     };
     ProfScope ps(MATCHA_PROF_FUSED_BWD, (double)tcap * MATCHA_N_HEAD * 8.0 * 2.0 * 64.0 * 64.0, st);
     switch (L <= 2 ? 2 : (L <= 6 ? L : 8)) {
-      case 2: if (xrow) launch(fused_bwdh_kernel<2, true>); else launch(fused_bwdh_kernel<2, false>); break;
-      case 3: if (xrow) launch(fused_bwdh_kernel<3, true>); else launch(fused_bwdh_kernel<3, false>); break;
-      case 4: if (xrow) launch(fused_bwdh_kernel<4, true>); else launch(fused_bwdh_kernel<4, false>); break;
-      case 5: if (xrow) launch(fused_bwdh_kernel<5, true>); else launch(fused_bwdh_kernel<5, false>); break;
-      case 6: if (xrow) launch(fused_bwdh_kernel<6, true>); else launch(fused_bwdh_kernel<6, false>); break;
-      default: if (xrow) launch(fused_bwdh_kernel<8, true>); else launch(fused_bwdh_kernel<8, false>); break;
+      case 2: if (vn) launch(fused_bwdh_kernel<2, true, true>); else if (xrow) launch(fused_bwdh_kernel<2, true>); else launch(fused_bwdh_kernel<2, false>); break;
+      case 3: if (vn) launch(fused_bwdh_kernel<3, true, true>); else if (xrow) launch(fused_bwdh_kernel<3, true>); else launch(fused_bwdh_kernel<3, false>); break;
+      case 4: if (vn) launch(fused_bwdh_kernel<4, true, true>); else if (xrow) launch(fused_bwdh_kernel<4, true>); else launch(fused_bwdh_kernel<4, false>); break;
+      case 5: if (vn) launch(fused_bwdh_kernel<5, true, true>); else if (xrow) launch(fused_bwdh_kernel<5, true>); else launch(fused_bwdh_kernel<5, false>); break;
+      case 6: if (vn) launch(fused_bwdh_kernel<6, true, true>); else if (xrow) launch(fused_bwdh_kernel<6, true>); else launch(fused_bwdh_kernel<6, false>); break;
+      default: if (vn) launch(fused_bwdh_kernel<8, true, true>); else if (xrow) launch(fused_bwdh_kernel<8, true>); else launch(fused_bwdh_kernel<8, false>); break;
     }
     MATCHA_CHECK_LAUNCH("fused_bwdh_kernel");
   }
diff --git a/matcha_amd/csrc/fused_fwd32.hip b/matcha_amd/csrc/fused_fwd32.hip
--- a/matcha_amd/csrc/fused_fwd32.hip
+++ b/matcha_amd/csrc/fused_fwd32.hip
@@ -562,15 +562,16 @@
 #endif
 }
 
-struct NodeRArgs { const float* X; const u32x4* wfrag; float* rn; int rows; };
+struct NodeRArgs { const float* X; const u32x4* wfrag; float* rn; int rows; float* vn; };
 __global__ __launch_bounds__(64) void node_r_kernel(NodeRArgs g) {
   const int lane = threadIdx.x, r = lane & 31, h = lane >> 5;
-  const int hd = blockIdx.y;
+  const int hd = blockIdx.y & 7;
+  const bool vrole = blockIdx.y >= MATCHA_N_HEAD;
   const int row = (int)blockIdx.x * 32 + r;
   const bool live = row < g.rows;
   const u32x4* wp;
   u32x4 W_[F32_WIN];
-  W32_PRIME_AT(hd == 0 ? 0 : 2 * hd - 1);
+  W32_PRIME_AT(vrole ? (hd < 7 ? 2 * hd + 2 : 15) : (hd == 0 ? 0 : 2 * hd - 1));
   FL xh = fl_load(g.X + (int64_t)(live ? row : g.rows - 1) * 64 + 4 * h);
   {
     float mean, rx;
@@ -581,16 +582,17 @@
   B3 xs[4];
   FL_SPLIT(xs[0], xh, 0); FL_SPLIT(xs[1], xh, 1); FL_SPLIT(xs[2], xh, 2); FL_SPLIT(xs[3], xh, 3);
   FL q = F32_BIAS(kBiasR + hd);
+  if (vrole) q = fl_zero();
   W32_CHAIN_XS(q, xs, false);
-  if (live) fl_store_global(g.rn + ((int64_t)hd * g.rows + row) * 64 + 4 * h, q);
+  if (live) fl_store_global((vrole ? g.vn : g.rn) + ((int64_t)hd * g.rows + row) * 64 + 4 * h, q);
 }
 
 size_t node_r_floats(int64_t rows) { return (size_t)MATCHA_N_HEAD * rows * 64; }
-int launch_node_r(const float* XN, const float* frag, int64_t rows, float* rn, hipStream_t st) {
+int launch_node_r(const float* XN, const float* frag, int64_t rows, float* rn, hipStream_t st, float* vn) {
   NodeRArgs g;
-  g.X = XN; g.wfrag = reinterpret_cast<const u32x4*>(frag); g.rn = rn; g.rows = (int)rows;
+  g.X = XN; g.wfrag = reinterpret_cast<const u32x4*>(frag); g.rn = rn; g.rows = (int)rows; g.vn = vn;
   ProfScope ps(MATCHA_PROF_FUSED_FWD, 0.0, st);
-  hipLaunchKernelGGL(node_r_kernel, dim3((unsigned)cdiv(rows, 32), MATCHA_N_HEAD), dim3(64), 0, st, g);
+  hipLaunchKernelGGL(node_r_kernel, dim3((unsigned)cdiv(rows, 32), vn ? 2 * MATCHA_N_HEAD : MATCHA_N_HEAD), dim3(64), 0, st, g);
   MATCHA_CHECK_LAUNCH("node_r_kernel");
   return MATCHA_OK;
 }
diff --git a/matcha_amd/csrc/kernels.hpp b/matcha_amd/csrc/kernels.hpp
--- a/matcha_amd/csrc/kernels.hpp
+++ b/matcha_amd/csrc/kernels.hpp
@@ -102,6 +102,7 @@
   int disable_wide_gemm;
   int disable_node_front;
   int disable_node_r;
+  int disable_node_v;
   int debug_nan, fused_dbg;
 };
 Options& options();
@@ -143,7 +144,7 @@
                        const int32_t* xrow = nullptr,
                        const float* rn = nullptr, int64_t rn_rows = 0);
 size_t node_r_floats(int64_t rows);
-int launch_node_r(const float* XN, const float* frag, int64_t rows, float* rn, hipStream_t st);
+int launch_node_r(const float* XN, const float* frag, int64_t rows, float* rn, hipStream_t st, float* vn = nullptr);
 int tail_bwd_grid();
 size_t tail_bwd_slab_floats();
 int launch_tail_bwd64(const matcha_tensors& p, const float* dH2, const float* Y, const float* H1, const Ragged& rg, const uint64_t* seed, float p_fc1,
@@ -156,7 +157,8 @@
                             const Ragged& rg, int64_t B, int L, float* dxh, float* ws, matcha_tensors& grads, float* dZ0, hipStream_t st, const float* rimg,
                             bool dx_atomic, bool dx_zeroed = false,
                             const struct TailReduceArgs* tail = nullptr, const int32_t* xrow = nullptr, const float* xhatN = nullptr,
-                            const float* rn = nullptr, int64_t rn_rows = 0);
+                            const float* rn = nullptr, int64_t rn_rows = 0,
+                            const float* vn = nullptr);
 size_t fused_qkv_floats(int64_t B, int L);
 constexpr int kImgRecH = 2048 + 256;
 
diff --git a/matcha_amd/csrc/model.hip b/matcha_amd/csrc/model.hip
--- a/matcha_amd/csrc/model.hip
+++ b/matcha_amd/csrc/model.hip
@@ -96,13 +96,14 @@
   void* tg_ws;      size_t tg_ws_bytes;
   float *XN, *x0N, *xhN, *GN; int64_t* node_ids; int32_t* node_cnt;
   float* RN;
+  float* VN;
   size_t total;
 };
 
 struct OptionName { const char* name; int Options::*field; };
 static const OptionName kOptionNames[] = {
     {"disable_fused", &Options::disable_fused}, {"disable_merged", &Options::disable_merged}, {"disable_small_batch", &Options::disable_small_batch},
-    {"disable_wide_gemm", &Options::disable_wide_gemm}, {"disable_node_front", &Options::disable_node_front}, {"disable_node_r", &Options::disable_node_r}, {"debug_nan", &Options::debug_nan}, {"fused_dbg", &Options::fused_dbg}};
+    {"disable_wide_gemm", &Options::disable_wide_gemm}, {"disable_node_front", &Options::disable_node_front}, {"disable_node_r", &Options::disable_node_r}, {"disable_node_v", &Options::disable_node_v}, {"debug_nan", &Options::debug_nan}, {"fused_dbg", &Options::fused_dbg}};
 Options& options() {
   static Options o = [] {
     Options v;
@@ -130,6 +131,7 @@
 static bool node_front_shape(const matcha_shape& s, int64_t B, int L) {
   return s.mode == 0 && s.d == 64 && front_bwd_supported(s.d, s.n_attr) && B * L + 1 >= 4 * ((int64_t)s.n_nodes + 1);
 }
+static bool node_v_shape(const matcha_shape& s, int64_t B, int L) { return B * L + 1 >= 64 * ((int64_t)s.n_nodes + 1); }
 static bool has_target(int objective, const float* y, const float* w) { return objective == MATCHA_OBJECTIVE_SOFTPLUS_MSE ? y != nullptr : (y && w); }
 static bool loss_in_forward(const matcha_shape& s, const matcha_step_opts& o, const float* y, const float* w, int objective) {
   return o.loss_in_forward && !o.forward_only && has_target(objective, y, w) && fused_enabled(s);
@@ -142,7 +144,7 @@
 static std::mutex g_fwd_mu;
 static std::unordered_map<const void*, std::pair<int, uint64_t>> g_fwd_state;
 static uint64_t g_fwd_clock = 0;
-static void note_forward(const void* ws, bool merged, bool fused, bool enc = false, bool split_tail = false, bool dx_zeroed = false, bool node = false, bool node_r = false) {
+static void note_forward(const void* ws, bool merged, bool fused, bool enc = false, bool split_tail = false, bool dx_zeroed = false, bool node = false, bool node_r = false, bool node_v = false) {
   std::lock_guard<std::mutex> lk(g_fwd_mu);
   if (g_fwd_state.size() >= 4096 && g_fwd_state.find(ws) == g_fwd_state.end()) {
     auto old = g_fwd_state.begin();
@@ -150,7 +152,7 @@
       if (it->second.second < old->second.second) old = it;
     g_fwd_state.erase(old);
   }
-  g_fwd_state[ws] = std::make_pair((merged ? 1 : 0) | (fused ? 2 : 0) | (enc ? 4 : 0) | (split_tail ? 8 : 0) | (dx_zeroed ? 16 : 0) | (node ? 32 : 0) | (node_r ? 64 : 0), ++g_fwd_clock);
+  g_fwd_state[ws] = std::make_pair((merged ? 1 : 0) | (fused ? 2 : 0) | (enc ? 4 : 0) | (split_tail ? 8 : 0) | (dx_zeroed ? 16 : 0) | (node ? 32 : 0) | (node_r ? 64 : 0) | (node_v ? 128 : 0), ++g_fwd_clock);
 }
 static int ws_state(const void* ws) {
   std::lock_guard<std::mutex> lk(g_fwd_mu);
@@ -251,6 +253,7 @@
     w.node_ids = reinterpret_cast<int64_t*>(take_always(nn * 2));
     w.node_cnt = reinterpret_cast<int32_t*>(take_always(nn ? 64 : 0));
     w.RN = nn ? (compact ? take_always(node_r_floats((int64_t)nn)) : w.Q) : nullptr;
+    w.VN = (nn && !compact && w.Q) ? w.Q + node_r_floats((int64_t)nn) : nullptr;
   }
   w.total = off;
   return off;
@@ -417,6 +420,7 @@
   const bool node = front && fused_path && node_front_shape(s, B, L) && !fused_small_batch(w.rg) && !opts->deterministic && !opts->sparse_table_grad &&
                     !options().disable_node_front;
   const bool node_r = node && !options().disable_node_r;
+  const bool node_v = node_r && !opts->forward_only && w.VN && node_v_shape(s, B, L) && !options().disable_node_v;
   MATCHA_TRY(launch_ragged_plan(x, B, L, s.n_nodes, opts->status, w.rg, st, plan_level, node ? w.node_ids : nullptr, node ? w.node_cnt : nullptr,
                                 (node && !opts->forward_only) ? w.GN : nullptr));
   float* recon_out = losses ? losses + 1 : nullptr;
@@ -440,7 +444,7 @@
       MATCHA_TRY(launch_front_fwd(p, w.node_ids, p.table, nullptr, *frozen, s.n_attr, w.rg, (int64_t)s.n_nodes + 1, opts->forward_only ? nullptr : w.x0N, w.XN, st,
                                   prep_in_front ? &prep : nullptr, w.node_cnt));
       if (!opts->forward_only) MATCHA_TRY(launch_node_xhat(w.XN, w.node_cnt, (int64_t)s.n_nodes + 1, w.xhN, st));
-      if (node_r) MATCHA_TRY(launch_node_r(w.XN, w.frag, (int64_t)s.n_nodes + 1, w.RN, st));
+      if (node_r) MATCHA_TRY(launch_node_r(w.XN, w.frag, (int64_t)s.n_nodes + 1, w.RN, st, node_v ? w.VN : nullptr));
     } else
     MATCHA_TRY(launch_front_fwd(p, ids, s.mode == 0 ? p.table : nullptr, s.mode == 0 ? nullptr : w.node, *frozen, s.n_attr, w.rg, Tn,
                                 opts->forward_only ? nullptr : w.x0, w.X, st, prep_in_front ? &prep : nullptr));
@@ -457,7 +461,7 @@
     float* lg_out = (logits && !save) ? logits : w.logits;
     const bool split_tail = lif && !fused_small_batch(w.rg) && (options().fused_dbg & 1) == 0;
     const bool zero_dx = lif && !opts->deterministic && !opts->sparse_table_grad && (split_tail || fused_small_batch(w.rg)) && tgt && losses;
-    if (opts->forward_only) forget_forward(ws); else note_forward(ws, true, true, false, split_tail, zero_dx, node, node_r);
+    if (opts->forward_only) forget_forward(ws); else note_forward(ws, true, true, false, split_tail, zero_dx, node, node_r, node_v);
     MATCHA_TRY(launch_fused_fwd32(p, w.folded, w.frag, node ? w.XN : w.X, w.rg, B, L, y, w_bce, (save || lif) ? w.Y : nullptr, (save || lif) ? w.H1 : nullptr, (save || lif) ? w.H2 : nullptr,
                                   lg_out, w.row_loss, opts->seed, train ? opts->p_drop_fc1 : 0.f, train ? opts->p_drop_pff : 0.f, st,
                                   lif ? w.ddyn0 : nullptr, w.dXs, w.tslab, opts->alpha, keep_rimg ? w.qkv : nullptr, split_tail ? w.dH2 : nullptr, objective,
@@ -575,7 +579,7 @@
       {"dXs", w.dXs}, {"dZ1", w.dZ1}, {"ddyn0", w.ddyn0}, {"dZ0", w.dZ0}, {"dX0", w.dX0}, {"slab", w.slab}, {"gemm_ws", w.gemm_ws}, {"adj_ws", w.adj_ws},
       {"folded", w.folded}, {"frag", w.frag}, {"merged", w.merged}, {"lwB", w.lwB}, {"lwM", w.lwM}, {"lwdB", w.lwdB}, {"lwdM", w.lwdM}, {"enc", w.enc}, {"fb_ws", w.fb_ws},
       {"tpart", w.tpart}, {"tslab", w.tslab}, {"tslab2", w.tslab2}, {"qkv_records", w.qkv}, {"front_ws", w.front_ws}, {"tg_ws", w.tg_ws}, {"XN", w.XN}, {"x0N", w.x0N}, {"xhN", w.xhN}, {"GN", w.GN},
-      {"node_ids", w.node_ids}, {"node_cnt", w.node_cnt}, {"RN", w.RN}};
+      {"node_ids", w.node_ids}, {"node_cnt", w.node_cnt}, {"RN", w.RN}, {"VN", w.VN}};
   size_t n = 0;
   for (const auto& e : f) {
     if (!e.p) continue;
@@ -657,6 +661,7 @@
   TailReduceArgs tail_args;
   const bool node = fused_fwd && (fwd_state & 32) != 0;
   const bool node_r = node && (fwd_state & 64) != 0;
+  const bool node_v = node_r && (fwd_state & 128) != 0;
   if (lif) {
     const bool small = fused_small_batch(w.rg);
     dx_zeroed = (fwd_state & 16) != 0 && !opts->deterministic && !opts->sparse_table_grad;
@@ -694,7 +699,7 @@
     MATCHA_CHECK_ARG(!node || dx_atomic, "matcha_backward: deterministic / sparse_table_grad differ from the forward's on this workspace");
     MATCHA_TRY(launch_fused_bwd_merged(p, w.folded, w.merged, node ? w.XN : w.X, w.ddyn0, w.dXs, w.rg, B, L, w.dO, w.fb_ws, g_, front ? nullptr : w.dZ0, st, w.qkv, dx_atomic, dx_zeroed,
                                        tail_in_bwd ? &tail_args : nullptr, node ? w.rg.tok_key : nullptr, node ? w.xhN : nullptr,
-                                       node_r ? w.RN : nullptr, (int64_t)s.n_nodes + 1));
+                                       node_r ? w.RN : nullptr, (int64_t)s.n_nodes + 1, node_v ? w.VN : nullptr));
     MATCHA_TRY(encoder_done(*opts, st));
     if (front) {
       if (s.mode == 0) MATCHA_CHECK_ARG(g_.table, "matcha_backward: table mode without a table gradient buffer");
```

New measurement: 55.59 million hyperedges/s (median of 6 runs). +1.6%, better.
